# DecodeGenetics/Ratatosk

Hardware: AMD Instinct MI355X
Metric: corrected long-read bases/sec (higher is better)
Workload: dtype u64

## Files before the change

include/ratatosk_hip.h:

```cpp
#ifndef RATATOSK_HIP_H
#define RATATOSK_HIP_H

#include <stdint.h>

#ifdef __cplusplus
extern "C" {
#endif

#define RTK_OK 0
#define RTK_ERR_IO (-1)
#define RTK_ERR_FORMAT (-2)
#define RTK_ERR_ARG (-3)
#define RTK_ERR_NO_DEVICE (-4)
#define RTK_ERR_DEVICE (-5)
#define RTK_ERR_UNSUPPORTED (-6)

typedef struct rtk_graph rtk_graph;
typedef struct rtk_batch rtk_batch;

typedef struct rtk_opts {
    uint64_t insert_sz;
    uint64_t min_cov_vertices;
    uint64_t max_len_weak_region1;
    uint64_t max_km_cov;
    double weak_region_len_factor;
    double large_k_factor;
    double min_score;
    int32_t max_qual;
    int32_t out_qual;
    double min_confidence_snp_corr;
    int32_t long_read_correct;
    int32_t force_unres_snp_corr;
    uint64_t max_len_weak_region2;
    int32_t a2_exclusive;
    int32_t a3_strand_order;
    int32_t d1_desc;
    uint32_t struct_size;
} rtk_opts;

typedef struct rtk_graph_info {
    uint64_t n_unitigs, n_kmers, n_bases, n_colour_ids, n_global_sets;
    uint64_t table_slots, hbm_bytes;
    uint64_t max_km_cov_top;
    int32_t k, device;
} rtk_graph_info;

typedef struct rtk_stats {
    double ms_total, ms_lookup_exact, ms_mask, ms_lookup_inexact, ms_seeds, ms_regions, ms_correct, ms_stitch;
    uint64_t n_windows, n_probes_exact, n_probes_inexact, n_hits_inexact, n_regions, n_region_items, n_arena_overflow;
    uint64_t n_expand, n_colour_elem, n_path_base, n_align, n_align_cells;
    uint64_t in_bases, out_bases;
    uint64_t cyc_colour, cyc_paths, cyc_consensus, cyc_total, cyc_myers, cyc_sets , cyc_tostring, cyc_pathqual;
    uint64_t n_slots_exact, n_slots_inexact;
    uint64_t cyc_walk, n_moves;
    double ms_lanes;
    uint64_t n_lane_regions, n_lane_handed;
    double ms_phase;
    uint64_t n_phase_skipped;
    uint64_t n_trim_stored, n_trim_column, n_trim_fallback, n_consensus_resumed, n_consensus_swept;
    uint64_t n_fa_linked_run, n_fa_linked_skipped, n_fa_linked_entries;
    uint64_t n_strand2_run, n_strand2_skipped, n_strand2_audit_mismatch;
    uint64_t n_park_walked, n_park_deferred;
    uint64_t n_colours_small, n_colours_wide, n_colours_bits, n_colours_general, n_colours_audit_mismatch;
} rtk_stats;

int rtk_graph_load(const char* unitig_fasta_gz, const char* rtsk, int k, int n_threads, rtk_graph** out);
#define RTK_LOAD_DEVICE_TABLES 1u
int rtk_graph_load2(const char* unitig_fasta_gz, const char* rtsk, int k, int n_threads, uint32_t flags, rtk_graph** out);

int rtk_graph_upload(rtk_graph* g, int device);

int rtk_graph_shell(int k, rtk_graph** out);
int rtk_graph_n_buffers(const rtk_graph* g);
int rtk_graph_buffer(rtk_graph* g, int idx, void** dev_ptr, uint64_t* bytes);
int rtk_graph_alloc_buffers(rtk_graph* g, int device, const uint64_t* bytes, int n, const rtk_graph_info* info);
int rtk_graph_adopt_device(rtk_graph* g);
int rtk_graph_attach_buffers(rtk_graph* g, int device, void* const* dev_ptrs, const uint64_t* bytes, int n, const rtk_graph_info* info);
int rtk_graph_buffer_bytes(const rtk_graph* g, uint64_t* bytes, int n);
int rtk_graph_move_buffer(rtk_graph* g, int idx, void* dev_ptr, uint64_t bytes);
int rtk_graph_host_buffer(const rtk_graph* g, int idx, const void** p, uint64_t* bytes);
int rtk_graph_download_buffer(const rtk_graph* g, int idx, void* host_dst, uint64_t bytes);

int rtk_n_devices(void);
int rtk_device_memory(int device, uint64_t* free_bytes, uint64_t* total_bytes);
int rtk_graph_clone_to_device(const rtk_graph* src, int device, rtk_graph** out);

int rtk_graph_get_info(const rtk_graph* g, rtk_graph_info* info);
void rtk_graph_free(rtk_graph* g);
long long rtk_graph_strip_annotations(rtk_graph* g);

int rtk_reserve_scratch(int device, uint32_t max_read_len);
int rtk_reserve_second_pass(int device, uint32_t n_tickets, uint64_t phase_bytes, uint64_t region_bytes);
int rtk_graph_reserve_batches(rtk_graph* g, uint32_t n_batches, uint64_t bases_per_batch, uint32_t reads_per_batch, int with_qualities, uint64_t raw_bases_per_batch);

int rtk_opts_default(const rtk_graph* g, rtk_opts* opts);

int rtk_correct_batch(rtk_graph* g, const rtk_opts* opts, uint32_t n, const char* const* seq, const char* const* qual,
                      const uint32_t* len, char** out_seq, char** out_qual, uint32_t* out_len);
int rtk_coalesce_stats(rtk_graph* g, uint64_t* n_groups, uint64_t* n_tickets);

int rtk_batch_create(rtk_graph* g, uint32_t n, const char* const* seq, const char* const* qual, const uint32_t* len, rtk_batch** out);
int rtk_batch_create2(rtk_graph* g, uint32_t n, const char* const* seq, const char* const* qual, const uint32_t* len,
                      const char* const* raw, const uint32_t* raw_len, rtk_batch** out);
int rtk_batch_run(rtk_batch* b, const rtk_opts* opts);
int rtk_batch_run_seeds(rtk_batch* b, const rtk_opts* opts);
int rtk_batch_run_regions(rtk_batch* b, const rtk_opts* opts);
int rtk_batch_fetch(rtk_batch* b, char** out_seq, char** out_qual, uint32_t* out_len);
int rtk_batch_fetch_view(rtk_batch* b, const char** pool, const uint64_t** off, const uint32_t** len);
int rtk_batch_get_stats(const rtk_batch* b, rtk_stats* stats);
void rtk_batch_free(rtk_batch* b);


int rtk_lookup_exact(rtk_graph* g, const char* seq, uint32_t len, int64_t* hits);

int rtk_fix_snps(rtk_graph* g, const char* seq, uint32_t len, char* out);

int rtk_seeds(rtk_graph* g, const rtk_opts* opts, const char* seq, uint32_t len,
              uint64_t* n_solid, int64_t* solid, uint64_t* n_weak, int64_t* weak, uint64_t cap);

int rtk_myers_batch(uint32_t n, const char* const* query, const uint32_t* qlen, const char* const* target, const uint32_t* tlen,
                    const int32_t* k, const int32_t* mode, int want_path, int use_iupac,
                    int32_t* dist, int32_t* n_loc, int32_t* end_locs, uint32_t cap_locs, char* cigar, uint32_t cap_cigar);

int rtk_myers_batch_waves(uint32_t n, const char* const* query, const uint32_t* qlen, const char* const* target, const uint32_t* tlen,
                          const int32_t* k, const int32_t* mode, int want_path, int use_iupac,
                          int32_t* dist, int32_t* n_loc, int32_t* end_locs, uint32_t cap_locs, char* cigar, uint32_t cap_cigar, int waves);

#define RTK_MYERS_MODE_SHW_BY_COLUMN 3
#define RTK_MYERS_MODE_NW_PREFIX 4
#define RTK_MYERS_MODE_NW_PREFIX_LAST 5
void rtk_myers_column_last_routes(uint64_t* column_route, uint64_t* fallback);

int rtk_myers_batch_lanes(uint32_t n, const char* const* query, const uint32_t* qlen, const char* const* target, const uint32_t* tlen,
                          const int32_t* k, const int32_t* mode, int want_path, int use_iupac,
                          int32_t* dist, int32_t* n_loc, int32_t* end_locs, uint32_t cap_locs, char* cigar, uint32_t cap_cigar);
void rtk_myers_lanes_last_routes(uint64_t* lane_route, uint64_t* wave_route);

int rtk_index_count_kmers(int device, int k, const char* const* files, int n_files, uint32_t min_count, int n_threads, uint64_t** solid, uint64_t* n_solid);
int rtk_index_unitigs(int device, int k, const uint64_t* solid, uint64_t n_solid, char** seq_pool, uint64_t** seq_off, uint64_t** seeds, uint64_t* n_unitigs,
                      uint64_t** left, uint64_t* n_left);

int rtk_index_colour_begin(int device, int k, const char* seq_pool, const uint64_t* seq_off, uint64_t n_unitigs, void** job);
int rtk_index_colour_chunk(void* job, const char* chars, uint64_t n_chars, const uint64_t* starts, const uint32_t* ids, uint32_t n_reads);
int rtk_index_colour_end(void* job, uint64_t** events, uint64_t* n_events, uint64_t** cov);

int rtk_rescue_begin(int device, int k, const uint64_t* lr, uint64_t n_lr, const uint64_t* sr, uint64_t n_sr, uint32_t min_positions, void** job);
int rtk_rescue_chunk(void* job, const char* chars, uint64_t n_chars, const uint64_t* starts, uint32_t n_reads, unsigned char* keep);
int rtk_rescue_end(void* job, uint64_t* n_positions_probed, uint64_t* n_hits);

#define RTK_SETS_UNION 0
#define RTK_SETS_INTER 1
#define RTK_SETS_DIFF 2
#define RTK_SETS_INTER_COUNT 3
#define RTK_SETS_SORT_PAIRS 4
#define RTK_SETS_RADIX_U32 5
#define RTK_SETS_RADIX_PAIRS_U32 6
#define RTK_SETS_BM_LOWEST 7
#define RTK_SETS_BM8_LOWEST 8
#define RTK_SETS_OK 0
#define RTK_SETS_NOT_IN_BUILD 1
int rtk_sets_batch(uint32_t n, const uint32_t* op, const uint32_t* const* a, const uint32_t* na, const uint32_t* const* b, const uint32_t* nb, const uint32_t* scalar,
                   uint32_t* out_pool, const uint64_t* out_off, uint32_t* out_n, uint32_t* result, uint32_t* status);

void rtk_free(void* p);
void rtk_free_many(void** p, uint32_t n);
const char* rtk_last_error(void);
const char* rtk_version(void);
#define RTK_API_REVISION 10
int rtk_api_revision(void);

#ifdef __cplusplus
}
#endif

#endif
```

ratatosk_amd/api.py:

```python
import ctypes as C
import os

_HERE = os.path.dirname(os.path.abspath(__file__))
LIB_PATH = os.environ.get("RTK_LIB_OVERRIDE") or os.path.join(_HERE, "libratatosk_hip.so")


class RtkError(RuntimeError):
    pass


class RtkOpts(C.Structure):
    _fields_ = [("insert_sz", C.c_uint64), ("min_cov_vertices", C.c_uint64), ("max_len_weak_region1", C.c_uint64),
                ("max_km_cov", C.c_uint64), ("weak_region_len_factor", C.c_double), ("large_k_factor", C.c_double),
                ("min_score", C.c_double), ("max_qual", C.c_int32), ("out_qual", C.c_int32), ("min_confidence_snp_corr", C.c_double),
                ("long_read_correct", C.c_int32), ("force_unres_snp_corr", C.c_int32), ("max_len_weak_region2", C.c_uint64),
                ("a2_exclusive", C.c_int32), ("a3_strand_order", C.c_int32), ("d1_desc", C.c_int32), ("struct_size", C.c_uint32)]


class RtkGraphInfo(C.Structure):
    _fields_ = [("n_unitigs", C.c_uint64), ("n_kmers", C.c_uint64), ("n_bases", C.c_uint64), ("n_colour_ids", C.c_uint64),
                ("n_global_sets", C.c_uint64), ("table_slots", C.c_uint64), ("hbm_bytes", C.c_uint64), ("max_km_cov_top", C.c_uint64),
                ("k", C.c_int32), ("device", C.c_int32)]


class RtkStats(C.Structure):
    _fields_ = [(n, C.c_double) for n in ("ms_total", "ms_lookup_exact", "ms_mask", "ms_lookup_inexact", "ms_seeds", "ms_regions", "ms_correct", "ms_stitch")] + \
               [(n, C.c_uint64) for n in ("n_windows", "n_probes_exact", "n_probes_inexact", "n_hits_inexact", "n_regions", "n_region_items", "n_arena_overflow",
                                         "n_expand", "n_colour_elem", "n_path_base", "n_align", "n_align_cells", "in_bases", "out_bases",
                                         "cyc_colour", "cyc_paths", "cyc_consensus", "cyc_total", "cyc_myers", "cyc_sets", "cyc_tostring", "cyc_pathqual", "n_slots_exact", "n_slots_inexact", "cyc_walk", "n_moves")] + \
               [("ms_lanes", C.c_double), ("n_lane_regions", C.c_uint64), ("n_lane_handed", C.c_uint64), ("ms_phase", C.c_double), ("n_phase_skipped", C.c_uint64)] + \
               [(n, C.c_uint64) for n in ("n_trim_stored", "n_trim_column", "n_trim_fallback", "n_consensus_resumed", "n_consensus_swept",
                                         "n_fa_linked_run", "n_fa_linked_skipped", "n_fa_linked_entries",
                                         "n_strand2_run", "n_strand2_skipped", "n_strand2_audit_mismatch",
                                         "n_park_walked", "n_park_deferred",
                                         "n_colours_small", "n_colours_wide", "n_colours_bits", "n_colours_general", "n_colours_audit_mismatch")]

    def as_dict(self):
        return {n: getattr(self, n) for n, _ in self._fields_}


_libs = {}


os.environ.setdefault("GPU_MAX_HW_QUEUES", "16")


def load_library(path=None):
    path = path or LIB_PATH
    if path in _libs:
        return _libs[path]
    if not os.path.exists(path):
        raise RtkError("%s is missing: build it with `python -c 'import __graft_entry__ as g; g.build()'` (make -C ratatosk_amd/csrc)" % path)
    L = C.CDLL(path)
    L.rtk_last_error.restype = C.c_char_p
    L.rtk_version.restype = C.c_char_p
    L.rtk_graph_load.argtypes = [C.c_char_p, C.c_char_p, C.c_int, C.c_int, C.POINTER(C.c_void_p)]
    L.rtk_graph_load2.argtypes = [C.c_char_p, C.c_char_p, C.c_int, C.c_int, C.c_uint32, C.POINTER(C.c_void_p)]
    L.rtk_graph_move_buffer.argtypes = [C.c_void_p, C.c_int, C.c_void_p, C.c_uint64]
    L.rtk_graph_host_buffer.argtypes = [C.c_void_p, C.c_int, C.POINTER(C.c_void_p), C.POINTER(C.c_uint64)]
    L.rtk_graph_download_buffer.argtypes = [C.c_void_p, C.c_int, C.c_void_p, C.c_uint64]
    L.rtk_graph_upload.argtypes = [C.c_void_p, C.c_int]
    L.rtk_graph_shell.argtypes = [C.c_int, C.POINTER(C.c_void_p)]
    L.rtk_graph_n_buffers.argtypes = [C.c_void_p]
    L.rtk_graph_buffer.argtypes = [C.c_void_p, C.c_int, C.POINTER(C.c_void_p), C.POINTER(C.c_uint64)]
    L.rtk_graph_alloc_buffers.argtypes = [C.c_void_p, C.c_int, C.POINTER(C.c_uint64), C.c_int, C.POINTER(RtkGraphInfo)]
    L.rtk_graph_adopt_device.argtypes = [C.c_void_p]
    L.rtk_graph_buffer_bytes.argtypes = [C.c_void_p, C.POINTER(C.c_uint64), C.c_int]
    L.rtk_graph_get_info.argtypes = [C.c_void_p, C.POINTER(RtkGraphInfo)]
    L.rtk_graph_free.argtypes = [C.c_void_p]
    L.rtk_opts_default.argtypes = [C.c_void_p, C.POINTER(RtkOpts)]
    L.rtk_correct_batch.argtypes = [C.c_void_p, C.POINTER(RtkOpts), C.c_uint32, C.POINTER(C.c_char_p), C.POINTER(C.c_char_p), C.POINTER(C.c_uint32),
                                    C.POINTER(C.c_void_p), C.POINTER(C.c_void_p), C.POINTER(C.c_uint32)]
    L.rtk_batch_create.argtypes = [C.c_void_p, C.c_uint32, C.POINTER(C.c_char_p), C.POINTER(C.c_char_p), C.POINTER(C.c_uint32), C.POINTER(C.c_void_p)]
    L.rtk_batch_create2.argtypes = [C.c_void_p, C.c_uint32, C.POINTER(C.c_char_p), C.POINTER(C.c_char_p), C.POINTER(C.c_uint32),
                                    C.POINTER(C.c_char_p), C.POINTER(C.c_uint32), C.POINTER(C.c_void_p)]
    L.rtk_batch_run.argtypes = [C.c_void_p, C.POINTER(RtkOpts)]
    L.rtk_graph_strip_annotations.restype = C.c_longlong
    L.rtk_graph_strip_annotations.argtypes = [C.c_void_p]
    L.rtk_batch_run_seeds.argtypes = [C.c_void_p, C.POINTER(RtkOpts)]
    L.rtk_batch_run_regions.argtypes = [C.c_void_p, C.POINTER(RtkOpts)]
    L.rtk_batch_fetch.argtypes = [C.c_void_p, C.POINTER(C.c_void_p), C.POINTER(C.c_void_p), C.POINTER(C.c_uint32)]
    L.rtk_batch_fetch_view.argtypes = [C.c_void_p, C.POINTER(C.c_char_p), C.POINTER(C.POINTER(C.c_uint64)), C.POINTER(C.POINTER(C.c_uint32))]
    L.rtk_n_devices.restype = C.c_int
    L.rtk_device_memory.argtypes = [C.c_int, C.POINTER(C.c_uint64), C.POINTER(C.c_uint64)]
    L.rtk_graph_clone_to_device.argtypes = [C.c_void_p, C.c_int, C.POINTER(C.c_void_p)]
    L.rtk_batch_get_stats.argtypes = [C.c_void_p, C.POINTER(RtkStats)]
    L.rtk_batch_free.argtypes = [C.c_void_p]
    L.rtk_lookup_exact.argtypes = [C.c_void_p, C.c_char_p, C.c_uint32, C.POINTER(C.c_int64)]
    L.rtk_fix_snps.argtypes = [C.c_void_p, C.c_char_p, C.c_uint32, C.c_char_p]
    L.rtk_seeds.argtypes = [C.c_void_p, C.POINTER(RtkOpts), C.c_char_p, C.c_uint32, C.POINTER(C.c_uint64), C.POINTER(C.c_int64),
                            C.POINTER(C.c_uint64), C.POINTER(C.c_int64), C.c_uint64]
    L.rtk_myers_batch.argtypes = [C.c_uint32, C.POINTER(C.c_char_p), C.POINTER(C.c_uint32), C.POINTER(C.c_char_p), C.POINTER(C.c_uint32),
                                  C.POINTER(C.c_int32), C.POINTER(C.c_int32), C.c_int, C.c_int,
                                  C.POINTER(C.c_int32), C.POINTER(C.c_int32), C.POINTER(C.c_int32), C.c_uint32, C.c_char_p, C.c_uint32]
    L.rtk_myers_batch_waves.argtypes = L.rtk_myers_batch.argtypes + [C.c_int]
    L.rtk_myers_batch_lanes.argtypes = L.rtk_myers_batch.argtypes
    L.rtk_myers_batch_lanes.restype = C.c_int
    L.rtk_coalesce_stats.argtypes = [C.c_void_p, C.POINTER(C.c_uint64), C.POINTER(C.c_uint64)]
    L.rtk_graph_reserve_batches.argtypes = [C.c_void_p, C.c_uint32, C.c_uint64, C.c_uint32, C.c_int, C.c_uint64]
    L.rtk_free_many.argtypes = [C.POINTER(C.c_void_p), C.c_uint32]; L.rtk_free_many.restype = None
    if L.rtk_api_revision() >= 9:
        L.rtk_rescue_begin.argtypes = [C.c_int, C.c_int, C.POINTER(C.c_uint64), C.c_uint64, C.POINTER(C.c_uint64), C.c_uint64, C.c_uint32, C.POINTER(C.c_void_p)]
        L.rtk_rescue_chunk.argtypes = [C.c_void_p, C.c_char_p, C.c_uint64, C.POINTER(C.c_uint64), C.c_uint32, C.POINTER(C.c_ubyte)]
        L.rtk_rescue_end.argtypes = [C.c_void_p, C.POINTER(C.c_uint64), C.POINTER(C.c_uint64)]
    if L.rtk_api_revision() >= 10:
        L.rtk_sets_batch.argtypes = [C.c_uint32, C.POINTER(C.c_uint32), C.POINTER(C.POINTER(C.c_uint32)), C.POINTER(C.c_uint32), C.POINTER(C.POINTER(C.c_uint32)), C.POINTER(C.c_uint32),
                                     C.POINTER(C.c_uint32), C.POINTER(C.c_uint32), C.POINTER(C.c_uint64), C.POINTER(C.c_uint32), C.POINTER(C.c_uint32), C.POINTER(C.c_uint32)]
    L.rtk_free.argtypes = [C.c_void_p]
    _libs[path] = L
    return L


RTK_LOAD_DEVICE_TABLES = 1


def _b(s):
    return s.encode() if isinstance(s, str) else s


class Graph:

    def __init__(self, fasta_gz, rtsk, k=31, device=0, lib_path=None, upload=True, n_threads=None, host_tables=None):
        self.L = load_library(lib_path)
        self.h = C.c_void_p()
        if n_threads is None:
            n_threads = max(1, min(32, os.cpu_count() or 1))
        if host_tables is None:
            host_tables = not upload or os.environ.get("RTK_HOST_TABLES") == "1"
        self._check(self.L.rtk_graph_load2(_b(fasta_gz), _b(rtsk), k, n_threads, 0 if host_tables else RTK_LOAD_DEVICE_TABLES, C.byref(self.h)))
        self.k = k
        if upload:
            self._check(self.L.rtk_graph_upload(self.h, device))

    def _check(self, rc):
        if rc != 0:
            raise RtkError("rtk error %d: %s" % (rc, self.L.rtk_last_error().decode()))

    def close(self):
        if getattr(self, "h", None):
            self.L.rtk_graph_free(self.h)
            self.h = None

    def __del__(self):
        try:
            self.close()
        except Exception:
            pass

    def info(self):
        i = RtkGraphInfo()
        self._check(self.L.rtk_graph_get_info(self.h, C.byref(i)))
        return i

    def opts(self, **kw):
        o = RtkOpts()
        self._check(self.L.rtk_opts_default(self.h, C.byref(o)))
        for k_, v in kw.items():
            setattr(o, k_, v)
        return o

    def lookup_exact(self, seq):
        s = _b(seq)
        nw = max(0, len(s) - self.k + 1)
        out = (C.c_int64 * max(1, nw))()
        self._check(self.L.rtk_lookup_exact(self.h, s, len(s), out))
        return [out[i] for i in range(nw)]

    def fix_snps(self, seq):
        s = _b(seq)
        out = C.create_string_buffer(len(s) + 1)
        self._check(self.L.rtk_fix_snps(self.h, s, len(s), out))
        return out.raw[:len(s)]

    def seeds(self, seq, opts=None):
        s = _b(seq)
        o = opts or self.opts()
        cap = 64 * len(s) + 64
        ns, nw = C.c_uint64(), C.c_uint64()
        so, we = (C.c_int64 * (4 * cap))(), (C.c_int64 * (4 * cap))()
        self._check(self.L.rtk_seeds(self.h, C.byref(o), s, len(s), C.byref(ns), so, C.byref(nw), we, cap))
        f = lambda a, n: [(a[4 * i], a[4 * i + 1], a[4 * i + 2], a[4 * i + 3]) for i in range(n)]
        return f(so, ns.value), f(we, nw.value)

    def correct_batch(self, seqs, quals=None, opts=None, raw=None):
        b = Batch(self, seqs, quals, raw)
        try:
            b.run(opts)
            return b.fetch()
        finally:
            b.close()


class Batch:

    def __init__(self, graph, seqs, quals=None, raw=None):
        self.g = graph
        self.L = graph.L
        n = len(seqs)
        bs = [_b(s) for s in seqs]
        seq_arr = (C.c_char_p * n)(*bs)
        qual_arr = None
        if quals is not None:
            bq = [_b(q) for q in quals]
            qual_arr = (C.c_char_p * n)(*bq)
        lens = (C.c_uint32 * n)(*[len(b) for b in bs])
        self.n = n
        self.in_bases = sum(len(b) for b in bs)
        self.h = C.c_void_p()
        if raw is not None:
            br = [_b(s) for s in raw]
            raw_arr = (C.c_char_p * n)(*br)
            raw_lens = (C.c_uint32 * n)(*[len(b) for b in br])
            graph._check(self.L.rtk_batch_create2(graph.h, n, seq_arr, qual_arr, lens, raw_arr, raw_lens, C.byref(self.h)))
        else:
            graph._check(self.L.rtk_batch_create(graph.h, n, seq_arr, qual_arr, lens, C.byref(self.h)))

    def run(self, opts=None):
        o = opts or self.g.opts()
        self.g._check(self.L.rtk_batch_run(self.h, C.byref(o)))

    def run_seeds(self, opts=None):
        o = opts or self.g.opts()
        self.g._check(self.L.rtk_batch_run_seeds(self.h, C.byref(o)))

    def run_regions(self, opts=None):
        o = opts or self.g.opts()
        self.g._check(self.L.rtk_batch_run_regions(self.h, C.byref(o)))

    def fetch(self):
        n = self.n
        os_, oq = (C.c_void_p * n)(), (C.c_void_p * n)()
        ol = (C.c_uint32 * n)()
        self.g._check(self.L.rtk_batch_fetch(self.h, os_, oq, ol))
        out = []
        for i in range(n):
            out.append((C.string_at(os_[i], ol[i]).decode(), C.string_at(oq[i], ol[i]).decode()))
            self.L.rtk_free(os_[i]); self.L.rtk_free(oq[i])
        return out

    def stats(self):
        s = RtkStats()
        self.g._check(self.L.rtk_batch_get_stats(self.h, C.byref(s)))
        return s.as_dict()

    def close(self):
        if getattr(self, "h", None):
            self.L.rtk_batch_free(self.h)
            self.h = None

    def __del__(self):
        try:
            self.close()
        except Exception:
            pass


def myers_batch(queries, targets, ks=None, modes=None, want_path=False, use_iupac=True, lib_path=None, waves=0, lanes=False):
    L = load_library(lib_path)
    n = len(queries)
    bq = [_b(q) for q in queries]; bt = [_b(t) for t in targets]
    ks = ks if ks is not None else [-1] * n
    modes = modes if modes is not None else [0] * n
    qa = (C.c_char_p * n)(*bq); ta = (C.c_char_p * n)(*bt)
    ql = (C.c_uint32 * n)(*[len(x) for x in bq]); tl = (C.c_uint32 * n)(*[len(x) for x in bt])
    ka = (C.c_int32 * n)(*ks); ma = (C.c_int32 * n)(*modes)
    cap_locs = max(len(x) for x in bt) + 2 if n else 2
    cap_cig = 4 * (max((len(x) for x in bq), default=0) + max((len(x) for x in bt), default=0)) + 16
    dist = (C.c_int32 * n)(); nloc = (C.c_int32 * n)(); locs = (C.c_int32 * (n * cap_locs))()
    cig = C.create_string_buffer(n * cap_cig) if want_path else None
    if lanes:
        rc = L.rtk_myers_batch_lanes(n, qa, ql, ta, tl, ka, ma, 1 if want_path else 0, 1 if use_iupac else 0, dist, nloc, locs, cap_locs, cig, cap_cig)
    elif waves > 1:
        rc = L.rtk_myers_batch_waves(n, qa, ql, ta, tl, ka, ma, 1 if want_path else 0, 1 if use_iupac else 0, dist, nloc, locs, cap_locs, cig, cap_cig, waves)
    else:
        rc = L.rtk_myers_batch(n, qa, ql, ta, tl, ka, ma, 1 if want_path else 0, 1 if use_iupac else 0, dist, nloc, locs, cap_locs, cig, cap_cig)
    if rc != 0:
        raise RtkError("rtk error %d: %s" % (rc, L.rtk_last_error().decode()))
    out = []
    for i in range(n):
        el = [locs[i * cap_locs + j] for j in range(min(nloc[i], cap_locs))] if dist[i] >= 0 else []
        c = ""
        if want_path:
            c = cig.raw[i * cap_cig:(i + 1) * cap_cig].split(b"\0", 1)[0].decode()
        out.append((dist[i], el, c))
    return out


def _u64_array(a):
    if hasattr(a, "ctypes"):
        import numpy as np
        arr = np.ascontiguousarray(a, dtype=np.uint64)
        return arr, arr.ctypes.data_as(C.POINTER(C.c_uint64)), int(arr.size)
    arr = (C.c_uint64 * max(1, len(a)))(*[int(x) for x in a])
    return arr, arr, len(a)


def rescue_reads(lr_kmers, sr_kmers, seqs, k=31, min_positions=31, device=0, stats=None, lib_path=None):
    L = load_library(lib_path)
    if L.rtk_api_revision() < 9:
        raise RtkError("%s is of interface revision %d: the rescue entries came with revision 9" % (L._name, L.rtk_api_revision()))
    keep_lr, p_lr, n_lr = _u64_array(lr_kmers)
    keep_sr, p_sr, n_sr = _u64_array(sr_kmers)
    job = C.c_void_p()

    def check(rc):
        if rc != 0:
            raise RtkError("rtk error %d: %s" % (rc, L.rtk_last_error().decode()))

    check(L.rtk_rescue_begin(device, k, p_lr, n_lr, p_sr, n_sr, min_positions, C.byref(job)))
    out = []
    try:
        bs = [_b(s) for s in seqs]
        i = 0
        while i < len(bs):
            j, size = i, 0
            while j < len(bs) and (j == i or (size + len(bs[j]) + 1 <= (48 << 20) and j - i < (2 << 20))):
                size += len(bs[j]) + 1; j += 1
            starts, at = (C.c_uint64 * (j - i))(), 0
            for r in range(i, j):
                starts[r - i] = at; at += len(bs[r]) + 1
            chars = b"\n".join(bs[i:j]) + b"\n"
            keep = (C.c_ubyte * (j - i))()
            check(L.rtk_rescue_chunk(job, chars, len(chars), starts, j - i, keep))
            out.extend(bool(x) for x in keep)
            i = j
    except Exception:
        L.rtk_rescue_end(job, None, None)
        raise
    probed, hits = C.c_uint64(), C.c_uint64()
    check(L.rtk_rescue_end(job, C.byref(probed), C.byref(hits)))
    if stats is not None:
        stats["n_positions_probed"], stats["n_hits"] = probed.value, hits.value
    return out


MODE_SHW_BY_COLUMN, MODE_NW_PREFIX, MODE_NW_PREFIX_LAST = 3, 4, 5


def myers_column_last_routes(lib_path=None):
    L = load_library(lib_path)
    a, b = C.c_uint64(), C.c_uint64()
    L.rtk_myers_column_last_routes.argtypes = [C.POINTER(C.c_uint64), C.POINTER(C.c_uint64)]; L.rtk_myers_column_last_routes.restype = None
    L.rtk_myers_column_last_routes(C.byref(a), C.byref(b))
    return a.value, b.value


def myers_lanes_last_routes(lib_path=None):
    L = load_library(lib_path)
    a, b = C.c_uint64(), C.c_uint64()
    L.rtk_myers_lanes_last_routes.argtypes = [C.POINTER(C.c_uint64), C.POINTER(C.c_uint64)]; L.rtk_myers_lanes_last_routes.restype = None
    L.rtk_myers_lanes_last_routes(C.byref(a), C.byref(b))
    return a.value, b.value


SETS_UNION, SETS_INTER, SETS_DIFF, SETS_INTER_COUNT, SETS_SORT_PAIRS, SETS_RADIX_U32, SETS_RADIX_PAIRS_U32, SETS_BM_LOWEST, SETS_BM8_LOWEST = range(9)
SETS_OK, SETS_NOT_IN_BUILD = 0, 1


def sets_batch(problems, lib_path=None):
    import numpy as np
    L = load_library(lib_path)
    if L.rtk_api_revision() < 10:
        raise RtkError("%s is of interface revision %d: rtk_sets_batch came with revision 10" % (L._name, L.rtk_api_revision()))
    n = len(problems)
    keep, off = [], [0]
    ops = (C.c_uint32 * max(1, n))(); na = (C.c_uint32 * max(1, n))(); nb = (C.c_uint32 * max(1, n))(); sc = (C.c_uint32 * max(1, n))()
    pa = (C.POINTER(C.c_uint32) * max(1, n))(); pb = (C.POINTER(C.c_uint32) * max(1, n))()
    for i, (op, a, b, scalar) in enumerate(problems):
        if op == SETS_SORT_PAIRS:
            a = np.ascontiguousarray(a, dtype="<u8"); b = np.ascontiguousarray(b, dtype="<u8")
            count_a, count_b, a, b = int(a.size), int(b.size), a.view("<u4"), b.view("<u4")
        else:
            a = np.ascontiguousarray(a, dtype=np.uint32); b = np.ascontiguousarray(b, dtype=np.uint32)
            count_a, count_b = int(a.size), int(b.size)
        keep.append((a, b))
        ops[i], na[i], nb[i], sc[i] = op, count_a, count_b, scalar
        pa[i] = a.ctypes.data_as(C.POINTER(C.c_uint32)); pb[i] = b.ctypes.data_as(C.POINTER(C.c_uint32))
        need = {SETS_UNION: count_a + count_b, SETS_INTER: count_a, SETS_DIFF: count_a, SETS_INTER_COUNT: 0, SETS_SORT_PAIRS: 4 * count_a, SETS_RADIX_U32: count_a,
                SETS_RADIX_PAIRS_U32: 2 * count_a, SETS_BM_LOWEST: min(scalar, count_b), SETS_BM8_LOWEST: min(scalar, count_b)}.get(op, 0)
        off.append(off[-1] + need)
    out = np.zeros(max(1, off[-1]), dtype=np.uint32)
    offs = (C.c_uint64 * (n + 1))(*off)
    out_n = (C.c_uint32 * max(1, n))(); res = (C.c_uint32 * max(1, n))(); st = (C.c_uint32 * max(1, n))()
    rc = L.rtk_sets_batch(n, ops, pa, na, pb, nb, sc, out.ctypes.data_as(C.POINTER(C.c_uint32)), offs, out_n, res, st)
    if rc != 0:
        raise RtkError("rtk error %d: %s" % (rc, L.rtk_last_error().decode()))
    ret = []
    for i, (op, _, _, _) in enumerate(problems):
        if out_n[i] > off[i + 1] - off[i]:
            raise RtkError("rtk_sets_batch: problem %d reports %d output words for a slice of %d" % (i, out_n[i], off[i + 1] - off[i]))
        w = out[off[i]:off[i] + out_n[i]]
        if op == SETS_SORT_PAIRS and st[i] == SETS_OK:
            h = len(w) // 2
            words = (w[:h].copy().view("<u8").tolist(), w[h:].copy().view("<u8").tolist())
        else:
            words = w.tolist()
        ret.append((words, int(res[i]), int(st[i])))
    return ret


def run_pipelined(batches, opts=None):
    import threading
    prev, err = None, []

    def seeds(b):
        try:
            b.run_seeds(opts)
        except Exception as e:
            err.append(e)

    for b in batches:
        t = threading.Thread(target=seeds, args=(b,))
        t.start()
        if prev is not None:
            prev.run_regions(opts)
        t.join()
        if err:
            raise err[0]
        prev = b
    if prev is not None:
        prev.run_regions(opts)
```

ratatosk_amd/csrc/hip/rtk_colours.h:

```cpp
#ifndef RTK_COLOURS_H
#define RTK_COLOURS_H

#define RTK_CB_MAX_IDS (RTK_LDS_SET_CAP - 384u)
#define RTK_CB_MAX_SLOTS 24u

#ifndef RTK_SIM
RTK_DEV void rtk_radix_sort_u32(uint32_t* a, uint32_t* b, uint32_t n, uint32_t* bins, uint32_t max_key) {
    const uint32_t lane = static_cast<uint32_t>(rtk_lane());
    const uint64_t lt = (1ull << lane) - 1ull;
    int passes = 0; { uint32_t m = max_key; while (m) { ++passes; m >>= 8; } if (passes == 0) passes = 1; }
    if (passes & 1) ++passes;
    uint32_t* src = a; uint32_t* dst = b;
    for (int ps = 0; ps < passes; ++ps) {
        const int sh = 8 * ps;
        for (uint32_t i = lane; i < 256u; i += RTK_WAVE) bins[i] = 0u;
        RTK_WG_SYNC();
        for (uint32_t c0 = 0; c0 < n; c0 += RTK_WAVE) {
            const uint32_t i = c0 + lane; const bool ok = i < n;
            const uint32_t d = ok ? ((src[i] >> sh) & 0xFFu) : 0x100u;
            uint64_t eq = rtk_ballot(ok);
            for (int bt = 0; bt < 8; ++bt) { const uint64_t bb = rtk_ballot((d >> bt) & 1u); eq &= ((d >> bt) & 1u) ? bb : ~bb; }
            if (ok && (eq & lt) == 0ull) atomicAdd(&bins[d], static_cast<uint32_t>(rtk_popc(eq)));
        }
        RTK_WG_SYNC();
        {
            uint32_t v[4]; uint32_t sum = 0;
            for (int x = 0; x < 4; ++x) { v[x] = bins[4u * lane + static_cast<uint32_t>(x)]; sum += v[x]; }
            int tot; uint32_t base = static_cast<uint32_t>(rtk_wave_excl_scan(static_cast<int>(sum), &tot));
            RTK_WG_SYNC();
            for (int x = 0; x < 4; ++x) { bins[4u * lane + static_cast<uint32_t>(x)] = base; base += v[x]; }
        }
        RTK_WG_SYNC();
        for (uint32_t c0 = 0; c0 < n; c0 += RTK_WAVE) {
            const uint32_t i = c0 + lane; const bool ok = i < n;
            const uint32_t key = ok ? src[i] : 0u;
            const uint32_t d = ok ? ((key >> sh) & 0xFFu) : 0x100u;
            uint64_t eq = rtk_ballot(ok);
            for (int bt = 0; bt < 8; ++bt) { const uint64_t bb = rtk_ballot((d >> bt) & 1u); eq &= ((d >> bt) & 1u) ? bb : ~bb; }
            const uint32_t before = static_cast<uint32_t>(rtk_popc(eq & lt));
            uint32_t base = 0;
            if (ok) base = bins[d];
            RTK_WG_SYNC();
            if (ok && before == 0u) bins[d] = base + static_cast<uint32_t>(rtk_popc(eq));
            if (ok) dst[base + before] = key;
            RTK_WG_SYNC();
        }
        uint32_t* t_ = src; src = dst; dst = t_;
    }
}
#endif

#ifdef RTK_SIM
struct RtkBM { uint64_t w[64]; };
inline RtkBM rtk_bm_zero() { RtkBM r; for (int i = 0; i < 64; ++i) r.w[i] = 0; return r; }
inline RtkBM operator|(const RtkBM& a, const RtkBM& b) { RtkBM r; for (int i = 0; i < 64; ++i) r.w[i] = a.w[i] | b.w[i]; return r; }
inline RtkBM operator&(const RtkBM& a, const RtkBM& b) { RtkBM r; for (int i = 0; i < 64; ++i) r.w[i] = a.w[i] & b.w[i]; return r; }
inline RtkBM rtk_bm_andn(const RtkBM& a, const RtkBM& b) { RtkBM r; for (int i = 0; i < 64; ++i) r.w[i] = a.w[i] & ~b.w[i]; return r; }
inline uint32_t rtk_bm_count(const RtkBM& a) { uint32_t c = 0; for (int i = 0; i < 64; ++i) c += static_cast<uint32_t>(__builtin_popcountll(a.w[i])); return c; }
inline RtkBM rtk_bm_lowest(const RtkBM& a, uint32_t q) { RtkBM r = rtk_bm_zero(); for (int i = 0; i < 64 && q; ++i) { uint64_t x = a.w[i]; while (x && q) { const uint64_t b = x & (~x + 1ull); r.w[i] |= b; x ^= b; --q; } } return r; }
inline RtkBM rtk_bm_load(const uint64_t* p) { RtkBM r; for (int i = 0; i < 64; ++i) r.w[i] = p[i]; return r; }
inline void rtk_bm_store(uint64_t* p, const RtkBM& a) { for (int i = 0; i < 64; ++i) p[i] = a.w[i]; }
#else
typedef uint64_t RtkBM;
RTK_DEV RtkBM rtk_bm_zero() { return 0ull; }
RTK_DEV RtkBM rtk_bm_andn(RtkBM a, RtkBM b) { return a & ~b; }
RTK_DEV uint32_t rtk_bm_count(RtkBM a) { return static_cast<uint32_t>(rtk_u(rtk_wave_sum(rtk_popc(a)))); }
RTK_DEV RtkBM rtk_bm_lowest(RtkBM a, uint32_t q) {
    int total; const int before = rtk_wave_excl_scan(rtk_popc(a), &total);
    int keep = static_cast<int>(q) - before; const int mine = rtk_popc(a);
    keep = keep < 0 ? 0 : (keep > mine ? mine : keep);
    uint64_t rest = a; for (int i = 0; i < keep; ++i) rest &= rest - 1ull;
    return a & ~rest;
}
RTK_DEV RtkBM rtk_bm_load(const uint64_t* p) { return p[rtk_lane()]; }
RTK_DEV void rtk_bm_store(uint64_t* p, RtkBM a) { p[rtk_lane()] = a; }
#endif

RTK_DEV RtkBM rtk_bm_from_ids(const uint32_t* uni, uint32_t U, uint64_t* scatter, const uint32_t* ids, uint32_t n) {
#ifdef RTK_SIM
    (void)scatter;
    RtkBM r = rtk_bm_zero();
    for (uint32_t i = 0; i < n; ++i) { const uint32_t x = rtk_lower_bound(uni, U, ids[i]); r.w[x >> 6] |= 1ull << (x & 63u); }
    return r;
#else
    scatter[rtk_lane()] = 0ull;
    RTK_WG_SYNC();
    for (uint32_t i = static_cast<uint32_t>(rtk_lane()); i < n; i += RTK_WAVE) {
        const uint32_t id = ids[i];
        uint32_t lo = 0, hi = U; while (lo < hi) { const uint32_t mid = (lo + hi) >> 1; if (uni[mid] < id) lo = mid + 1; else hi = mid; }
        atomicOr(reinterpret_cast<unsigned long long*>(scatter) + (lo >> 6), 1ull << (lo & 63u));
    }
    RTK_WG_SYNC();
    return scatter[rtk_lane()];
#endif
}


#ifndef RTK_SIM
#ifndef RTK_CS_MAX_IDS
#define RTK_CS_MAX_IDS 512u
#endif
static_assert(2u * RTK_CS_MAX_IDS + 768u <= RTK_LDS_SET_CAP && RTK_CS_MAX_IDS <= 512u, "small path of the colour selection: universe + unsorted ids + 24 x 2 x 8 vector words in the LDS buffer");
RTK_DEV int rtk_sum8(int v) {
    v += __builtin_amdgcn_update_dpp(0, v, 0xB1, 0xF, 0xF, false);
    v += __builtin_amdgcn_update_dpp(0, v, 0x4E, 0xF, 0xF, false);
    v += __builtin_amdgcn_update_dpp(0, v, 0x141, 0xF, 0xF, false);
    return v;
}
RTK_DEV uint32_t rtk_bm8_count(RtkBM a) { return static_cast<uint32_t>(__builtin_amdgcn_readfirstlane(rtk_sum8(rtk_popc(a)))); }
RTK_DEV RtkBM rtk_bm8_lowest(RtkBM a, uint32_t q) {
    const int mine = rtk_popc(a);
    int inc = mine;
    inc += __builtin_amdgcn_update_dpp(0, inc, 0x111, 0xF, 0xF, true);
    inc += __builtin_amdgcn_update_dpp(0, inc, 0x112, 0xF, 0xF, true);
    inc += __builtin_amdgcn_update_dpp(0, inc, 0x114, 0xF, 0xF, true);
    int keep = static_cast<int>(q) - (inc - mine);
    keep = keep < 0 ? 0 : (keep > mine ? mine : keep);
    uint64_t rest = a; for (int i = 0; i < keep; ++i) rest &= rest - 1ull;
    return a & ~rest;
}
RTK_FN uint32_t rtk_choose_colors_small(const RCtx& c_, const SideList& side_s_, const SideList& side_e_, const SideList& side_w_) {
    const RCtx& c = *rtk_u(&c_); const SideList& side_s = *rtk_u(&side_s_); const SideList& side_e = *rtk_u(&side_e_); const SideList& side_w = *rtk_u(&side_w_); RTK_ASSUME_LDS(&side_s); RTK_ASSUME_LDS(&side_e); RTK_ASSUME_LDS(&side_w);
    RegionScratch& s = rtk_hdr(c);
    const GraphView& g = c.g;
    const uint32_t nw = rtk_u(side_w.n), ne = rtk_u(side_e.n), ns = rtk_u(side_s.n), n_slots = nw + ne + ns;
    if (n_slots == 0 || n_slots > RTK_CB_MAX_SLOTS) return RTK_NONE32;
    const uint32_t lane = static_cast<uint32_t>(rtk_lane());
    const uint32_t* const pw = rtk_u(side_w.u); const uint32_t* const pe = rtk_u(side_e.u); const uint32_t* const ps = rtk_u(side_s.u);
    const uint8_t* const qw = rtk_u(side_w.nb); const uint8_t* const qe = rtk_u(side_e.nb); const uint8_t* const qs = rtk_u(side_s.nb);
    const uint32_t* const col = g.col; const uint64_t* const loff = g.loff; const uint64_t* const goff = g.goff; const int32_t* const gid = g.gid; const uint32_t* const cardp = g.card;
    unsigned long long tl_ = rtk_clock();
#define RTK_CS_LAP(i) { (void)tl_; }
    uint32_t m_u = 0, m_nl = 0, m_ng = 0, m_card = 0, m_nb = 0; uint64_t m_lo = 0, m_go = 0; int32_t m_gi = -1;
    if (lane < n_slots) {
        const uint32_t* pu; const uint8_t* pn; uint32_t i = lane;
        if (i < nw) { pu = pw; pn = qw; } else if (i - nw < ne) { i -= nw; pu = pe; pn = qe; } else { i -= nw + ne; pu = ps; pn = qs; }
        m_u = pu[i]; m_nb = pn[i];
        m_gi = gid[m_u]; m_lo = loff[m_u]; m_nl = static_cast<uint32_t>(loff[m_u + 1] - m_lo); m_card = cardp[m_u];
        if (m_gi >= 0) { m_go = goff[m_gi]; m_ng = static_cast<uint32_t>(goff[m_gi + 1] - m_go); }
    }
    int total = 0; const uint32_t st = static_cast<uint32_t>(rtk_wave_excl_scan(static_cast<int>(m_nl + m_ng), &total));
    const uint32_t T = static_cast<uint32_t>(rtk_u(total));
    const bool big = T > RTK_CS_MAX_IDS;
    if (T > RTK_CB_MAX_IDS || (big && (s.set_cap < RTK_CB_MAX_IDS || s.set_cap < 2u * 2u * 64u * RTK_CB_MAX_SLOTS))) return RTK_NONE32;
    RTK_CS_LAP(1)
    const uint32_t min_cov_v = c.o.min_cov_vertices;
    bool dup = false;
    for (uint32_t j = 0; j + 1 < n_slots; ++j) { const uint32_t uj = rtk_shfl(m_u, static_cast<int>(j)); dup = dup || ((j < lane) && (uj == m_u)); }
    const bool cand = lane < n_slots && m_card >= min_cov_v && !dup;
    const uint64_t cb = rtk_ballot(cand); const uint32_t nsp = static_cast<uint32_t>(rtk_popc(cb));
    const uint64_t key = rtk_d1_key(m_card, m_u, c.o.d1_desc);
    uint32_t rank = 0;
    for (uint32_t j = 0; j < n_slots; ++j) { const uint64_t kj = rtk_shfl(key, static_cast<int>(j)); rank += (((cb >> j) & 1ull) && kj < key) ? 1u : 0u; }
    uint32_t src = 0;
    for (uint32_t j = 0; j < n_slots; ++j) { const uint32_t rj = rtk_shfl(rank, static_cast<int>(j)); if (((cb >> j) & 1ull) && rj == lane) src = j; }
    const uint32_t cov = 30;
    const uint32_t k_slot = src; const uint32_t k_card = rtk_shfl(m_card, static_cast<int>(src));
    uint32_t k_quota = k_card < cov ? k_card : cov;
    RTK_CS_LAP(2)
    uint32_t* const L = rtk_lds_set_buf();
    uint32_t* const uni = L; uint32_t* const raw = L + RTK_CS_MAX_IDS;
    uint64_t* const cbm = big ? reinterpret_cast<uint64_t*>(s.set[2].get()) : reinterpret_cast<uint64_t*>(L + 2u * RTK_CS_MAX_IDS);
    const uint32_t VW = big ? 64u : 8u;
    uint32_t P = 64; while (P < T) P <<= 1;
    for (uint32_t t0 = 0; t0 < P; t0 += RTK_WAVE) {
        const uint32_t t = t0 + lane;
        uint32_t i = 0;
        for (uint32_t j = 1; j < n_slots; ++j) { const uint32_t sj = rtk_shfl(st, static_cast<int>(j)); if (sj <= t) i = j; }
        const uint32_t s_i = rtk_shfl(st, static_cast<int>(i)), nl_i = rtk_shfl(m_nl, static_cast<int>(i));
        const uint64_t lo_i = rtk_shfl(m_lo, static_cast<int>(i)), go_i = rtk_shfl(m_go, static_cast<int>(i));
        uint32_t x = 0xFFFFFFFFu;
        if (t < T) { const uint32_t off = t - s_i; x = col[off < nl_i ? lo_i + off : go_i + (off - nl_i)]; if (!big) raw[t] = x; }
        if (t < T || !big) uni[t] = x;
    }
    RTK_WG_SYNC();
    s.cnt[RTK_RC_COLOUR] += T;
    RTK_CS_LAP(3)
    {
        uint32_t mx = 0; for (uint32_t i2 = lane; i2 < T; i2 += RTK_WAVE) mx = uni[i2] > mx ? uni[i2] : mx;
        for (int o = 32; o > 0; o >>= 1) { const uint32_t v2 = static_cast<uint32_t>(__shfl_xor(static_cast<int>(mx), o, 64)); mx = v2 > mx ? v2 : mx; }
        if (big) rtk_radix_sort_u32(uni, s.set[1], T, L + RTK_CB_MAX_IDS, rtk_u(mx));
        else rtk_radix_sort_u32(uni, L + 2u * RTK_CS_MAX_IDS, T, L + 2u * RTK_CS_MAX_IDS + RTK_CS_MAX_IDS, rtk_u(mx));
    }
    uint32_t U = 0;
    for (uint32_t i0 = 0; i0 < T; i0 += RTK_WAVE) {
        const uint32_t i = i0 + lane;
        uint32_t x = 0; bool keep = false;
        if (i < T) { x = uni[i]; keep = (i == 0) || (uni[i - 1] != x); }
        RTK_WG_SYNC();
        const uint64_t bal = rtk_ballot(keep);
        if (keep) uni[U + static_cast<uint32_t>(rtk_popc(bal & ((1ull << lane) - 1ull)))] = x;
        U += static_cast<uint32_t>(rtk_popc(bal));
        RTK_WG_SYNC();
    }
    RTK_CS_LAP(4)
    for (uint32_t i = lane; i < n_slots * 2u * VW; i += RTK_WAVE) cbm[i] = 0ull;
    RTK_WG_SYNC();
    for (uint32_t t0 = 0; t0 < T; t0 += RTK_WAVE) {
        const uint32_t t = t0 + lane;
        uint32_t i = 0;
        for (uint32_t j = 1; j < n_slots; ++j) { const uint32_t sj = rtk_shfl(st, static_cast<int>(j)); if (sj <= t) i = j; }
        const uint32_t s_i = rtk_shfl(st, static_cast<int>(i)), nl_i = rtk_shfl(m_nl, static_cast<int>(i));
        const uint64_t lo_i2 = rtk_shfl(m_lo, static_cast<int>(i)), go_i2 = rtk_shfl(m_go, static_cast<int>(i));
        if (t < T) {
            const uint32_t off2 = t - s_i;
            const uint32_t id = big ? col[off2 < nl_i ? lo_i2 + off2 : go_i2 + (off2 - nl_i)] : raw[t];
            uint32_t lo = 0, hi = U; while (lo < hi) { const uint32_t mid = (lo + hi) >> 1; if (uni[mid] < id) lo = mid + 1; else hi = mid; }
            const uint32_t seg = 2u * i + ((t - s_i) >= nl_i ? 1u : 0u);
            atomicOr(reinterpret_cast<unsigned long long*>(cbm) + seg * VW + (lo >> 6), 1ull << (lo & 63u));
        }
    }
    RTK_WG_SYNC();
    RTK_CS_LAP(5)
    auto ld = [&](uint32_t idx) -> RtkBM { if (lane >= VW) return 0ull; return big ? static_cast<RtkBM>(__hip_atomic_load(reinterpret_cast<const unsigned long long*>(cbm) + idx * VW + lane, __ATOMIC_RELAXED, __HIP_MEMORY_SCOPE_AGENT)) : cbm[idx * VW + lane]; };
    auto cnt_ = [&](RtkBM a) -> uint32_t { return big ? rtk_bm_count(a) : rtk_bm8_count(a); };
    auto low_ = [&](RtkBM a, uint32_t q) -> RtkBM { return big ? rtk_bm_lowest(a, q) : rtk_bm8_lowest(a, q); };
    RtkBM a[6];
    for (int sh = 0; sh < 6; ++sh) {
        RtkBM acc = 0ull;
        const uint32_t first = (sh % 3 == 0) ? 0u : (sh % 3 == 1 ? nw : nw + ne), cnt = (sh % 3 == 0) ? nw : (sh % 3 == 1 ? ne : ns);
        const uint32_t want_nb = sh >= 3 ? 1u : 0u;
        for (uint32_t slot = first; slot < first + cnt; ++slot) {
            if (rtk_u(rtk_shfl(m_nb, static_cast<int>(slot))) != want_nb) continue;
            const bool has_global = rtk_u(rtk_shfl(m_gi, static_cast<int>(slot))) >= 0;
            acc |= ld(2u * slot + (has_global ? 1u : 0u));
        }
        a[sh] = acc;
    }
    const RtkBM pos0 = a[0] | a[3], pos1 = a[1] | a[4], pos2 = a[2] | a[5];
    const RtkBM a01 = pos0 & pos1, a12 = pos1 & pos2, a02 = pos0 & pos2;
    const RtkBM nobranch_all = a[3] | a[4] | a[5];
    const RtkBM i3 = a01 & a12, i2 = a01 | a12 | a02;
    RtkBM nobranch = nobranch_all, branching = 0ull, prev2 = 0ull, all = 0ull;
    uint32_t nb_unselected = nsp;
    for (int i = 5; i >= 0; --i) {
        if (nb_unselected == 0) break;
        RtkBM a2;
        if (i == 5) a2 = nobranch & i3;
        else if (i == 4) { nobranch = rtk_bm_andn(nobranch, prev2); a2 = nobranch & i2; }
        else if (i == 3) { nobranch = rtk_bm_andn(nobranch, prev2); a2 = nobranch; }
        else if (i == 2) { branching = rtk_bm_andn(a[0] | a[1] | a[2], nobranch_all); a2 = branching & i3; }
        else if (i == 1) { branching = rtk_bm_andn(branching, prev2); a2 = branching & i2; }
        else { branching = rtk_bm_andn(branching, prev2); a2 = branching; }
        prev2 = a2;
        if (cnt_(a2) == 0) continue;
        nb_unselected = 0;
        RtkBM curr = a2;
        for (uint32_t j = 0; j < nsp; ++j) {
            int quota = static_cast<int>(rtk_u(rtk_shfl(k_quota, static_cast<int>(j))));
            if (quota > 0) {
                const uint32_t slot = rtk_u(rtk_shfl(k_slot, static_cast<int>(j)));
                const RtkBM cu = ld(2u * slot) | ld(2u * slot + 1u);
                if (i == 0 || cnt_(cu & curr) >= 1) {
                    const uint32_t cd = rtk_u(rtk_shfl(k_card, static_cast<int>(j))); const uint32_t min_cov = cd < cov ? cd : cov;
                    const uint32_t sh = cnt_(cu & all);
                    quota = static_cast<int>(min_cov - (sh < min_cov ? sh : min_cov));
                    if (quota > 0) {
                        const uint32_t all_card = cnt_(all);
                        const RtkBM pid = low_(cu & curr, static_cast<uint32_t>(quota));
                        all = all | pid; curr = rtk_bm_andn(curr, pid);
                        const int gained = static_cast<int>(cnt_(all) - all_card);
                        quota -= gained < quota ? gained : quota;
                    }
                }
                if (lane == j) k_quota = static_cast<uint32_t>(quota);
            }
            nb_unselected += quota > 0 ? 1u : 0u;
        }
    }
    RTK_CS_LAP(6)
    const uint32_t n_all = rtk_bm_count(all);
    if (n_all > s.set_cap) { rtk_fail_ovf(s, 9); return 0; }
    uint32_t* out = s.set[0];
    { int tot2; uint32_t at = static_cast<uint32_t>(rtk_wave_excl_scan(rtk_popc(all), &tot2)); uint64_t x = all;
      while (x) { const int b = __builtin_ctzll(x); out[at++] = uni[64u * lane + static_cast<uint32_t>(b)]; x &= x - 1ull; } }
    rtk_sync();
    s.cnt[big ? RTK_RC_COLOURS_WIDE : RTK_RC_COLOURS_SMALL] += 1;
    return n_all;
}
#endif

RTK_FN uint32_t rtk_choose_colors_bits(const RCtx& c_, const SideList& side_s_, const SideList& side_e_, const SideList& side_w_) {
    const RCtx& c = *rtk_u(&c_); const SideList& side_s = *rtk_u(&side_s_); const SideList& side_e = *rtk_u(&side_e_); const SideList& side_w = *rtk_u(&side_w_); RTK_ASSUME_LDS(&side_s); RTK_ASSUME_LDS(&side_e); RTK_ASSUME_LDS(&side_w);
    RegionScratch& s = rtk_hdr(c);
    const GraphView& g = c.g;
    const SideList* sides[3] = {&side_w, &side_e, &side_s};
    const uint32_t n_slots = side_w.n + side_e.n + side_s.n;
    if (n_slots == 0 || n_slots > RTK_CB_MAX_SLOTS || s.set_cap < 2 * RTK_CB_MAX_IDS + 64u * 4u * RTK_CB_MAX_SLOTS || s.list_cap < 2 * RTK_CB_MAX_SLOTS) return RTK_NONE32;
    uint32_t T = 0;
    for (int sd = 0; sd < 3; ++sd) for (uint32_t i = 0; i < sides[sd]->n; ++i) {
        const uint32_t u = sides[sd]->u[i]; const int32_t gi = g.gid[u];
        T += static_cast<uint32_t>(g.loff[u + 1] - g.loff[u]) + (gi >= 0 ? static_cast<uint32_t>(g.goff[gi + 1] - g.goff[gi]) : 0u);
        if (T > RTK_CB_MAX_IDS) return RTK_NONE32;
    }
    uint64_t* keys = s.list[4]; uint64_t* vals = s.list[3]; uint64_t* slot_of = s.list[5];
    uint32_t nsp = 0;
    { uint32_t slot = 0;
      for (int sd = 0; sd < 3; ++sd) for (uint32_t i = 0; i < sides[sd]->n; ++i, ++slot) {
        const uint32_t u = sides[sd]->u[i];
        if (g.card[u] < c.o.min_cov_vertices) continue;
        bool dup = false; for (uint32_t j0 = 0; j0 < nsp && !dup; j0 += RTK_WAVE) { const uint32_t j = j0 + static_cast<uint32_t>(rtk_lane()); dup = rtk_ballot(j < nsp && rtk_d1_unitig(keys[j], c.o.d1_desc) == u) != 0ull; }
        if (dup) continue;
        keys[nsp] = rtk_d1_key(g.card[u], u, c.o.d1_desc); vals[nsp] = slot; ++nsp; rtk_sync();
      } }
    rtk_sort_pairs(keys, vals, nsp);
    const uint32_t cov = 30;
    for (uint32_t j = static_cast<uint32_t>(rtk_lane()); j < nsp; j += RTK_WAVE) { slot_of[j] = vals[j]; const uint32_t cd = static_cast<uint32_t>(keys[j] >> 32); vals[j] = cd < cov ? cd : cov; }
    rtk_sync();
    uint32_t* gathered = s.set[1];
    { uint32_t at = 0;
      for (int sd = 0; sd < 3; ++sd) for (uint32_t i = 0; i < sides[sd]->n; ++i) {
        const uint32_t u = sides[sd]->u[i]; const int32_t gi = g.gid[u];
        const uint32_t nl = static_cast<uint32_t>(g.loff[u + 1] - g.loff[u]); const uint32_t* pl = g.col + g.loff[u];
        for (uint32_t x = static_cast<uint32_t>(rtk_lane()); x < nl; x += RTK_WAVE) gathered[at + x] = pl[x];
        at += nl;
        if (gi >= 0) { const uint32_t ng = static_cast<uint32_t>(g.goff[gi + 1] - g.goff[gi]); const uint32_t* pg = g.col + g.goff[gi];
                       for (uint32_t x = static_cast<uint32_t>(rtk_lane()); x < ng; x += RTK_WAVE) gathered[at + x] = pg[x]; at += ng; }
      } }
    rtk_sync();
    s.cnt[RTK_RC_COLOUR] += T;
    uint32_t U = 0;
#ifdef RTK_SIM
    uint32_t* const uni = s.set[1] + RTK_CB_MAX_IDS; uint64_t* const scatter = nullptr;
    { for (uint32_t i = 0; i < T; ++i) uni[i] = gathered[i];
      std::sort(uni, uni + T);
      for (uint32_t i = 0; i < T; ++i) if (i == 0 || uni[i] != uni[i - 1]) uni[U++] = uni[i]; }
#else
    uint32_t* const uni = rtk_lds_set_buf(); uint64_t* const scatter = reinterpret_cast<uint64_t*>(uni + RTK_CB_MAX_IDS + 256u);
    {
      uint32_t mx = 0;
      for (uint32_t i = static_cast<uint32_t>(rtk_lane()); i < T; i += RTK_WAVE) { const uint32_t x = gathered[i]; uni[i] = x; mx = x > mx ? x : mx; }
      for (int o = 32; o > 0; o >>= 1) { const uint32_t v2 = static_cast<uint32_t>(__shfl_xor(static_cast<int>(mx), o, 64)); mx = v2 > mx ? v2 : mx; }
      RTK_WG_SYNC();
      rtk_radix_sort_u32(uni, gathered, T, uni + RTK_CB_MAX_IDS, rtk_u(mx));
      for (uint32_t i0 = 0; i0 < T; i0 += RTK_WAVE) {
          const uint32_t i = i0 + static_cast<uint32_t>(rtk_lane());
          uint32_t x = 0; bool keep = false;
          if (i < T) { x = uni[i]; keep = (i == 0) || (uni[i - 1] != x); }
          RTK_WG_SYNC();
          const uint64_t bal = rtk_ballot(keep);
          if (keep) uni[U + static_cast<uint32_t>(rtk_popc(bal & ((1ull << rtk_lane()) - 1ull)))] = x;
          U += static_cast<uint32_t>(rtk_popc(bal));
          RTK_WG_SYNC();
      } }
#endif
    uint64_t* const store = reinterpret_cast<uint64_t*>(s.set[2].get());
    { uint32_t slot = 0;
      for (int sd = 0; sd < 3; ++sd) for (uint32_t i = 0; i < sides[sd]->n; ++i, ++slot) {
        const uint32_t u = sides[sd]->u[i]; const int32_t gi = g.gid[u];
        const RtkBM bl = rtk_bm_from_ids(uni, U, scatter, g.col + g.loff[u], static_cast<uint32_t>(g.loff[u + 1] - g.loff[u]));
        rtk_bm_store(store + (2ull * slot) * 64ull, bl);
        const RtkBM bg = gi >= 0 ? rtk_bm_from_ids(uni, U, scatter, g.col + g.goff[gi], static_cast<uint32_t>(g.goff[gi + 1] - g.goff[gi])) : rtk_bm_zero();
        rtk_bm_store(store + (2ull * slot + 1ull) * 64ull, bg);
      } }
    rtk_sync();
    RtkBM a[6];
    for (int sh = 0; sh < 6; ++sh) {
        RtkBM acc = rtk_bm_zero();
        uint32_t slot = (sh % 3 == 0) ? 0u : (sh % 3 == 1 ? side_w.n : side_w.n + side_e.n);
        const SideList& sl = *sides[sh % 3]; const uint8_t want_nb = sh >= 3 ? 1 : 0;
        for (uint32_t i = 0; i < sl.n; ++i, ++slot) {
            if (sl.nb[i] != want_nb) continue;
            const bool has_global = g.gid[sl.u[i]] >= 0;
            acc = acc | rtk_bm_load(store + (2ull * slot + (has_global ? 1ull : 0ull)) * 64ull);
        }
        a[sh] = acc;
    }
    const RtkBM pos0 = a[0] | a[3], pos1 = a[1] | a[4], pos2 = a[2] | a[5];
    const RtkBM a01 = pos0 & pos1, a12 = pos1 & pos2, a02 = pos0 & pos2;
    const RtkBM nobranch_all = a[3] | a[4] | a[5];
    const RtkBM i3 = a01 & a12, i2 = a01 | a12 | a02;
    RtkBM nobranch = nobranch_all, branching = rtk_bm_zero(), prev2 = rtk_bm_zero(), all = rtk_bm_zero();
    uint32_t nb_unselected = nsp;
    for (int i = 5; i >= 0; --i) {
        if (nb_unselected == 0) break;
        RtkBM a2;
        if (i == 5) a2 = nobranch & i3;
        else if (i == 4) { nobranch = rtk_bm_andn(nobranch, prev2); a2 = nobranch & i2; }
        else if (i == 3) { nobranch = rtk_bm_andn(nobranch, prev2); a2 = nobranch; }
        else if (i == 2) { branching = rtk_bm_andn(a[0] | a[1] | a[2], nobranch_all); a2 = branching & i3; }
        else if (i == 1) { branching = rtk_bm_andn(branching, prev2); a2 = branching & i2; }
        else { branching = rtk_bm_andn(branching, prev2); a2 = branching; }
        prev2 = a2;
        if (rtk_bm_count(a2) == 0) continue;
        nb_unselected = 0;
        RtkBM curr = a2;
        for (uint32_t j = 0; j < nsp; ++j) {
            const uint32_t u = rtk_d1_unitig(rtk_ld(keys + j), c.o.d1_desc);
            int quota = static_cast<int>(rtk_ld(vals + j));
            if (quota > 0) {
                const uint64_t slot = rtk_ld(slot_of + j);
                const RtkBM cu = rtk_bm_load(store + (2ull * slot) * 64ull) | rtk_bm_load(store + (2ull * slot + 1ull) * 64ull);
                if (i == 0 || rtk_bm_count(cu & curr) >= 1) {
                    const uint32_t cd = rtk_ld(g.card.get() + u); const uint32_t min_cov = cd < cov ? cd : cov;
                    const uint32_t sh = rtk_bm_count(cu & all);
                    quota = static_cast<int>(min_cov - (sh < min_cov ? sh : min_cov));
                    if (quota > 0) {
                        const uint32_t all_card = rtk_bm_count(all);
                        const RtkBM pid = rtk_bm_lowest(cu & curr, static_cast<uint32_t>(quota));
                        all = all | pid; curr = rtk_bm_andn(curr, pid);
                        const int gained = static_cast<int>(rtk_bm_count(all) - all_card);
                        quota -= gained < quota ? gained : quota;
                    }
                }
            }
            vals[j] = static_cast<uint64_t>(quota);
            nb_unselected += quota > 0 ? 1u : 0u;
        }
        rtk_sync();
    }
    const uint32_t n_all = rtk_bm_count(all);
    if (n_all > s.set_cap) { rtk_fail_ovf(s, 9); return 0; }
    uint32_t* out = s.set[0];
#ifdef RTK_SIM
    { uint32_t at = 0; for (uint32_t w = 0; w < 64; ++w) { uint64_t x = all.w[w]; while (x) { const int b = __builtin_ctzll(x); out[at++] = uni[64u * w + static_cast<uint32_t>(b)]; x &= x - 1ull; } } }
#else
    { int total; uint32_t at = static_cast<uint32_t>(rtk_wave_excl_scan(rtk_popc(all), &total)); uint64_t x = all;
      while (x) { const int b = __builtin_ctzll(x); out[at++] = uni[64u * static_cast<uint32_t>(rtk_lane()) + static_cast<uint32_t>(b)]; x &= x - 1ull; } }
#endif
    rtk_sync();
    return n_all;
}

#endif
```

ratatosk_amd/csrc/hip/rtk_device.hip:

```cpp
#include <algorithm>
#include <atomic>
#include <chrono>
#include <cmath>
#include <cstdio>
#include <cstring>
#include <map>
#include <memory>
#include <condition_variable>
#include <mutex>
#include <string>
#include <thread>
#include <vector>

#include "../../../include/ratatosk_hip.h"
#include "../host/flat_graph.hpp"
#include "rtk_graph_tables.h"
#include "rtk_mem.h"
#include "rtk_myers.h"
#include "rtk_myers_lane.h"
#include "rtk_types.h"
#include "rtk_wave.h"

#ifdef RTK_SIM
thread_local int rtk_sim_block_id = 0;
// ... 432 lines not shown

RTK_FN void rtk_myers_column_item(const MyersScratch& sc, const MyersProb& p, uint32_t i, const char* q, const char* t, int use_iupac, int32_t* dist, int32_t* n_loc, int32_t* end_locs,
                                  uint32_t cap_locs, uint8_t* moves_out, uint32_t* n_moves_out, uint32_t cap_moves, uint32_t* status) {
    const int m = static_cast<int>(p.qlen), n = static_cast<int>(p.tlen); const bool iupac = use_iupac != 0;
    uint32_t route = 2, nm = 0;
    MyersResult r;
    if (p.mode == RTK_MYERS_MODE_SHW_BY_COLUMN) {
        if (rtk_myers_shw_by_column(sc, t, n, q, m, iupac, 0, 0, &r, nullptr)) route = 1;
        else r = rtk_myers_distance(sc, q, m, t, n, -1, RTK_MODE_SHW, iupac);
        if (cap_locs > 0) end_locs[static_cast<uint64_t>(i) * cap_locs] = r.first;
        if (r.nloc > 1 && static_cast<uint32_t>(r.nloc) <= cap_locs) end_locs[static_cast<uint64_t>(i) * cap_locs + (r.nloc - 1)] = r.last;
        n_loc[i] = r.nloc;
    } else {
        const int k = p.k; const bool last_only = p.mode == RTK_MYERS_MODE_NW_PREFIX_LAST;
        int at = 0, last = -1;
        if (k > 0 && rtk_myers_shw_by_column(sc, q, m, t, n, iupac, 1, k, &r, &at)) {
            const long long W = (k + 63) >> 6;
            if (static_cast<uint32_t>(k) <= sc.r_cap && static_cast<uint32_t>(k + n) <= sc.mv_cap && (2LL * 8 + 4) * W * n + 8LL * n < 1024 * 1024) {
                if (last_only) last = rtk_myers_last_move(sc, k, n, n, at);
                else rtk_myers_walk(sc, k, n, n, at, &nm);
                r.dist = at; route = 1;
            }
        }
        if (route != 1) {
            if (k > 0 && n > 0) r = rtk_myers_path(sc, q, k, t, n, RTK_MODE_NW, iupac, &nm);
            else r = rtk_myers_distance(sc, q, k, t, n, -1, RTK_MODE_NW, iupac);
            if (last_only) { rtk_sync(); last = nm ? static_cast<int>(rtk_ld(sc.moves.get() + (nm - 1u))) : -1; nm = 0; }
        }
        if (cap_locs > 0) end_locs[static_cast<uint64_t>(i) * cap_locs] = last_only ? last : n - 1;
        n_loc[i] = 1;
    }
    dist[i] = r.dist;
    if (nm <= cap_moves) rtk_wcopy(moves_out + static_cast<uint64_t>(i) * cap_moves, sc.moves, nm);
    n_moves_out[i] = nm;
    status[i] = *sc.overflow | (route << 16);
}

RTK_FN void rtk_myers_batch_item(const MyersScratch& sc, const MyersProb& p, uint32_t i, const char* pool, int want_path, int use_iupac, int32_t* dist, int32_t* n_loc, int32_t* end_locs, uint32_t cap_locs,
                                 uint8_t* moves_out, uint32_t* n_moves_out, uint32_t cap_moves, uint32_t* status) {
    *sc.overflow = 0;
    const char* q = pool + p.q_off; const char* t = pool + p.t_off;
    if (p.mode >= RTK_MYERS_MODE_SHW_BY_COLUMN) { rtk_myers_column_item(sc, p, i, q, t, use_iupac, dist, n_loc, end_locs, cap_locs, moves_out, n_moves_out, cap_moves, status); return; }
    const MyersResult r = rtk_myers_distance(sc, q, static_cast<int>(p.qlen), t, static_cast<int>(p.tlen), p.k, p.mode, use_iupac != 0, cap_locs ? end_locs + static_cast<uint64_t>(i) * cap_locs : nullptr, static_cast<int>(cap_locs));
    dist[i] = r.dist; n_loc[i] = r.nloc;
    uint32_t nm = 0;
    if (want_path && r.dist >= 0 && p.qlen > 0 && p.tlen > 0) {
        if (p.k < 0 && p.mode != RTK_MODE_HW) {
            const MyersResult r2 = rtk_myers_path(sc, q, static_cast<int>(p.qlen), t, static_cast<int>(p.tlen), p.mode, use_iupac != 0, &nm);
            if (r2.dist != r.dist || r2.first != r.first) *sc.overflow = 3;
        } else
        rtk_myers_alignment(sc, q, static_cast<int>(p.qlen), t, r.first + 1, r.dist, use_iupac != 0, &nm);
        if (nm <= cap_moves) rtk_wcopy(moves_out + static_cast<uint64_t>(i) * cap_moves, sc.moves, nm);
    }
    n_moves_out[i] = nm;
    status[i] = *sc.overflow;
}

RTK_GLOBAL void k_myers_batch(const MyersProb* probs, uint32_t n, const char* pool, int want_path, int use_iupac, char* scratch, uint64_t scratch_stride, ScratchCfg cfg,
                              int grid, int32_t* dist, int32_t* n_loc, int32_t* end_locs, uint32_t cap_locs, uint8_t* moves_out, uint32_t* n_moves_out, uint32_t cap_moves, uint32_t* status, unsigned long long* prof) {
#ifdef RTK_SIM
    const MyersScratch sc = scratch_carve(scratch + static_cast<uint64_t>(RTK_BLOCK_ID) * scratch_stride, cfg);
#else
    __shared__ MyersScratch sc;
    sc = scratch_carve(scratch + static_cast<uint64_t>(RTK_BLOCK_ID) * scratch_stride, cfg);
    __syncthreads();
#endif
    for (uint32_t i = static_cast<uint32_t>(RTK_BLOCK_ID); i < n; i += static_cast<uint32_t>(grid))
        rtk_myers_batch_item(sc, probs[i], i, pool, want_path, use_iupac, dist, n_loc, end_locs, cap_locs, moves_out, n_moves_out, cap_moves, status);
    if (prof && rtk_lane() == 0) { rtk_atomic_add(prof + 0, sc.hb_total.get()); rtk_atomic_add(prof + 1, sc.hb_pass.get()); rtk_atomic_add(prof + 2, sc.hb_split.get()); rtk_atomic_add(prof + 3, sc.hb_leaf.get()); rtk_atomic_add(prof + 4, sc.walk_cycles.get()); }
}

#ifndef RTK_SIM
void rtk_launch_myers_batch_waves(int grid, int waves, const MyersProb* probs, uint32_t n, const char* pool, int want_path, int use_iupac, char* scratch, uint64_t scratch_stride, const ScratchCfg& cfg,
                                  int32_t* dist, int32_t* n_loc, int32_t* end_locs, uint32_t cap_locs, uint8_t* moves_out, uint32_t* n_moves_out, uint32_t cap_moves, uint32_t* status, unsigned long long* prof);
#endif
static thread_local uint64_t g_col_routes[2] = {0, 0};
extern "C" void rtk_myers_column_last_routes(uint64_t* column_route, uint64_t* fallback) { if (column_route) *column_route = g_col_routes[0]; if (fallback) *fallback = g_col_routes[1]; }
extern "C" int rtk_myers_batch(uint32_t n, const char* const* query, const uint32_t* qlen, const char* const* target, const uint32_t* tlen,
                               const int32_t* k, const int32_t* mode, int want_path, int use_iupac,
                               int32_t* dist, int32_t* n_loc, int32_t* end_locs, uint32_t cap_locs, char* cigar, uint32_t cap_cigar) {
    return rtk_myers_batch_waves(n, query, qlen, target, tlen, k, mode, want_path, use_iupac, dist, n_loc, end_locs, cap_locs, cigar, cap_cigar, 1);
}
extern "C" int rtk_myers_batch_waves(uint32_t n, const char* const* query, const uint32_t* qlen, const char* const* target, const uint32_t* tlen,
                                     const int32_t* k, const int32_t* mode, int want_path, int use_iupac,
                                     int32_t* dist, int32_t* n_loc, int32_t* end_locs, uint32_t cap_locs, char* cigar, uint32_t cap_cigar, int waves) {
    if (waves > 16) return rtk_fail(RTK_ERR_ARG, "rtk_myers_batch_waves: at most 16 waves per workgroup");
    if (!query || !qlen || !target || !tlen || !k || !mode || !dist || !n_loc || (!end_locs && cap_locs)) return rtk_fail(RTK_ERR_ARG, "rtk_myers_batch: null argument");
    if (rtk_device_count() <= 0) return rtk_fail(RTK_ERR_NO_DEVICE, "rtk_myers_batch: no HIP device visible (no CPU fallback)");
    if (n == 0) return RTK_OK;
    try {
        std::vector<MyersProb> probs(n);
        std::string pool;
        uint32_t max_q = 1, max_t = 1;
        for (uint32_t i = 0; i < n; ++i) {
            probs[i].q_off = pool.size(); pool.append(query[i], qlen[i]);
            probs[i].t_off = pool.size(); pool.append(target[i], tlen[i]);
            probs[i].qlen = qlen[i]; probs[i].tlen = tlen[i]; probs[i].k = k[i]; probs[i].mode = mode[i];
            if (mode[i] == RTK_MODE_HW && want_path) return rtk_fail(RTK_ERR_UNSUPPORTED, "rtk_myers_batch: HW path alignment is not on the hot path");
            if (mode[i] < 0 || mode[i] > RTK_MYERS_MODE_NW_PREFIX_LAST || (mode[i] > RTK_MODE_HW && waves > 1)) return rtk_fail(RTK_ERR_ARG, "rtk_myers_batch: unknown mode (the test-only modes 3 to 5 run on one wave)");
            if ((mode[i] == RTK_MYERS_MODE_SHW_BY_COLUMN && k[i] >= 0) || (mode[i] >= RTK_MYERS_MODE_NW_PREFIX && (k[i] < 0 || static_cast<uint32_t>(k[i]) > qlen[i])))
                return rtk_fail(RTK_ERR_ARG, "rtk_myers_batch: mode 3 takes k < 0, modes 4 and 5 a query row 0 <= k <= qlen");
            max_q = std::max(max_q, qlen[i]); max_t = std::max(max_t, tlen[i]);
        }
        for (uint32_t i = 0; i < n; ++i) if (mode[i] > RTK_MODE_HW) { max_q = max_t = std::max(max_q, max_t); break; }
        ScratchCfg cfg;
        cfg.w_cap = (max_q + 63) / 64 + 1; cfg.t_cap = max_t + 64; cfg.r_cap = max_q + 64; cfg.mv_cap = max_q + max_t + 64;
        cfg.tb_cap_words = std::max<uint64_t>(4ull * 52429 + 64, 4ull * cfg.w_cap + 64);
        const int grid = static_cast<int>(std::min<uint32_t>(n, static_cast<uint32_t>(default_grid() / 4 > 0 ? default_grid() / 4 : 1)));
        const uint64_t stride = scratch_bytes(cfg) + (waves > 1 ? static_cast<uint64_t>((waves < RTK_LEAF_WAVES ? waves : RTK_LEAF_WAVES) - 1) * scratch_bytes(rtk_leaf_cfg()) : 0ull);
        const uint32_t cap_moves = want_path ? (max_q + max_t + 8) : 1;
        struct Held { std::vector<void*> v; void* get(uint64_t bytes) { v.push_back(nullptr); v.back() = rtk_dmalloc(bytes); return v.back(); } void release() { for (void* p : v) if (p) rtk_dfree(p); v.clear(); } ~Held() { release(); } } held;
        char* dpool = static_cast<char*>(held.get(pool.size() + 64));
        MyersProb* dprobs = static_cast<MyersProb*>(held.get(sizeof(MyersProb) * n));
        char* dscr = static_cast<char*>(held.get(stride * grid));
        int32_t* ddist = static_cast<int32_t*>(held.get(4ull * n)); int32_t* dnloc = static_cast<int32_t*>(held.get(4ull * n));
        int32_t* dlocs = static_cast<int32_t*>(held.get(4ull * n * cap_locs + 8)); uint32_t* dst = static_cast<uint32_t*>(held.get(4ull * n));
        uint8_t* dmoves = static_cast<uint8_t*>(held.get(static_cast<uint64_t>(n) * cap_moves + 8)); uint32_t* dnm = static_cast<uint32_t*>(held.get(4ull * n));
        rtk_h2d(dpool, pool.data(), pool.size()); rtk_h2d(dprobs, probs.data(), sizeof(MyersProb) * n);
        unsigned long long* dprof = nullptr;
        if (rtk_knob_myers_prof()) { dprof = static_cast<unsigned long long*>(rtk_dmalloc(64)); const unsigned long long z[8] = {0, 0, 0, 0, 0, 0, 0, 0}; rtk_h2d(dprof, z, 64); }
#ifndef RTK_SIM
        if (waves > 1) rtk_launch_myers_batch_waves(grid, waves, static_cast<const MyersProb*>(dprobs), n, static_cast<const char*>(dpool), want_path, use_iupac, dscr, stride, cfg, ddist, dnloc, dlocs, cap_locs, dmoves, dnm, cap_moves, dst, dprof);
        else
#endif
        { RtkTimer tk; const bool timed = rtk_knob_myers_time() && waves <= 1; if (timed) tk.start(0);
          rtk_launch(k_myers_batch, grid, 0, static_cast<const MyersProb*>(dprobs), n, static_cast<const char*>(dpool), want_path, use_iupac, dscr, stride, cfg, grid, ddist, dnloc, dlocs, cap_locs, dmoves, dnm, cap_moves, dst, dprof);
          if (timed) { tk.stop(0); rtk_dsync(); fprintf(stderr, "[rtk myers time] one wave per problem: %u problems, %d waves, kernel %.3f ms\n", n, grid, tk.elapsed()); } }
        if (dprof) { rtk_dsync(); unsigned long long pc[8]; rtk_d2h(pc, dprof, 64); rtk_dfree(dprof);
            fprintf(stderr, "[rtk myers prof] waves %d: Hirschberg driver %.3g cycles (half passes %.3g, columns + split %.3g, leaf tracebacks %.3g of which walks %.3g)\n", waves, double(pc[0]), double(pc[1]), double(pc[2]), double(pc[3]), double(pc[4])); }
        rtk_dsync();
        std::vector<uint32_t> st(n), nm(n);
        rtk_d2h(dist, ddist, 4ull * n); rtk_d2h(n_loc, dnloc, 4ull * n); if (cap_locs) rtk_d2h(end_locs, dlocs, 4ull * n * cap_locs);
        rtk_d2h(st.data(), dst, 4ull * n); rtk_d2h(nm.data(), dnm, 4ull * n);
        int rc = RTK_OK;
        g_col_routes[0] = 0; g_col_routes[1] = 0;
        for (uint32_t i = 0; i < n; ++i) {
            if (st[i] & 0xFFFFu) rc = rtk_fail(RTK_ERR_DEVICE, "rtk_myers_batch: scratch capacity exceeded on device");
            if (mode[i] > RTK_MODE_HW) ++g_col_routes[(st[i] >> 16) == 1u ? 0 : 1];
        }
        if (want_path && cigar && rc == RTK_OK) {
            std::vector<uint8_t> mv(static_cast<size_t>(n) * cap_moves);
            rtk_d2h(mv.data(), dmoves, mv.size());
            static const char code[4] = {'M', 'I', 'D', 'M'};
            for (uint32_t i = 0; i < n; ++i) {
                std::string c;
                const uint8_t* a = &mv[static_cast<size_t>(i) * cap_moves];
                for (uint32_t x = 0; x < nm[i];) { uint32_t y = x; while (y < nm[i] && code[a[y]] == code[a[x]]) ++y; c += std::to_string(y - x); c.push_back(code[a[x]]); x = y; }
                if (c.size() + 1 > cap_cigar) { rc = rtk_fail(RTK_ERR_ARG, "rtk_myers_batch: cigar buffer too small"); break; }
                memcpy(cigar + static_cast<size_t>(i) * cap_cigar, c.c_str(), c.size() + 1);
            }
        }
        held.release();
        return rc;
    } catch (const std::exception& e) { return rtk_fail(RTK_ERR_DEVICE, e.what()); }
}

RTK_GLOBAL void k_myers_batch_lanes(const MyersProb* probs, uint32_t n, const char* pool, int want_path, int use_iupac, char* scratch, uint64_t stride, int grid, int32_t* dist, int32_t* n_loc, int32_t* end_locs, uint32_t cap_locs,
                                    uint8_t* moves_out, uint32_t* n_moves_out, uint32_t cap_moves, uint32_t* status) {
#ifdef RTK_SIM
    static thread_local uint64_t lpeq[RTK_ML_PEQ_WORDS];
#else
    __shared__ uint64_t lpeq[RTK_ML_PEQ_WORDS];
#endif
    uint64_t* const peq = lpeq + rtk_lane();
    char* const area = scratch + static_cast<uint64_t>(RTK_BLOCK_ID) * stride;
    int32_t* const cs = reinterpret_cast<int32_t*>(area) + rtk_lane();
    uint64_t* const tb = reinterpret_cast<uint64_t*>(area + rtk_ml_scratch_bytes()) + rtk_lane();
    for (uint64_t i0 = static_cast<uint64_t>(RTK_BLOCK_ID) * RTK_WAVE; i0 < n; i0 += static_cast<uint64_t>(grid) * RTK_WAVE) {
        const uint64_t i = i0 + static_cast<uint64_t>(rtk_lane());
        if (i >= n) continue;
        const MyersProb p = probs[i];
        const int m = static_cast<int>(p.qlen), tn = static_cast<int>(p.tlen);
        int32_t d = -1, nl = 0, first = -1; uint32_t nm = 0;
        uint32_t st = rtk_myers_lane(pool + p.q_off, m, pool + p.t_off, tn, p.k, p.mode, use_iupac != 0, peq, cs, &d, &nl, cap_locs ? end_locs + i * cap_locs : nullptr, static_cast<int>(cap_locs), &first);
        if (st == 0u && want_path && d >= 0 && m > 0 && tn > 0) {
            uint8_t* const mv = moves_out + i * cap_moves;
            if (first + 1 == 0) { if (static_cast<uint32_t>(m) > cap_moves) st = 1u; else { for (int x = 0; x < m; ++x) mv[x] = 1; nm = static_cast<uint32_t>(m); } }
            else st = rtk_myers_lane_path(m, pool + p.t_off, first + 1, peq, tb, mv, cap_moves, &nm);
        }
        status[i] = st; dist[i] = d; n_loc[i] = nl; n_moves_out[i] = nm;
    }
}

static thread_local uint64_t g_ml_routes[2] = {0, 0};
extern "C" void rtk_myers_lanes_last_routes(uint64_t* lane_route, uint64_t* wave_route) { if (lane_route) *lane_route = g_ml_routes[0]; if (wave_route) *wave_route = g_ml_routes[1]; }
extern "C" int rtk_myers_batch_lanes(uint32_t n, const char* const* query, const uint32_t* qlen, const char* const* target, const uint32_t* tlen,
                                     const int32_t* k, const int32_t* mode, int want_path, int use_iupac,
                                     int32_t* dist, int32_t* n_loc, int32_t* end_locs, uint32_t cap_locs, char* cigar, uint32_t cap_cigar) {
    if (!query || !qlen || !target || !tlen || !k || !mode || !dist || !n_loc || (!end_locs && cap_locs)) return rtk_fail(RTK_ERR_ARG, "rtk_myers_batch_lanes: null argument");
    if (rtk_device_count() <= 0) return rtk_fail(RTK_ERR_NO_DEVICE, "rtk_myers_batch_lanes: no HIP device visible (no CPU fallback)");
    g_ml_routes[0] = 0; g_ml_routes[1] = 0;
    if (n == 0) return RTK_OK;
    try {
        std::vector<MyersProb> probs(n);
        std::string pool;
        uint32_t max_q = 1, max_t = 1;
        for (uint32_t i = 0; i < n; ++i) {
            probs[i].q_off = pool.size(); pool.append(query[i], qlen[i]);
            probs[i].t_off = pool.size(); pool.append(target[i], tlen[i]);
            probs[i].qlen = qlen[i]; probs[i].tlen = tlen[i]; probs[i].k = k[i]; probs[i].mode = mode[i];
            if (mode[i] == RTK_MODE_HW && want_path) return rtk_fail(RTK_ERR_UNSUPPORTED, "rtk_myers_batch_lanes: HW path alignment is not on the hot path");
            if (mode[i] < 0 || mode[i] > RTK_MODE_HW) return rtk_fail(RTK_ERR_ARG, "rtk_myers_batch_lanes: unknown mode (the test-only modes 3 to 5 are rtk_myers_batch's)");
            max_q = std::max(max_q, qlen[i]); max_t = std::max(max_t, tlen[i]);
        }
        uint64_t tb_cols = 1;
        if (want_path) for (uint32_t i = 0; i < n; ++i) tb_cols = std::max(tb_cols, std::min<uint64_t>(static_cast<uint64_t>((qlen[i] + 63u) >> 6) * tlen[i], RTK_ML_TB_WORDCOLS));
        const uint64_t stride = rtk_ml_scratch_bytes() + (want_path ? static_cast<uint64_t>(RTK_WAVE) * 32ull * tb_cols : 0ull);
        const int grid = static_cast<int>(std::min<uint64_t>((static_cast<uint64_t>(n) + RTK_WAVE - 1) / RTK_WAVE, static_cast<uint64_t>(want_path ? std::min(default_grid(), 512) : default_grid())));
        const uint32_t cap_moves = want_path ? (std::min<uint32_t>(max_q, 64u * RTK_ML_MAXW) + std::min<uint32_t>(max_t, RTK_ML_MAXN) + 8) : 1;
        struct Held { std::vector<void*> v; void* get(uint64_t bytes) { v.push_back(nullptr); v.back() = rtk_dmalloc(bytes); return v.back(); } void release() { for (void* p : v) if (p) rtk_dfree(p); v.clear(); } ~Held() { release(); } } held;
        char* dpool = static_cast<char*>(held.get(pool.size() + 64));
        MyersProb* dprobs = static_cast<MyersProb*>(held.get(sizeof(MyersProb) * n));
        char* dscr = static_cast<char*>(held.get(stride * grid));
        int32_t* ddist = static_cast<int32_t*>(held.get(4ull * n)); int32_t* dnloc = static_cast<int32_t*>(held.get(4ull * n));
        int32_t* dlocs = static_cast<int32_t*>(held.get(4ull * n * cap_locs + 8)); uint32_t* dst = static_cast<uint32_t*>(held.get(4ull * n));
        uint8_t* dmoves = static_cast<uint8_t*>(held.get(static_cast<uint64_t>(n) * cap_moves + 8)); uint32_t* dnm = static_cast<uint32_t*>(held.get(4ull * n));
        rtk_h2d(dpool, pool.data(), pool.size()); rtk_h2d(dprobs, probs.data(), sizeof(MyersProb) * n);
        { RtkTimer tk; const bool timed = rtk_knob_myers_time(); if (timed) tk.start(0);
          rtk_launch(k_myers_batch_lanes, grid, 0, static_cast<const MyersProb*>(dprobs), n, static_cast<const char*>(dpool), want_path, use_iupac, dscr, stride, grid, ddist, dnloc, dlocs, cap_locs, dmoves, dnm, cap_moves, dst);
          if (timed) { tk.stop(0); rtk_dsync(); fprintf(stderr, "[rtk myers time] one lane per problem%s: %u problems, %d waves, kernel %.3f ms\n", want_path ? " (with paths)" : "", n, grid, tk.elapsed()); } }
        rtk_dsync();
        std::vector<uint32_t> st(n), nm(n);
        rtk_d2h(dist, ddist, 4ull * n); rtk_d2h(n_loc, dnloc, 4ull * n); if (cap_locs) rtk_d2h(end_locs, dlocs, 4ull * n * cap_locs); rtk_d2h(st.data(), dst, 4ull * n); rtk_d2h(nm.data(), dnm, 4ull * n);
        int rc = RTK_OK;
        if (want_path && cigar) {
            std::vector<uint8_t> mv(static_cast<size_t>(n) * cap_moves);
            rtk_d2h(mv.data(), dmoves, mv.size());
            static const char code[4] = {'M', 'I', 'D', 'M'};
            for (uint32_t i = 0; i < n && rc == RTK_OK; ++i) {
                if (st[i]) continue;
                std::string c;
                const uint8_t* a = &mv[static_cast<size_t>(i) * cap_moves];
                for (uint32_t x = 0; x < nm[i];) { uint32_t y = x; while (y < nm[i] && code[a[y]] == code[a[x]]) ++y; c += std::to_string(y - x); c.push_back(code[a[x]]); x = y; }
                if (c.size() + 1 > cap_cigar) { rc = rtk_fail(RTK_ERR_ARG, "rtk_myers_batch_lanes: cigar buffer too small"); break; }
                memcpy(cigar + static_cast<size_t>(i) * cap_cigar, c.c_str(), c.size() + 1);
            }
        }
        held.release();
        if (rc != RTK_OK) return rc;
        std::vector<uint32_t> rest; for (uint32_t i = 0; i < n; ++i) if (st[i]) rest.push_back(i);
        g_ml_routes[0] = n - rest.size(); g_ml_routes[1] = rest.size();
        if (rtk_knob_myers_time()) fprintf(stderr, "[rtk myers time] %zu of %u problems handed on to the wave route\n", rest.size(), n);
        if (!rest.empty()) {
            const uint32_t nr = static_cast<uint32_t>(rest.size());
            std::vector<const char*> q2(nr), t2(nr); std::vector<uint32_t> ql2(nr), tl2(nr); std::vector<int32_t> k2(nr), m2(nr), d2(nr), nl2(nr), loc2(static_cast<size_t>(nr) * cap_locs + 1);
            std::vector<char> cg2(want_path && cigar ? static_cast<size_t>(nr) * cap_cigar : 1);
            for (uint32_t x = 0; x < nr; ++x) { const uint32_t i = rest[x]; q2[x] = query[i]; t2[x] = target[i]; ql2[x] = qlen[i]; tl2[x] = tlen[i]; k2[x] = k[i]; m2[x] = mode[i]; }
            rc = rtk_myers_batch(nr, q2.data(), ql2.data(), t2.data(), tl2.data(), k2.data(), m2.data(), want_path, use_iupac, d2.data(), nl2.data(), loc2.data(), cap_locs, want_path && cigar ? cg2.data() : nullptr, cap_cigar);
            if (rc != RTK_OK) return rc;
            for (uint32_t x = 0; x < nr; ++x) { const uint32_t i = rest[x]; dist[i] = d2[x]; n_loc[i] = nl2[x]; for (uint32_t y = 0; y < cap_locs; ++y) end_locs[static_cast<size_t>(i) * cap_locs + y] = loc2[static_cast<size_t>(x) * cap_locs + y];
                if (want_path && cigar) memcpy(cigar + static_cast<size_t>(i) * cap_cigar, &cg2[static_cast<size_t>(x) * cap_cigar], cap_cigar); }
        }
        return RTK_OK;
    } catch (const std::exception& e) { return rtk_fail(RTK_ERR_DEVICE, e.what()); }
}

#include "rtk_pipeline.inc"

struct SetsProb { uint32_t op, na, nb, scalar; uint64_t a_off, b_off, out_off, work_off; uint32_t out_cap, pad; };

RTK_GLOBAL void k_sets_batch(const SetsProb* probs, uint32_t n, const uint32_t* in_pool, uint32_t* out_pool, uint64_t* work_pool, int grid, uint32_t* out_n, uint32_t* result, uint32_t* status) {
    const uint32_t lane = static_cast<uint32_t>(rtk_lane());
    for (uint32_t pi = static_cast<uint32_t>(RTK_BLOCK_ID); pi < n; pi += static_cast<uint32_t>(grid)) {
        const uint32_t op = rtk_u(probs[pi].op), na = rtk_u(probs[pi].na), nb = rtk_u(probs[pi].nb), sc = rtk_u(probs[pi].scalar), cap = rtk_u(probs[pi].out_cap);
        const uint32_t* const a = in_pool + rtk_u(probs[pi].a_off); const uint32_t* const b = in_pool + rtk_u(probs[pi].b_off);
        uint32_t* const out = out_pool + rtk_u(probs[pi].out_off); uint64_t* const work = work_pool + rtk_u(probs[pi].work_off);
        uint32_t* const work32 = reinterpret_cast<uint32_t*>(work);
        uint32_t nout = 0, res = 0, st = RTK_SETS_OK;
        if (op == RTK_SETS_UNION) { nout = res = rtk_u(rtk_set_union(a, na, b, nb, out, work32)); }
        else if (op == RTK_SETS_INTER) { nout = res = rtk_u(rtk_set_inter(a, na, b, nb, out)); }
        else if (op == RTK_SETS_DIFF) { nout = res = rtk_u(rtk_set_diff(a, na, b, nb, out)); }
        else if (op == RTK_SETS_INTER_COUNT) { res = rtk_u(rtk_set_inter_count(a, na, b, nb, sc)); }
        else if (op == RTK_SETS_SORT_PAIRS) {
            uint32_t p = 1; while (p < na) p <<= 1;
            uint64_t* const key = work; uint64_t* const val = work + p;
            for (uint32_t i = lane; i < na; i += RTK_WAVE) { key[i] = static_cast<uint64_t>(a[2u * i]) | (static_cast<uint64_t>(a[2u * i + 1u]) << 32); val[i] = static_cast<uint64_t>(b[2u * i]) | (static_cast<uint64_t>(b[2u * i + 1u]) << 32); }
            rtk_sync();
            rtk_sort_pairs(key, val, na);
            rtk_sync();
            for (uint32_t i = lane; i < na; i += RTK_WAVE) { out[2u * i] = static_cast<uint32_t>(key[i]); out[2u * i + 1u] = static_cast<uint32_t>(key[i] >> 32); out[2u * na + 2u * i] = static_cast<uint32_t>(val[i]); out[2u * na + 2u * i + 1u] = static_cast<uint32_t>(val[i] >> 32); }
            nout = 4u * na;
        }
#ifndef RTK_SIM
        else if (op == RTK_SETS_RADIX_U32) {
            uint32_t* const L = rtk_lds_set_buf();
            const bool wide = na > RTK_CS_MAX_IDS || nb != 0u;
            for (uint32_t i = lane; i < na; i += RTK_WAVE) L[i] = a[i];
            RTK_WG_SYNC();
            if (wide) rtk_radix_sort_u32(L, work32, na, L + RTK_CB_MAX_IDS, sc);
            else rtk_radix_sort_u32(L, L + 2u * RTK_CS_MAX_IDS, na, L + 2u * RTK_CS_MAX_IDS + RTK_CS_MAX_IDS, sc);
            RTK_WG_SYNC();
            for (uint32_t i = lane; i < na; i += RTK_WAVE) out[i] = L[i];
            nout = na;
        }
        else if (op == RTK_SETS_RADIX_PAIRS_U32) {
            uint32_t* const ka = work32; uint32_t* const pa = ka + na; uint32_t* const kb = pa + na; uint32_t* const pb = kb + na;
            for (uint32_t i = lane; i < na; i += RTK_WAVE) { ka[i] = a[i]; pa[i] = b[i]; }
            rtk_sync();
            rtk_radix_sort_pairs_u32(ka, pa, kb, pb, na, sc);
            rtk_sync();
            for (uint32_t i = lane; i < na; i += RTK_WAVE) { out[i] = ka[i]; out[na + i] = pa[i]; }
            nout = 2u * na;
        }
#endif
        else if (op == RTK_SETS_BM_LOWEST
#ifndef RTK_SIM
                 || op == RTK_SETS_BM8_LOWEST
#endif
                 ) {
#ifdef RTK_SIM
            const uint32_t* const uni = a; uint64_t* const scatter = nullptr;
            const RtkBM v = rtk_bm_from_ids(uni, na, scatter, b, nb);
            res = rtk_bm_count(v);
            const RtkBM low = rtk_bm_lowest(v, sc);
            for (uint32_t w = 0; w < 64; ++w) { uint64_t x = low.w[w]; while (x) { const int bt = __builtin_ctzll(x); if (nout < cap) out[nout] = uni[64u * w + static_cast<uint32_t>(bt)]; ++nout; x &= x - 1ull; } }
#else
            uint32_t* const L = rtk_lds_set_buf(); uint64_t* const scatter = reinterpret_cast<uint64_t*>(L + RTK_CB_MAX_IDS + 256u);
            const uint32_t* uni = a;
            if (na <= RTK_CB_MAX_IDS) { for (uint32_t i = lane; i < na; i += RTK_WAVE) L[i] = a[i]; RTK_WG_SYNC(); uni = L; }
            RtkBM v = rtk_bm_from_ids(uni, na, scatter, b, nb);
            RtkBM low;
            if (op == RTK_SETS_BM8_LOWEST) { if (lane >= 8u) v = 0ull; res = rtk_bm8_count(v); low = rtk_bm8_lowest(v, sc); }
            else { res = rtk_bm_count(v); low = rtk_bm_lowest(v, sc); }
            int tot; uint32_t at = static_cast<uint32_t>(rtk_wave_excl_scan(rtk_popc(low), &tot)); uint64_t x = low;
            while (x) { const int bt = __builtin_ctzll(x); if (at < cap) out[at] = uni[64u * lane + static_cast<uint32_t>(bt)]; ++at; x &= x - 1ull; }
            nout = static_cast<uint32_t>(rtk_u(tot));
#endif
        }
        else st = RTK_SETS_NOT_IN_BUILD;
        if (lane == 0u) { out_n[pi] = nout; result[pi] = res; status[pi] = st; }
        rtk_sync();
    }
}

extern "C" int rtk_sets_batch(uint32_t n, const uint32_t* op, const uint32_t* const* a, const uint32_t* na, const uint32_t* const* b, const uint32_t* nb, const uint32_t* scalar,
                              uint32_t* out_pool, const uint64_t* out_off, uint32_t* out_n, uint32_t* result, uint32_t* status) {
    if (!op || !a || !na || !b || !nb || !scalar || !out_pool || !out_off || !out_n || !result || !status) return rtk_fail(RTK_ERR_ARG, "rtk_sets_batch: null argument");
    if (rtk_device_count() <= 0) return rtk_fail(RTK_ERR_NO_DEVICE, "rtk_sets_batch: no HIP device visible (no CPU fallback)");
    if (n == 0) return RTK_OK;
    try {
        std::vector<SetsProb> probs(n);
        std::vector<uint32_t> in_pool;
        uint64_t work_top = 0;
        for (uint32_t i = 0; i < n; ++i) {
            SetsProb& p = probs[i];
            if ((na[i] && !a[i]) || (nb[i] && !b[i]) || out_off[i + 1] < out_off[i] || out_off[i + 1] - out_off[i] > 0xFFFFFFFFull) return rtk_fail(RTK_ERR_ARG, "rtk_sets_batch: null array or bad output slice");
            const uint64_t cap = out_off[i + 1] - out_off[i], A = na[i], B = nb[i];
            uint64_t need = 0, work = 0, wa = A, wb = B;
            switch (op[i]) {
                case RTK_SETS_UNION: need = A + B; work = (B + 1) / 2; break;
                case RTK_SETS_INTER: case RTK_SETS_DIFF: need = A; break;
                case RTK_SETS_INTER_COUNT: break;
                case RTK_SETS_SORT_PAIRS: { if (B != A || A > (1u << 24)) return rtk_fail(RTK_ERR_ARG, "rtk_sets_batch: SORT_PAIRS wants nb == na <= 2^24"); uint64_t pw = 1; while (pw < A) pw <<= 1; need = 4 * A; work = 2 * pw; wa = 2 * A; wb = 2 * B; break; }
                case RTK_SETS_RADIX_U32: if (A > RTK_CB_MAX_IDS) return rtk_fail(RTK_ERR_ARG, "rtk_sets_batch: RADIX_U32 sorts at most 1664 keys"); need = A; work = (A + 1) / 2; wb = 0; break;
                case RTK_SETS_RADIX_PAIRS_U32: if (B != A) return rtk_fail(RTK_ERR_ARG, "rtk_sets_batch: RADIX_PAIRS_U32 wants nb == na"); need = 2 * A; work = 2 * A; break;
                case RTK_SETS_BM_LOWEST: case RTK_SETS_BM8_LOWEST: {
                    if (A > (op[i] == RTK_SETS_BM8_LOWEST ? 512u : 4096u)) return rtk_fail(RTK_ERR_ARG, "rtk_sets_batch: universe too large for the bit vector");
                    for (uint64_t x = 1; x < A; ++x) if (a[i][x - 1] >= a[i][x]) return rtk_fail(RTK_ERR_ARG, "rtk_sets_batch: the universe is not sorted and free of repeats");
                    for (uint64_t x = 0; x < B; ++x) if (!std::binary_search(a[i], a[i] + A, b[i][x]) || (x && b[i][x - 1] >= b[i][x])) return rtk_fail(RTK_ERR_ARG, "rtk_sets_batch: the ids are not a sorted subset of the universe");
                    need = std::min<uint64_t>(scalar[i], B); break; }
                default: return rtk_fail(RTK_ERR_ARG, "rtk_sets_batch: unknown operation");
            }
            if (cap < need) return rtk_fail(RTK_ERR_ARG, "rtk_sets_batch: output slice too small for problem " + std::to_string(i));
            p.op = op[i]; p.na = na[i]; p.nb = nb[i]; p.scalar = scalar[i]; p.out_off = out_off[i]; p.out_cap = static_cast<uint32_t>(cap); p.pad = 0;
            p.a_off = in_pool.size(); in_pool.insert(in_pool.end(), a[i], a[i] + wa);
            p.b_off = in_pool.size(); in_pool.insert(in_pool.end(), b[i], b[i] + wb);
            p.work_off = work_top; work_top += work + 1;
        }
        const uint64_t out_words = out_off[n];
        const int grid = static_cast<int>(std::min<uint32_t>(n, static_cast<uint32_t>(default_grid())));
        struct Held { std::vector<void*> v; void* get(uint64_t bytes) { v.push_back(nullptr); v.back() = rtk_dmalloc(bytes); return v.back(); } void release() { for (void* p : v) if (p) rtk_dfree(p); v.clear(); } ~Held() { release(); } } held;
        SetsProb* dprobs = static_cast<SetsProb*>(held.get(sizeof(SetsProb) * n));
        uint32_t* din = static_cast<uint32_t*>(held.get(4ull * in_pool.size() + 8)); uint32_t* dout = static_cast<uint32_t*>(held.get(4ull * out_words + 8));
        uint64_t* dwork = static_cast<uint64_t*>(held.get(8ull * work_top + 8));
        uint32_t* dn = static_cast<uint32_t*>(held.get(4ull * n)); uint32_t* dres = static_cast<uint32_t*>(held.get(4ull * n)); uint32_t* dst = static_cast<uint32_t*>(held.get(4ull * n));
        rtk_h2d(dprobs, probs.data(), sizeof(SetsProb) * n); rtk_h2d(din, in_pool.data(), 4ull * in_pool.size()); rtk_dzero(dout, 4ull * out_words);
        rtk_launch(k_sets_batch, grid, 0, static_cast<const SetsProb*>(dprobs), n, static_cast<const uint32_t*>(din), dout, dwork, grid, dn, dres, dst);
        rtk_dsync();
        rtk_d2h(out_pool, dout, 4ull * out_words); rtk_d2h(out_n, dn, 4ull * n); rtk_d2h(result, dres, 4ull * n); rtk_d2h(status, dst, 4ull * n);
        return RTK_OK;
    } catch (const std::exception& e) { return rtk_fail(RTK_ERR_DEVICE, e.what()); }
}

#ifdef RTK_SIM
thread_local std::vector<RtkSimPair> rtk_sim_pair_log;
std::atomic<int> rtk_sim_pairs_on(0);
std::atomic<unsigned long long> rtk_sim_pair_stat[32][10];
extern "C" void rtk_sim_pairs(int on) { rtk_sim_pairs_on = on; }
extern "C" void rtk_sim_pair_stats(unsigned long long* out, int reset) { for (int i = 0; i < 32; ++i) for (int j = 0; j < 10; ++j) { out[10 * i + j] = rtk_sim_pair_stat[i][j].load(); if (reset) rtk_sim_pair_stat[i][j] = 0; } }
#endif
```

ratatosk_amd/csrc/hip/rtk_pipeline_run.inc:

```

RTK_GLOBAL void k_enum(const LaunchCtx* L, BatchView bv, int grid) {
#ifdef RTK_SIM
    unsigned char comp_tab[256];
#else
    __shared__ unsigned char comp_tab[256];
#endif
    for (uint32_t c = static_cast<uint32_t>(rtk_lane()); c < 256u; c += RTK_WAVE) comp_tab[c] = static_cast<unsigned char>(rtk_comp(static_cast<char>(c)));
    rtk_sync();
    for (uint32_t ri = static_cast<uint32_t>(RTK_BLOCK_ID); ri < bv.n_reads; ri += static_cast<uint32_t>(grid)) rtk_enum_regions(L->g, L->bv, L->rb, bv.order[ri], comp_tab);
}

RTK_DEV bool rtk_region_is_heavy(const BatchView& bv, const RegionDesc& rd) {
    if (rd.kind == RTK_RG_GAP) { const uint32_t* sp = bv.s_pos + bv.roff[rd.read]; return (sp[rd.i_solid + 1] - sp[rd.i_solid]) >= 160u; }
    return rd.kind == RTK_RG_HEAD || rd.kind == RTK_RG_TAIL;
}
RTK_DEV bool rtk_gap_is_easy(const GraphView& g, const OptsView& o, const BatchView& bv, const RegionDesc& rd, bool* shortcut, UMap* ua_out, uint32_t* len_unitig_km_out, uint32_t* min_pos_out) {
    const uint64_t base = bv.roff[rd.read]; const uint32_t* sp = bv.s_pos + base; const uint32_t k = static_cast<uint32_t>(g.k);
    const uint32_t pa = sp[rd.i_solid], pb = sp[rd.i_solid + 1];
    const UMap ua = rtk_unpack_hit(bv.hits[base + pa]), ub = rtk_unpack_hit(bv.hits[base + pb]);
    *shortcut = false;
    bool same = (ua.unitig == ub.unitig) && (ua.strand == ub.strand);
    if (same && !(g.flags[ua.unitig] & RTK_F_SHORT_CYCLE)) {
        const uint32_t min_pos = ua.dist < ub.dist ? ua.dist : ub.dist, max_pos = ua.dist < ub.dist ? ub.dist : ua.dist;
        const uint32_t len_query_km = pb - pa, len_unitig_km = max_pos - min_pos;
// ... 398 lines not shown
    ~OwnSlab() { if (p) g->phase_give(p, n); }
};
struct RegionRun {
    rtk_batch* b; rtk_graph* g; OptsView ov; rtk_stream_t sm;
    bool trace;
    bool own_slab;
    std::chrono::steady_clock::time_point w0;
    int grid; uint32_t max_len; unsigned long long n_regions, n_ovf_total, out_top;
    bool lane_auto, lanes_on, lanes_beside; int lane_waves_used;
    RtkTimer t_enum, t_easy, t_lanes, t_reg, t_st; double ms_reg;
    SlabHold hold; OwnSlab slab;
    const LaunchCtx* ctx() const { return static_cast<const LaunchCtx*>(b->ctx()); }
    void set_ctx() { rtk_launch(k_set_ctx, 1, sm, b->ctx(), g->dview, ov, b->bv, b->rb); }
    void lap(const char* what) const {
        if (trace) fprintf(stderr, "[rtk trace] regions %-10s +%.2f ms\n", what, std::chrono::duration<double, std::milli>(std::chrono::steady_clock::now() - w0).count());
    }
};

static void region_alloc_lists(rtk_batch* b, uint64_t cap) {
    RegionBatch& rb = b->rb;
    rb.regions_cap = cap;
    rb.regions = b->alloc<RegionDesc>(cap); rb.rorder = b->alloc<uint32_t>(cap); rb.eorder = b->alloc<uint32_t>(cap);
    rb.lorder = b->alloc<uint32_t>(4 * cap); rb.horder = b->alloc<uint32_t>(cap); rb.st_off = b->alloc<uint64_t>(cap);
}

static void region_alloc(RegionRun& R) {
    rtk_batch* b = R.b; RegionBatch& rb = b->rb;
    if (rb.seq_rc) return;
    rb.seq_rc = b->alloc<char>(b->n_bases + 64);
    rb.qual_rev = b->bv.qual.get() ? b->alloc<char>(b->n_bases + 64) : nullptr;
    rb.r_first = b->alloc<uint64_t>(b->n); rb.r_count = b->alloc<uint32_t>(b->n);
    rb.n_regions = b->alloc<unsigned long long>(1); rb.n_heavy = b->alloc<unsigned long long>(16); rb.seg_top = b->alloc<unsigned long long>(1);
    rb.next_region = b->alloc<unsigned long long>(1); rb.n_overflow = b->alloc<unsigned long long>(1); rb.out_top = b->alloc<unsigned long long>(1);
    rb.out_off = b->alloc<uint64_t>(b->n); rb.out_seq_len = b->alloc<uint32_t>(b->n); rb.out_qual_len = b->alloc<uint32_t>(b->n);
    region_alloc_lists(b, std::max<uint64_t>(1024, b->n_bases / 8 + 4ull * b->n));
    rb.next_lane = b->alloc<unsigned long long>(4);
    rb.seg_cap = 6 * b->n_bases + (1ull << 20); rb.seg_pool = b->alloc<char>(rb.seg_cap);
    rb.out_cap = 6 * b->n_bases + (1ull << 20); rb.out_pool = b->alloc<char>(rb.out_cap);
}

static void region_lane_class(RegionRun& R) {
    const uint64_t auto_bases = rtk_knob_lane_auto_bases();
    R.lane_auto = !R.own_slab && !rtk_knob_lane_max_gap_set() && auto_bases != 0 && R.b->n_bases >= auto_bases;
    R.b->rb.lane_max_gap = R.own_slab ? 0u : (R.lane_auto ? 128u : rtk_knob_lane_max_gap());
}

static void region_enumerate(RegionRun& R) {
    rtk_batch* b = R.b; RegionBatch& rb = b->rb; const rtk_stream_t sm = R.sm;
    const int eg = std::min<int>(R.grid, static_cast<int>(b->n) > 0 ? static_cast<int>(b->n) : 1);
    for (int tries = 0; tries < 2; ++tries) {
        rtk_dzero_s(rb.n_regions, 8, sm);
        R.set_ctx();
        R.t_enum.start(sm);
        rtk_launch(k_enum, eg, sm, R.ctx(), b->bv, eg);
        R.t_enum.stop(sm);
        rtk_ssync(sm);
        rtk_d2h_s(&R.n_regions, rb.n_regions, 8, sm);
        if (R.n_regions <= rb.regions_cap) break;
        region_alloc_lists(b, R.n_regions + 1024);
    }
    if (R.n_regions) {
        rtk_dzero_s(rb.n_heavy, 128, sm);
        R.set_ctx();
        const unsigned long long per_wave = RTK_OQ * RTK_WAVE;
        const int og = static_cast<int>(std::min<unsigned long long>(static_cast<unsigned long long>(R.grid), (R.n_regions + per_wave - 1ull) / per_wave));
        rtk_launch(k_region_order, og, sm, R.ctx(), static_cast<uint64_t>(R.n_regions), og);
    }
}

static void region_easy(RegionRun& R) {
    rtk_dzero_s(R.b->rb.seg_top, 8, R.sm); rtk_dzero_s(R.b->rb.out_top, 8, R.sm);
    if (!R.n_regions) return;
    const int eg = static_cast<int>(std::min<unsigned long long>(static_cast<unsigned long long>(2 * R.grid), R.n_regions));
    R.t_easy.start(R.sm);
    rtk_launch(k_regions_easy, eg, R.sm, R.ctx(), eg);
    R.t_easy.stop(R.sm);
}

static void region_lanes(RegionRun& R) {
    rtk_batch* b = R.b; RegionBatch& rb = b->rb; const rtk_stream_t sm = R.sm;
    R.lane_waves_used = 0;
    R.lanes_on = R.n_regions && rb.lane_max_gap;
    R.lanes_beside = R.lanes_on && !R.lane_auto && !rtk_knob_lane_serial();
    if (!R.lanes_on) return;
    R.hold.take(false);
#ifdef RTK_SIM
    const int lgrid = 16;
#else
    const int lgrid = R.lane_auto ? 4096 : rtk_knob_lane_waves();
#endif
    R.lane_waves_used = lgrid;
    const uint64_t a_bytes = rl_area_bytes(), t_bytes = rl_table_bytes();
    char* ls = graph_scratch(R.g, 2, (a_bytes + t_bytes) * static_cast<uint64_t>(lgrid));
    RlLimits lim;
    lim.str = RL_STR_BYTES; lim.um = RL_UM_CAP; lim.list = RL_LIST_CAP; lim.arena0 = RL_A0_W; lim.arena1 = RL_A1_W; lim.arena2 = RL_A2_W; lim.tb = RL_TB_WORDCOLS;
    if (rtk_knob_test_tiny_scratch()) { lim.str = 200; lim.um = 6; lim.list = 3; lim.arena0 = 160; lim.arena1 = 400; lim.arena2 = 400; lim.tb = 400; }
    rtk_dzero_s(rb.next_lane, 32, sm);
    rtk_stream_t sl = sm;
    if (R.lanes_beside) { sl = b->lane_stream(); rtk_event_record(b->ev[0], sm); rtk_stream_wait(sl, b->ev[0]); }
    R.t_lanes.start(sl);
    rtk_launch(k_regions_lanes, lgrid, sl, R.ctx(), reinterpret_cast<uint32_t*>(ls), reinterpret_cast<uint64_t*>(ls + a_bytes * static_cast<uint64_t>(lgrid)),
               static_cast<uint64_t>(R.n_regions), lim, lgrid, rtk_knob_lane_round());
    R.t_lanes.stop(sl);
    if (R.lanes_beside) rtk_event_record(b->ev[1], sl);
}

static void region_take_areas(RegionRun& R) {
    rtk_batch* b = R.b; rtk_graph* g = R.g;
    if (!R.own_slab && R.hold.what < 0) {
        const uint64_t half_max_bases = rtk_knob_half_slab_bases();
        R.hold.take(half_max_bases != 0 && b->n_bases <= half_max_bases && !region_compact());
        if (R.hold.what != 2) {
            const uint64_t st0 = region_scratch_bytes(region_cfg(R.max_len, 0)), half_bytes = (g->scratch_bytes_[1] / 2) & ~255ull;
            if (!g->scratch[1] || half_bytes / st0 < 512) { R.hold.release(); R.hold.take(false); }
        }
    }
    if (b->on_region_slab) { b->on_region_slab(b->on_region_slab_arg); b->on_region_slab = nullptr; }
}

struct RegionGridIn {
    int attempt; bool compact;
    int waves_that_fit;
    bool own_slab; int p2_cap;
    bool lanes_beside; int lane_waves;
    bool on_half; int half_waves; uint64_t half_fit;
    unsigned long long n_regions;
};
static int region_grid(const RegionGridIn& in) {
#ifdef RTK_SIM
    int rgrid = 16;
#else
    const int big = in.attempt - (in.compact ? 1 : 0);
    int rgrid = in.attempt == 0 ? in.waves_that_fit : (big == 0 ? 1024 : (big == 1 ? 256 : 8));
#endif
    if (in.own_slab && in.attempt == 0)
        rgrid = static_cast<int>(std::min<unsigned long long>(static_cast<unsigned long long>(in.p2_cap), std::max<unsigned long long>(128ull, in.n_regions / 4ull)));
    if (in.attempt == 0 && in.lanes_beside) rgrid = std::max(1024, rgrid - in.lane_waves);
    rgrid = static_cast<int>(std::min<unsigned long long>(static_cast<unsigned long long>(rgrid), in.n_regions ? in.n_regions : 1ull));
    if (in.on_half) rgrid = static_cast<int>(std::min<uint64_t>(static_cast<uint64_t>(std::min(rgrid, in.half_waves)), in.half_fit));
    return rgrid;
}

static void region_attempt_trace(RegionRun& R, int attempt, int rgrid, uint64_t stride) {
    const BatchView& bv = R.b->bv; const rtk_stream_t sm = R.sm;
    std::vector<RegionDesc> rds(R.n_regions); rtk_d2h_s(rds.data(), R.b->rb.regions, sizeof(RegionDesc) * R.n_regions, sm);
    unsigned long long hist[16] = {0}; for (size_t i = 0; i < rds.size(); ++i) hist[rds[i].status & 15u]++;
    fprintf(stderr, "[rtk trace] k_regions attempt %d: %.2f ms, %d waves, stride %.2f MB; status codes:", attempt, R.t_reg.elapsed(), rgrid, stride / 1048576.0);
    for (int i = 1; i < 16; ++i) if (hist[i]) fprintf(stderr, " %d:%llu", i, hist[i]);
    fprintf(stderr, "\n");
    unsigned long long tc[RTK_CNT_WAVE_TRACE_END - RTK_CNT_WAVE_TRACE] = {0}; rtk_d2h_s(tc, bv.counters + RTK_CNT_WAVE_TRACE, sizeof(tc), sm);
    const double span = static_cast<double>(tc[2] - ~tc[1]) / 100e6 * 1e3, avg_life = tc[4] ? static_cast<double>(tc[3]) / static_cast<double>(tc[4]) / 100e6 * 1e3 : 0.0;
    fprintf(stderr, "[rtk trace] k_regions waves: first start to last end %.2f ms, average lifetime of a wave %.2f ms (%.0f %% of it), longest single region %.3g cycles "
                    "(taken off the queue at place %llu of %llu), most regions on one wave %llu\n",
            span, avg_life, span > 0 ? 100.0 * avg_life / span : 0.0, static_cast<double>(tc[0]), tc[6], static_cast<unsigned long long>(R.n_regions), tc[7]);
}

static int region_attempts(RegionRun& R) {
    rtk_batch* b = R.b; rtk_graph* g = R.g; RegionBatch& rb = b->rb; const rtk_stream_t sm = R.sm;
    const int n_attempts = region_compact() ? 4 : 3;
    R.ms_reg = 0; R.n_ovf_total = 0;
    for (int attempt = 0; attempt < n_attempts; ++attempt) {
        if (attempt != 0 && !R.own_slab && R.hold.what != 2) { R.hold.release(); R.hold.take(false); }
        const RegionScratchCfg cfg = region_cfg(R.max_len, attempt);
        const uint64_t stride = region_scratch_bytes(cfg);
        if (R.trace) fprintf(stderr, "[rtk trace] region work area: %llu bytes per wave\n", static_cast<unsigned long long>(stride));
        const bool on_half = !R.own_slab && R.hold.what != 2;
        const uint64_t half_bytes = (g->scratch_bytes_[1] / 2) & ~255ull;
        RegionGridIn gi;
        gi.attempt = attempt; gi.compact = region_compact(); gi.n_regions = R.n_regions;
#ifdef RTK_SIM
        gi.waves_that_fit = 0;
#else
        gi.waves_that_fit = attempt == 0 ? region_waves_that_fit(stride, R.own_slab ? 0 : g->scratch_bytes_[1], R.trace) : 0;
#endif
        gi.own_slab = R.own_slab; gi.p2_cap = rtk_knob_p2_rgrid();
        gi.lanes_beside = R.lanes_beside; gi.lane_waves = R.lane_waves_used;
        gi.on_half = on_half; gi.half_waves = on_half ? rtk_knob_half_waves() : 0; gi.half_fit = on_half ? half_bytes / stride : 0;
        const int rgrid = region_grid(gi);
        char* scratch;
        if (R.own_slab) scratch = R.slab.at_least(stride * rgrid);
        else if (!on_half) scratch = graph_scratch(g, 1, stride * rgrid);
        else scratch = static_cast<char*>(g->scratch[1]) + static_cast<uint64_t>(R.hold.what) * half_bytes;
        rtk_dzero_s(rb.next_region, 8, sm); rtk_dzero_s(rb.n_overflow, 8, sm);
        if (attempt != 0) R.set_ctx();
        const int tcls = rtk_knob_trace_class(R.trace ? -2 : -1);
        R.t_reg.start(sm);
        rtk_launch(k_regions, rgrid, sm, R.ctx(), g->dview, R.ov, b->bv, rb, scratch, stride, cfg, static_cast<uint64_t>(R.n_regions), attempt == 0 ? 0 : 1, tcls,
                   attempt == 0 ? (R.lanes_beside ? 5 : 1) : 3);
        if (attempt == 0 && R.lanes_on) {
            if (R.lanes_beside) rtk_stream_wait(sm, b->ev[1]);
            rtk_dzero_s(rb.next_region, 8, sm);
            rtk_launch(k_regions, std::min(rgrid, 1024), sm, R.ctx(), g->dview, R.ov, b->bv, rb, scratch, stride, cfg, static_cast<uint64_t>(R.n_regions), 0, tcls, 2);
        }
        R.t_reg.stop(sm);
        rtk_ssync(sm);
        R.ms_reg += R.t_reg.elapsed();
        if (R.trace) region_attempt_trace(R, attempt, rgrid, stride);
        unsigned long long n_ovf = 0; rtk_d2h_s(&n_ovf, rb.n_overflow, 8, sm);
        if (attempt == 0) R.n_ovf_total = n_ovf;
        unsigned long long seg_top = 0; rtk_d2h_s(&seg_top, rb.seg_top, 8, sm);
        if (seg_top > rb.seg_cap) return rtk_fail(RTK_ERR_DEVICE, "region stage: segment pool exhausted");
        if (n_ovf == 0) return RTK_OK;
    }
    return rtk_fail(RTK_ERR_DEVICE, "region stage: scratch capacity exceeded after " + std::to_string(n_attempts) + " attempts");
}

static int region_stitch(RegionRun& R) {
    rtk_batch* b = R.b; const rtk_stream_t sm = R.sm;
    R.t_st.start(sm);
    const int sg = std::min<int>(R.grid, static_cast<int>(b->n) > 0 ? static_cast<int>(b->n) : 1);
    rtk_launch(k_stitch, sg, sm, R.ctx(), b->bv, sg);
    if (R.n_regions) {
        const int cg = static_cast<int>(std::min<unsigned long long>(static_cast<unsigned long long>(2 * R.grid), (R.n_regions + RTK_WAVE - 1ull) / RTK_WAVE));
        rtk_launch(k_stitch_copy, cg, sm, R.ctx(), static_cast<uint64_t>(R.n_regions), cg);
    }
    R.t_st.stop(sm);
    b->t_all.stop(sm);
    rtk_ssync(sm);
    R.out_top = 0; rtk_d2h_s(&R.out_top, b->rb.out_top, 8, sm);
    if (R.out_top > b->rb.out_cap) return rtk_fail(RTK_ERR_DEVICE, "stitch: output pool exhausted");
    return RTK_OK;
}

static void region_trace_report(const unsigned long long* cnt) {
    const double total = double(cnt[RTK_CNT_CYC_TOTAL] ? cnt[RTK_CNT_CYC_TOTAL] : 1);
    auto share = [&](int slot) { return double(cnt[slot]) / total; };
#ifdef RTK_PROF
    {
        static const char* const pn[RTK_CNT_PROF_END - RTK_CNT_PROF] = {
            "driver: dispatch + anchors", "driver: same-unitig shortcut", "region: prologue", "region: side lists", "region: chooseColors",
            "semiweak: glue", "paths: prologue", "explore: prefix", "dfs: pop + adj", "dfs: nkm + colour_ok", "dfs T: load/extend",
            "dfs T: to_string", "dfs T: NW sweep", "dfs T: commit", "dfs NT: load/extend", "dfs NT: commit/rest", "dfs post: nt scoring",
            "dfs post: load + to_string", "dfs post: path qual", "dfs post: commit", "paths: after explore", "paths: final select",
            "semiweak: merge", "region: restart/select", "region: assemble", "region: fixAmbiguity", "region: corrected? + trim",
            "driver: between fw/bw", "consensus: rc + card", "consensus: fw NW path", "consensus: bw path / checks", "consensus: merge",
            "consensus: final", "driver: emit prep", "dequeue", "emit", 0, 0, 0, 0, "probe: 4 dependent cold loads", "probe: 4 dependent warm loads",
            "probe: slab store + load", 0};
        const unsigned long long* pr = cnt + RTK_CNT_PROF; const int n = RTK_CNT_PROF_END - RTK_CNT_PROF;
        if (pr[43]) fprintf(stderr, "[rtk trace] in-situ probes: cold load %.0f cycles, warm load %.0f cycles, slab store + load %.0f cycles "
                                    "(per round trip, %llu samples)\n",
                            double(pr[40]) / 4.0 / double(pr[43]), double(pr[41]) / 4.0 / double(pr[43]), double(pr[42]) / double(pr[43]), pr[43]);
        unsigned long long tot = 0; for (int i = 0; i < n; ++i) tot += pr[i];
        fprintf(stderr, "[rtk trace] k_regions lap profile (%.3g cycles):", double(tot));
        for (int i = 0; i < n; ++i) if (pr[i] && pn[i]) fprintf(stderr, " [%d %s %.4f]", i, pn[i], double(pr[i]) / double(tot ? tot : 1));
        fprintf(stderr, "\n");
    }
#endif
    {
        static const char* const hn[8] = {"gap<40", "gap<64", "gap<128", "gap<256", "gap<512", "gap<1024", "gap>=1024", "head/tail"};
        const unsigned long long* h = cnt + RTK_CNT_HIST;
        fprintf(stderr, "[rtk trace] k_regions by size class (share of region time, regions, avg kcycles, second-strand share, DFS calls per region):");
        for (int i = 0; i < 8; ++i) {
            const unsigned long long cyc = h[i], n = h[8 + i];
            if (n) fprintf(stderr, " [%s %.3f n=%llu %.0fk bw=%.2f dfs=%.1f]", hn[i], double(cyc) / total, n, 1e-3 * double(cyc) / double(n), double(h[16 + i]) / double(n),
                           double(h[24 + i]) / double(n));
        }
        fprintf(stderr, "\n");
    }
    {
        static const char* const fine_names[RTK_FINE_N] = {
            "colour: class unions", "fixAmbiguity: path alignment", "fixAmbiguity: walk of the moves",
            "fixAmbiguity: linked alleles (k-mer lookups)", "fixAmbiguity: apply", "colour small: bit vectors (or array: shared_with(all))",
            "colour small: classes + selection (or array: set ops)", "region: side lists", "region: trim alignment", "region: fixAmbiguity",
            "consensus: merge logic", "paths: explore_paths outside DFS", "colour: small path (cycles)", "colour: 4096-bit path (cycles)",
            "colour: small path calls / total cycles", "colour: 4096-bit path calls / total cycles"};
        const unsigned long long* f = cnt + RTK_CNT_FINE;
        fprintf(stderr, "[rtk trace] chooseColors calls: small path %llu, 4096-bit path %llu; fixAmbiguity calls %llu, of which left by the all-confident way out %llu\n",
                f[RTK_FINE_COL_S_CALLS], f[RTK_FINE_COL_B_CALLS], f[RTK_FINE_FA_CALLS], f[RTK_FINE_FA_ALL_CONFIDENT]);
        fprintf(stderr, "[rtk trace] k_regions fine shares:");
        for (int i = 0; i < RTK_FINE_N; ++i) if (f[i]) fprintf(stderr, " [%s %.3f]", fine_names[i], double(f[i]) / total);
        fprintf(stderr, "\n");
    }
#ifdef RTK_LANE_PROF
    {
        static const char* const ln[RL_NPROF] = {
            "driver", "side lists", "chooseColors", "search glue", "dfs walk", "colour_ok", "to_string", "peq build", "sweep", "walk",
            "path records", "path qual", "select", "amb collect", "fixAmbiguity", "assemble", "trim", "revcomp", "consensus", "emit",
            "idle at round end", "colours: universe", "colours: rows", 0};
        static_assert(RL_NPROF == RTK_CNT_LANE_PROF2 - RTK_CNT_LANE_PROF, "counter map: the lane profile has RL_NPROF slots");
        const unsigned long long* p1 = cnt + RTK_CNT_LANE_PROF; const unsigned long long* p2 = cnt + RTK_CNT_LANE_PROF2;
        unsigned long long tot = 0; for (int i = 0; i < RL_NPROF; ++i) tot += p1[i];
        fprintf(stderr, "[rtk trace] k_regions_lanes lap profile (%.3g lane cycles):", double(tot));
        for (int i = 0; i < RL_NPROF; ++i) if (p1[i] && ln[i]) fprintf(stderr, " [%s %.4f]", ln[i], double(p1[i]) / double(tot ? tot : 1));
        fprintf(stderr, "\n");
        unsigned long long tw = 0; for (int i = 0; i < RL_NPROF; ++i) tw += p2[i];
        fprintf(stderr, "[rtk trace] k_regions_lanes wave-time estimate by slot (share of %.3g, lanes together):", double(tw) / 64.0);
        for (int i = 0; i < RL_NPROF; ++i)
            if (p2[i] && ln[i]) fprintf(stderr, " [%s %.4f x%.1f]", ln[i], double(p2[i]) / double(tw ? tw : 1), 64.0 * double(p1[i]) / double(p2[i]));
        fprintf(stderr, "\n");
    }
#endif
    fprintf(stderr, "[rtk trace] k_regions shares of %.3g wave cycles: colour %.3f paths %.3f consensus %.3f myers %.3f sets %.3f tostring %.3f pathqual %.3f "
                    "walk %.3f\n",
            double(cnt[RTK_CNT_CYC_TOTAL]), share(RTK_CNT_CYC_COLOUR), share(RTK_CNT_CYC_PATHS), share(RTK_CNT_CYC_CONSENSUS), share(RTK_CNT_CYC_MYERS),
            share(RTK_CNT_CYC_SETS),
            share(RTK_CNT_CYC_TOSTRING), share(RTK_CNT_CYC_PATHQUAL), share(RTK_CNT_WALK_CYCLES));
    fprintf(stderr, "[rtk trace] k_regions cycle shares: DFS bookkeeping %.3f (of which colour checks %.3f)\n", share(RTK_CNT_CYC_DFS), share(RTK_CNT_CYC_COLOUR_OK));
    fprintf(stderr, "[rtk trace] trims: by column %llu (of which stored %llu), by the distance call %llu, cycles %.3g; consensus calls: forward alignment resumed %llu, swept %llu\n",
            cnt[RTK_CNT_ROUTES + 0] + cnt[RTK_CNT_ROUTES + 1], cnt[RTK_CNT_ROUTES + 0], cnt[RTK_CNT_ROUTES + 2], double(cnt[RTK_CNT_FINE + RTK_FINE_TRIM]), cnt[RTK_CNT_ROUTES + 3], cnt[RTK_CNT_ROUTES + 4]);
    fprintf(stderr, "[rtk trace] fixAmbiguity linked-allele searches: run %llu, skipped %llu, entries produced %llu, cycles %.3g\n", cnt[RTK_CNT_FA_LINKED + 0], cnt[RTK_CNT_FA_LINKED + 1],
            cnt[RTK_CNT_FA_LINKED + 2], double(cnt[RTK_CNT_FINE + RTK_FINE_FA_LINKED]));
    fprintf(stderr, "[rtk trace] second strand of gap regions: run %llu, skipped %llu (the forward result decides), audit mismatches %llu\n", cnt[RTK_CNT_STRAND2 + 0], cnt[RTK_CNT_STRAND2 + 1], cnt[RTK_CNT_STRAND2 + 2]);
    fprintf(stderr, "[rtk trace] stored sweeps of the forward trims: walked for a consensus %llu, never walked %llu\n", cnt[RTK_CNT_PARK + 0], cnt[RTK_CNT_PARK + 1]);
    fprintf(stderr, "[rtk trace] colour selections answered by: small %llu, wide %llu, bits %llu, general %llu; audit mismatches %llu\n", cnt[RTK_CNT_COLOURS + 0], cnt[RTK_CNT_COLOURS + 1], cnt[RTK_CNT_COLOURS + 2],
            cnt[RTK_CNT_COLOURS + 3], cnt[RTK_CNT_COLOURS + 4]);
    fprintf(stderr, "[rtk trace] walks %llu moves %llu reloads %llu scalar steps %llu cycles %.3g tail cycles %.3g\n", cnt[RTK_CNT_WALK_CALLS], cnt[RTK_CNT_WALK_MOVES],
            cnt[RTK_CNT_WALK_RELOADS], cnt[RTK_CNT_WALK_SCALAR], double(cnt[RTK_CNT_WALK_CYCLES]), double(cnt[RTK_CNT_WALK_TAIL]));
}

static void region_stats(RegionRun& R, const unsigned long long* cnt) {
    rtk_batch* b = R.b; rtk_stats& st = b->stats;
    st.cyc_colour = cnt[RTK_CNT_CYC_COLOUR]; st.cyc_paths = cnt[RTK_CNT_CYC_PATHS]; st.cyc_consensus = cnt[RTK_CNT_CYC_CONSENSUS]; st.cyc_total = cnt[RTK_CNT_CYC_TOTAL];
    st.cyc_myers = cnt[RTK_CNT_CYC_MYERS]; st.cyc_sets = cnt[RTK_CNT_CYC_SETS]; st.cyc_tostring = cnt[RTK_CNT_CYC_TOSTRING]; st.cyc_pathqual = cnt[RTK_CNT_CYC_PATHQUAL];
    st.cyc_walk = cnt[RTK_CNT_WALK_CYCLES]; st.n_moves = cnt[RTK_CNT_WALK_MOVES];
    st.n_slots_exact = cnt[RTK_CNT_SLOTS_EXACT]; st.n_slots_inexact = cnt[RTK_CNT_SLOTS_INEXACT];
    st.ms_regions = R.t_enum.elapsed() + (R.n_regions ? R.t_easy.elapsed() : 0.0);
    st.ms_lanes = R.lanes_on ? R.t_lanes.elapsed() : 0.0;
    st.ms_correct = R.ms_reg + ((R.lanes_on && !R.lanes_beside) ? st.ms_lanes : 0.0);
    st.n_lane_handed = cnt[RTK_CNT_LANE_HANDED]; st.n_lane_regions = cnt[RTK_CNT_LANE_HANDED] + cnt[RTK_CNT_LANE_DONE];
    st.n_trim_stored = cnt[RTK_CNT_ROUTES + 0]; st.n_trim_column = cnt[RTK_CNT_ROUTES + 1]; st.n_trim_fallback = cnt[RTK_CNT_ROUTES + 2];
    st.n_consensus_resumed = cnt[RTK_CNT_ROUTES + 3]; st.n_consensus_swept = cnt[RTK_CNT_ROUTES + 4];
    st.n_fa_linked_run = cnt[RTK_CNT_FA_LINKED + 0]; st.n_fa_linked_skipped = cnt[RTK_CNT_FA_LINKED + 1]; st.n_fa_linked_entries = cnt[RTK_CNT_FA_LINKED + 2];
    st.n_strand2_run = cnt[RTK_CNT_STRAND2 + 0]; st.n_strand2_skipped = cnt[RTK_CNT_STRAND2 + 1]; st.n_strand2_audit_mismatch = cnt[RTK_CNT_STRAND2 + 2];
    st.n_park_walked = cnt[RTK_CNT_PARK + 0]; st.n_park_deferred = cnt[RTK_CNT_PARK + 1];
    st.n_colours_small = cnt[RTK_CNT_COLOURS + 0]; st.n_colours_wide = cnt[RTK_CNT_COLOURS + 1]; st.n_colours_bits = cnt[RTK_CNT_COLOURS + 2]; st.n_colours_general = cnt[RTK_CNT_COLOURS + 3];
    st.n_colours_audit_mismatch = cnt[RTK_CNT_COLOURS + 4];
    st.ms_stitch = R.t_st.elapsed(); st.ms_total = b->t_all.elapsed();
    st.n_windows = b->n_bases;
    st.n_probes_exact = cnt[RTK_CNT_PROBES_EXACT]; st.n_probes_inexact = cnt[RTK_CNT_PROBES_INEXACT]; st.n_hits_inexact = cnt[RTK_CNT_HITS_INEXACT];
    st.n_regions = R.n_regions; st.n_region_items = R.n_regions; st.n_arena_overflow = R.n_ovf_total;
    st.n_expand = cnt[RTK_CNT_EXPAND]; st.n_colour_elem = cnt[RTK_CNT_COLOUR]; st.n_path_base = cnt[RTK_CNT_PATHBASE];
    st.n_align = cnt[RTK_CNT_ALIGN]; st.n_align_cells = cnt[RTK_CNT_CELLS];
    st.in_bases = b->n_bases; st.out_bases = R.out_top / 2;
}

extern "C" int rtk_batch_run_regions(rtk_batch* b, const rtk_opts* opts) {
    int rc = batch_precheck(b, opts, "rtk_batch_run_regions");
    if (rc) return rc;
    if (!b->seeded) return rtk_fail(RTK_ERR_ARG, "rtk_batch_run_regions: rtk_batch_run_seeds has not completed for this batch");
    if (opts->long_read_correct && !b->bv.qual.get())
        return rtk_fail(RTK_ERR_ARG, "rtk_batch_run_regions: the second pass (long_read_correct) needs a batch created with quality strings");
    rtk_graph* g = b->g;
    try {
        rtk_set_device(g->device);
        RegionRun R = {};
        R.b = b; R.g = g; R.ov = opts_view(opts); R.sm = b->stream; R.own_slab = opts->long_read_correct != 0;
        R.hold.g = g; R.hold.what = -1; R.slab.g = g;
        R.trace = rtk_knob_trace(); R.w0 = std::chrono::steady_clock::now();
        for (uint32_t i = 0; i < b->n; ++i) R.max_len = std::max<uint32_t>(R.max_len, static_cast<uint32_t>(b->roff[i + 1] - b->roff[i]));
        R.grid = default_grid();
        region_alloc(R);
        region_lane_class(R);
        R.lap("alloc");
        region_enumerate(R);
        R.lap("enum");
        region_easy(R);
        region_lanes(R);
        region_take_areas(R);
        rc = region_attempts(R);
        if (rc) return rc;
        R.hold.release();
        R.lap("regions");
        rc = region_stitch(R);
        if (rc) return rc;
        unsigned long long cnt[RTK_CNT_TOTAL]; rtk_d2h_s(cnt, b->bv.counters, sizeof(cnt), R.sm);
        if (R.trace) region_trace_report(cnt);
        region_stats(R, cnt);
        R.lap("done");
        if (b->h_out) { g->stage_give(b->h_out, b->h_out_bytes); b->h_out = nullptr; }
        b->ran = true; b->seeded = false;
    } catch (const std::exception& e) { return rtk_fail(RTK_ERR_DEVICE, e.what()); }
    return RTK_OK;
}

extern "C" int rtk_batch_run(rtk_batch* b, const rtk_opts* opts) {
    const int rc = rtk_batch_run_seeds(b, opts);
    return rc ? rc : rtk_batch_run_regions(b, opts);
}

static int batch_fetch_host(rtk_batch* b) {
    if (b->h_out) return RTK_OK;
    rtk_set_device(b->g->device);
    const auto tf0 = std::chrono::steady_clock::now();
    unsigned long long out_top = 0; rtk_d2h_s(&out_top, b->rb.out_top, 8, b->stream);
    const auto tf1 = std::chrono::steady_clock::now();
    b->h_out = b->g->stage_take(out_top + 8, &b->h_out_bytes);
    const auto tf2 = std::chrono::steady_clock::now();
    b->h_off.resize(b->n); b->h_sl.resize(b->n); b->h_ql.resize(b->n);
    if (out_top) rtk_check_async_d2h(b->h_out, b->rb.out_pool, out_top, b->stream);
    rtk_d2h_s(b->h_off.data(), b->rb.out_off, 8ull * b->n, b->stream); rtk_d2h_s(b->h_sl.data(), b->rb.out_seq_len, 4ull * b->n, b->stream); rtk_d2h_s(b->h_ql.data(), b->rb.out_qual_len, 4ull * b->n, b->stream);
    if (rtk_knob_trace()) { auto ms = [](std::chrono::steady_clock::time_point a, std::chrono::steady_clock::time_point b_) { return std::chrono::duration<double, std::milli>(b_ - a).count(); }; fprintf(stderr, "[rtk trace] fetch: wait for the stream %.2f ms, staging buffer %.2f ms, %.1f MB to the host %.2f ms\n", ms(tf0, tf1), ms(tf1, tf2), out_top / 1048576.0, ms(tf2, std::chrono::steady_clock::now())); }
    for (uint32_t i = 0; i < b->n; ++i) {
        const char* bad = nullptr;
        if (b->h_sl[i] != b->h_ql[i]) bad = "rtk_batch_fetch: sequence and quality lengths differ for a read";
        else if (b->h_off[i] + 2ull * b->h_sl[i] > out_top) bad = "rtk_batch_fetch: record outside the output pool";
        if (bad) { rtk_ssync(b->stream); b->g->stage_give(b->h_out, b->h_out_bytes); b->h_out = nullptr; return rtk_fail(RTK_ERR_DEVICE, bad); }
    }
    return RTK_OK;
}

extern "C" int rtk_batch_fetch_view(rtk_batch* b, const char** pool, const uint64_t** off, const uint32_t** len) {
    if (!b || !pool || !off || !len) return rtk_fail(RTK_ERR_ARG, "rtk_batch_fetch_view: null argument");
    if (!b->ran) return rtk_fail(RTK_ERR_ARG, "rtk_batch_fetch_view: rtk_batch_run has not completed");
    try { const int rc = batch_fetch_host(b); if (rc) return rc; }
    catch (const std::exception& e) { return rtk_fail(RTK_ERR_DEVICE, e.what()); }
    *pool = static_cast<const char*>(b->h_out); *off = b->h_off.data(); *len = b->h_sl.data();
    return RTK_OK;
}

extern "C" int rtk_batch_fetch(rtk_batch* b, char** out_seq, char** out_qual, uint32_t* out_len) {
    if (!b || !out_seq || !out_qual || !out_len) return rtk_fail(RTK_ERR_ARG, "rtk_batch_fetch: null argument");
    if (!b->ran) return rtk_fail(RTK_ERR_ARG, "rtk_batch_fetch: rtk_batch_run has not completed");
    try {
        const int rc = batch_fetch_host(b); if (rc) return rc;
        const char* pool = static_cast<const char*>(b->h_out);
        for (uint32_t i = 0; i < b->n; ++i) { out_seq[i] = nullptr; out_qual[i] = nullptr; }
        std::atomic<bool> oom(false);
        auto copy_range = [&](uint32_t lo, uint32_t hi) {
            for (uint32_t i = lo; i < hi && !oom.load(std::memory_order_relaxed); ++i) {
                const uint32_t sl = b->h_sl[i];
                out_seq[i] = static_cast<char*>(malloc(sl + 1)); out_qual[i] = static_cast<char*>(malloc(sl + 1));
                if (!out_seq[i] || !out_qual[i]) { oom.store(true); return; }
                memcpy(out_seq[i], pool + b->h_off[i], sl); out_seq[i][sl] = 0;
                memcpy(out_qual[i], pool + b->h_off[i] + sl, sl); out_qual[i][sl] = 0;
                out_len[i] = sl;
            }
        };
        {
            const uint32_t n_thr = (b->n_bases >= (4u << 20) && b->n >= 8) ? 4u : 1u;
            std::vector<uint32_t> cut(n_thr + 1, b->n); cut[0] = 0;
            for (uint32_t t = 1, i = 0; t < n_thr; ++t) { const uint64_t want = b->n_bases / n_thr * t; while (i < b->n && b->roff[i] < want) ++i; cut[t] = i; }
            std::vector<std::thread> thr;
            for (uint32_t t = 1; t < n_thr; ++t) thr.emplace_back(copy_range, cut[t], cut[t + 1]);
            copy_range(cut[0], cut[1]);
            for (size_t t = 0; t < thr.size(); ++t) thr[t].join();
        }
        if (oom.load()) { for (uint32_t j = 0; j < b->n; ++j) { free(out_seq[j]); free(out_qual[j]); out_seq[j] = nullptr; out_qual[j] = nullptr; } return rtk_fail(RTK_ERR_DEVICE, "rtk_batch_fetch: out of host memory"); }
    } catch (const std::exception& e) { return rtk_fail(RTK_ERR_DEVICE, e.what()); }
    return RTK_OK;
}

extern "C" int rtk_batch_get_stats(const rtk_batch* b, rtk_stats* stats) { if (!b || !stats) return rtk_fail(RTK_ERR_ARG, "rtk_batch_get_stats: null"); *stats = b->stats; return RTK_OK; }

struct CoGroup { rtk_batch* b = nullptr; const char* pool = nullptr; const uint64_t* off = nullptr; const uint32_t* len = nullptr; std::atomic<int> left{0}; };
struct CoTicket {
    const rtk_opts* opts; uint32_t n; const char* const* seq; const char* const* qual; const uint32_t* len; uint64_t bases;
    bool taken = false, done = false, alone_after_all = false; int rc = 0; std::string err; CoGroup* grp = nullptr; uint32_t first = 0;
};
static bool co_compatible(const CoTicket& a, const CoTicket& b) { return (a.qual == nullptr) == (b.qual == nullptr) && memcmp(a.opts, b.opts, sizeof(rtk_opts)) == 0; }

extern "C" int rtk_coalesce_stats(rtk_graph* g, uint64_t* n_groups, uint64_t* n_tickets) {
    if (!g || !n_groups || !n_tickets) return rtk_fail(RTK_ERR_ARG, "rtk_coalesce_stats: null argument");
    std::lock_guard<std::mutex> lk(g->co_m); *n_groups = g->co_groups; *n_tickets = g->co_tickets; return RTK_OK;
}

static int correct_batch_alone(rtk_graph* g, const rtk_opts* opts, uint32_t n, const char* const* seq, const char* const* qual, const uint32_t* len, char** out_seq, char** out_qual, uint32_t* out_len) {
    rtk_batch* b = nullptr;
    const bool trace = rtk_knob_trace();
    const auto t0 = std::chrono::steady_clock::now();
    auto ms = [&](std::chrono::steady_clock::time_point a) { return std::chrono::duration<double, std::milli>(std::chrono::steady_clock::now() - a).count(); };
    int rc = rtk_batch_create(g, n, seq, qual, len, &b);
    if (rc) return rc;
    const double t_create = ms(t0); const auto t1 = std::chrono::steady_clock::now();
    rc = rtk_batch_run(b, opts);
    const double t_run = ms(t1); const auto t2 = std::chrono::steady_clock::now();
    if (rc == RTK_OK) rc = rtk_batch_fetch(b, out_seq, out_qual, out_len);
    const double t_fetch = ms(t2); const auto t3 = std::chrono::steady_clock::now();
    rtk_batch_free(b);
    if (trace) fprintf(stderr, "[rtk trace] correct_batch: create %.1f ms, run %.1f ms, fetch %.1f ms, free %.1f ms\n", t_create, t_run, t_fetch, ms(t3));
    return rc;
}

extern "C" int rtk_correct_batch(rtk_graph* g, const rtk_opts* opts, uint32_t n, const char* const* seq, const char* const* qual, const uint32_t* len,
                                 char** out_seq, char** out_qual, uint32_t* out_len) {
    if (!g || !opts || (n && (!seq || !len || !out_seq || !out_qual || !out_len))) return rtk_fail(RTK_ERR_ARG, "rtk_correct_batch: null argument");
    if (!opts_ok(opts)) return rtk_fail(RTK_ERR_ARG, "rtk_correct_batch: rtk_opts was not filled by this library's rtk_opts_default (struct_size does not match: older header, or a zero-filled struct)");
    if (!g->on_device) return rtk_fail(RTK_ERR_NO_DEVICE, "rtk_correct_batch: graph is not resident on a device (call rtk_graph_upload); there is no CPU fallback");
    if (n == 0) return RTK_OK;
    uint64_t bases = 0; for (uint32_t i = 0; i < n; ++i) bases += len[i];
    const uint64_t cap = rtk_knob_coalesce_bases();
    if (cap == 0 || bases >= cap || opts->long_read_correct) return correct_batch_alone(g, opts, n, seq, qual, len, out_seq, out_qual, out_len);

    CoTicket me; me.opts = opts; me.n = n; me.seq = seq; me.qual = qual; me.len = len; me.bases = bases;
    std::unique_lock<std::mutex> lk(g->co_m);
    g->co_q.push_back(&me);
    g->co_cv.notify_all();
    while (!me.done) {
        if (me.taken || g->co_gathering) { g->co_cv.wait(lk); continue; }
        g->co_gathering = true;
        const bool alone = g->co_q.size() == 1 && g->co_running == 0 && g->co_last_group <= 1;
        const auto deadline = std::chrono::steady_clock::now() + std::chrono::microseconds(alone ? 0L : rtk_knob_coalesce_wait_us());
        const bool cold = g->co_running == 0;
        while (true) {
            uint64_t sum = 0; for (size_t i = 0; i < g->co_q.size(); ++i) if (co_compatible(*g->co_q[i], me)) sum += g->co_q[i]->bases;
            if (sum >= cap) break;
            const bool late = std::chrono::steady_clock::now() >= deadline;
            if (late && (g->co_running == 0 || (g->co_pre_region == 0 && g->co_running < 3))) break;
            if (late) g->co_cv.wait(lk); else g->co_cv.wait_until(lk, deadline);
        }
        uint64_t take_cap = cap; uint32_t take_n = 0xFFFFFFFFu;
        { uint32_t nw = 0; for (size_t i = 0; i < g->co_q.size(); ++i) if (co_compatible(*g->co_q[i], me)) ++nw;
          const uint32_t split = rtk_knob_coalesce_split();
          const uint32_t around = nw + g->co_inflight_tickets; if (around >= 2 * split) take_n = (around + split - 1) / split; }
        (void)cold;
        std::vector<CoTicket*> grp; uint64_t sum = 0;
        for (size_t i = 0; i < g->co_q.size();) {
            CoTicket* t = g->co_q[i];
            if (((sum < take_cap && grp.size() < take_n) || t == &me) && co_compatible(*t, me)) { t->taken = true; sum += t->bases; grp.push_back(t); g->co_q.erase(g->co_q.begin() + static_cast<long>(i)); } else ++i;
        }
        g->co_gathering = false; g->co_running += 1; g->co_pre_region += 1; g->co_last_group = static_cast<uint32_t>(grp.size()); g->co_inflight_tickets += static_cast<uint32_t>(grp.size()); g->co_groups += 1; g->co_tickets += grp.size();
        g->co_cv.notify_all();
        lk.unlock();
        int rc = RTK_OK; std::string err; CoGroup* cg = new CoGroup();
        struct Pace { rtk_graph* g; bool in_regions; } pace = {g, false};
        auto enter_regions_fn = [](void* p_) { Pace* p = static_cast<Pace*>(p_); if (!p->in_regions) { p->in_regions = true; std::lock_guard<std::mutex> l2(p->g->co_m); p->g->co_pre_region -= 1; p->g->co_cv.notify_all(); } };
        auto enter_regions = [&]() { enter_regions_fn(&pace); };
        if (grp.size() == 1) {
            delete cg; cg = nullptr;
            rtk_batch* b1 = nullptr;
            rc = rtk_batch_create(g, n, seq, qual, len, &b1);
            if (rc == RTK_OK) { b1->on_region_slab = enter_regions_fn; b1->on_region_slab_arg = &pace; rc = rtk_batch_run_seeds(b1, opts); }
            if (rc == RTK_OK) rc = rtk_batch_run_regions(b1, opts);
            enter_regions();
            if (rc == RTK_OK) rc = rtk_batch_fetch(b1, out_seq, out_qual, out_len);
            if (rc) err = rtk_last_error();
            if (b1) rtk_batch_free(b1);
        } else {
            uint32_t tot = 0; for (size_t i = 0; i < grp.size(); ++i) { grp[i]->first = tot; tot += grp[i]->n; }
            std::vector<const char*> sa(tot), qa(qual ? tot : 0); std::vector<uint32_t> la(tot);
            for (size_t i = 0; i < grp.size(); ++i) for (uint32_t j = 0; j < grp[i]->n; ++j) { sa[grp[i]->first + j] = grp[i]->seq[j]; la[grp[i]->first + j] = grp[i]->len[j]; if (qual) qa[grp[i]->first + j] = grp[i]->qual[j]; }
            const bool tr_ = rtk_knob_trace(); static const auto t_epoch = std::chrono::steady_clock::now();
            auto now_ms = [&]() { return std::chrono::duration<double, std::milli>(std::chrono::steady_clock::now() - t_epoch).count(); };
            const double tq0 = now_ms();
            rc = rtk_batch_create(g, tot, sa.data(), qual ? qa.data() : nullptr, la.data(), &cg->b);
            const double tq1 = now_ms();
            if (rc == RTK_OK) { cg->b->on_region_slab = enter_regions_fn; cg->b->on_region_slab_arg = &pace; rc = rtk_batch_run_seeds(cg->b, opts); }
            const double tq2 = now_ms();
            if (rc == RTK_OK) rc = rtk_batch_run_regions(cg->b, opts);
            enter_regions();
            const double tq3 = now_ms();
            if (rc == RTK_OK) rc = rtk_batch_fetch_view(cg->b, &cg->pool, &cg->off, &cg->len);
            if (tr_) fprintf(stderr, "[rtk trace] correct_batch group at %.1f ms: %zu tickets, %u reads, %.2f Mb; create %.2f seeds %.2f (kernels %.2f) regions %.2f (k_regions %.2f) fetch %.2f ms (rc %d)\n", tq0, grp.size(), tot, sum / 1e6, tq1 - tq0, tq2 - tq1,
                            cg->b ? cg->b->stats.ms_lookup_exact + cg->b->stats.ms_mask + cg->b->stats.ms_lookup_inexact + cg->b->stats.ms_seeds : 0.0, tq3 - tq2, cg->b ? cg->b->stats.ms_correct : 0.0, now_ms() - tq3, rc);
            if (rc == RTK_OK && rtk_knob_test_coalesce_fail()) rc = rtk_fail(RTK_ERR_DEVICE, "test hook: the merged batch is reported as failed");
            if (rc) { err = rtk_last_error(); if (cg->b) rtk_batch_free(cg->b); delete cg; cg = nullptr; }
            else cg->left.store(static_cast<int>(grp.size()));
        }
        enter_regions();
        lk.lock();
        g->co_running -= 1; g->co_inflight_tickets -= static_cast<uint32_t>(grp.size());
        const bool redo = rc != RTK_OK && grp.size() > 1;
        for (size_t i = 0; i < grp.size(); ++i) { grp[i]->rc = redo ? RTK_OK : rc; grp[i]->err = err; grp[i]->grp = cg; grp[i]->alone_after_all = redo; grp[i]->done = true; }
        g->co_cv.notify_all();
    }
    lk.unlock();
    if (me.rc) return rtk_fail(me.rc, me.err);
    if (me.alone_after_all) return correct_batch_alone(g, opts, n, seq, qual, len, out_seq, out_qual, out_len);
    if (!me.grp) return RTK_OK;
    CoGroup* cg = me.grp; int rc = RTK_OK;
    for (uint32_t i = 0; i < n; ++i) { out_seq[i] = nullptr; out_qual[i] = nullptr; }
    for (uint32_t i = 0; i < n && rc == RTK_OK; ++i) {
        const uint32_t r = me.first + i, sl = cg->len[r];
        out_seq[i] = static_cast<char*>(malloc(sl + 1)); out_qual[i] = static_cast<char*>(malloc(sl + 1));
        if (!out_seq[i] || !out_qual[i]) { for (uint32_t j = 0; j <= i; ++j) { free(out_seq[j]); free(out_qual[j]); out_seq[j] = nullptr; out_qual[j] = nullptr; } rc = rtk_fail(RTK_ERR_DEVICE, "rtk_correct_batch: out of host memory"); break; }
        memcpy(out_seq[i], cg->pool + cg->off[r], sl); out_seq[i][sl] = 0;
        memcpy(out_qual[i], cg->pool + cg->off[r] + sl, sl); out_qual[i][sl] = 0;
        out_len[i] = sl;
    }
    if (cg->left.fetch_sub(1) == 1) { rtk_batch_free(cg->b); delete cg; }
    return rc;
}

extern "C" int rtk_reserve_second_pass(int device, uint32_t n_tickets, uint64_t phase_bytes, uint64_t region_bytes) {
#ifdef RTK_SIM
    (void)device; (void)n_tickets; (void)phase_bytes; (void)region_bytes; return RTK_OK;
#endif
    try {
        rtk_set_device(device);
        {
            static std::vector<int> seeded; bool first = false;
            { std::lock_guard<std::mutex> lk(g_reserved_lock); if (std::find(seeded.begin(), seeded.end(), device) == seeded.end()) { seeded.push_back(device); first = true; } }
            if (first) {
                SeedScratchCfg sc; sc.set_cap = 32768u; sc.v_cap = 32768u; sc.s_cap = 131072u + 64;
                ReservedSlab r; r.device = device; r.bytes = seed_scratch_bytes(sc) * static_cast<uint64_t>(seed_waves()); r.p = rtk_dmalloc(r.bytes);
                std::lock_guard<std::mutex> lk(g_reserved_lock); g_reserved.push_back(r);
            }
        }
        for (uint32_t t = 0; t < n_tickets; ++t) for (int i = 0; i < 2; ++i) {
            const uint64_t want = i == 0 ? phase_bytes : region_bytes;
            if (!want) continue;
#ifndef RTK_SIM
            size_t fr = 0, tot = 0; if (hipMemGetInfo(&fr, &tot) != hipSuccess) break;
            if (static_cast<uint64_t>(fr) < want + (static_cast<uint64_t>(tot) / 4)) return rtk_fail(RTK_ERR_DEVICE, "rtk_reserve_second_pass: not reserved (less than a quarter of the device memory would stay free)");
#endif
            ReservedSlab r; r.device = device; r.bytes = want; r.p = rtk_dmalloc(want);
            std::lock_guard<std::mutex> lk(g_reserved_lock); g_reserved.push_back(r);
        }
    } catch (const std::exception& e) { return rtk_fail(RTK_ERR_DEVICE, std::string("rtk_reserve_second_pass: ") + e.what()); }
    return RTK_OK;
}

extern "C" int rtk_reserve_scratch(int device, uint32_t max_read_len) {
    try {
        rtk_set_device(device);
        SeedScratchCfg sc; sc.set_cap = 32768u; sc.v_cap = 32768u; { uint32_t q = 131072u; while (q < max_read_len) q <<= 1; sc.s_cap = q + 64; }
#ifdef RTK_SIM
        const uint64_t n_seed_waves = 16, reg_waves = 16;
#else
        const uint64_t n_seed_waves = static_cast<uint64_t>(seed_waves()), reg_waves = static_cast<uint64_t>(rtk_knob_region_waves());
#endif
#ifdef RTK_SIM
        uint64_t reg_bytes = region_scratch_bytes(region_cfg(max_read_len, 0)) * reg_waves;
#else
        (void)reg_waves;
        uint64_t reg_bytes = region_scratch_bytes(region_cfg(max_read_len, 0)) * static_cast<uint64_t>(region_waves_that_fit(region_scratch_bytes(region_cfg(max_read_len, 0)), 0, rtk_knob_trace()));
#endif
#ifndef RTK_SIM
        if (region_compact()) reg_bytes = std::max<uint64_t>(reg_bytes, region_scratch_bytes(region_cfg(max_read_len, 1)) * 1024ull);
#endif
        const uint64_t want[2] = { seed_scratch_bytes(sc) * n_seed_waves, reg_bytes };
        for (int i = 0; i < 2; ++i) {
            ReservedSlab r; r.device = device; r.bytes = want[i]; r.p = rtk_dmalloc(want[i]);
            std::lock_guard<std::mutex> lk(g_reserved_lock);
            g_reserved.push_back(r);
        }
    } catch (const std::exception& e) { return rtk_fail(RTK_ERR_DEVICE, std::string("rtk_reserve_scratch: ") + e.what()); }
    return RTK_OK;
}
```

ratatosk_amd/csrc/hip/rtk_types.h:

```cpp
#ifndef RTK_TYPES_H
#define RTK_TYPES_H

#include <stdint.h>

#if defined(__HIPCC__) && !defined(RTK_SIM)
#include <hip/hip_runtime.h>
#define RTK_HD __host__ __device__ __forceinline__
#else
#define RTK_HD inline
#endif

#if defined(__HIP_DEVICE_COMPILE__) && !defined(RTK_SIM)
template <class T> __device__ __forceinline__ T rtk_u(T v) {
    static_assert(sizeof(T) <= 8, "rtk_u: scalar types only");
    if (sizeof(T) <= 4) {
        uint32_t x = 0; __builtin_memcpy(&x, &v, sizeof(T));
        x = static_cast<uint32_t>(__builtin_amdgcn_readfirstlane(static_cast<int>(x)));
        T r; __builtin_memcpy(&r, &x, sizeof(T)); return r;
    } else {
        uint64_t x = 0; __builtin_memcpy(&x, &v, sizeof(T));
        const uint32_t lo = static_cast<uint32_t>(__builtin_amdgcn_readfirstlane(static_cast<int>(x & 0xFFFFFFFFull)));
        const uint32_t hi = static_cast<uint32_t>(__builtin_amdgcn_readfirstlane(static_cast<int>(x >> 32)));
        x = (static_cast<uint64_t>(hi) << 32) | lo;
        T r; __builtin_memcpy(&r, &x, sizeof(T)); return r;
    }
}
#else
template <class T> RTK_HD T rtk_u(T v) { return v; }
#endif

#if defined(__HIP_DEVICE_COMPILE__) && !defined(RTK_SIM) && !defined(RTK_NO_GLOBAL_PTRS)
template <class T> __device__ __forceinline__ T rtk_gp(T v) { return v; }
template <class T> __device__ __forceinline__ T* rtk_gp(T* p) { return (T*)(__attribute__((address_space(1))) T*)(unsigned long long)(p); }
#ifndef RTK_NO_CONST_PTRS
template <class T> __device__ __forceinline__ const T* rtk_gp(const T* p) { return (const T*)(__attribute__((address_space(4))) const T*)(unsigned long long)(p); }
#endif
#else
template <class T> RTK_HD T rtk_gp(T v) { return v; }
#endif

template <class T> struct U {
    T v;
    RTK_HD operator T() const { return rtk_gp(rtk_u(v)); }
    RTK_HD T get() const { return rtk_gp(rtk_u(v)); }
    RTK_HD U& operator=(T x) { v = x; return *this; }
    template <class X> RTK_HD U& operator+=(X x) { v = static_cast<T>(rtk_u(v) + x); return *this; }
    template <class X> RTK_HD U& operator-=(X x) { v = static_cast<T>(rtk_u(v) - x); return *this; }
    template <class X> RTK_HD U& operator*=(X x) { v = static_cast<T>(rtk_u(v) * x); return *this; }
    template <class X> RTK_HD U& operator|=(X x) { v = static_cast<T>(rtk_u(v) | x); return *this; }
    RTK_HD U& operator++() { v = rtk_u(v) + 1; return *this; }
    RTK_HD U& operator--() { v = rtk_u(v) - 1; return *this; }
    RTK_HD T operator++(int) { const T o = rtk_u(v); v = o + 1; return o; }
    RTK_HD T operator--(int) { const T o = rtk_u(v); v = o - 1; return o; }
    RTK_HD T operator->() const { return rtk_gp(rtk_u(v)); }
    RTK_HD decltype(auto) operator*() const { return *rtk_gp(rtk_u(v)); }
    template <class I> RTK_HD decltype(auto) operator[](I i) const { return rtk_gp(rtk_u(v))[i]; }
};
template <class T> struct UL {
    T v;
    RTK_HD operator T() const { return rtk_u(v); }
    RTK_HD T get() const { return rtk_u(v); }
    RTK_HD UL& operator=(T x) { v = x; return *this; }
    RTK_HD T operator->() const { return rtk_u(v); }
    RTK_HD decltype(auto) operator*() const { return *rtk_u(v); }
};

#define RTK_NONE32 0xFFFFFFFFu
#define RTK_EMPTY_KEY 0xFFFFFFFFFFFFFFFFull

#define RTK_F_EDGE_MASK 0xFFu
#define RTK_F_SHORT_CYCLE (1u << 8)
#define RTK_F_BRANCHING (1u << 9)
#define RTK_F_AMBIGUITY (1u << 10)

struct GraphView {
    U<int32_t> k;
    U<uint32_t> n_unitigs;
    U<uint64_t> n_kmers;
    U<uint64_t> ht_slots;
    U<const uint64_t*> useq;
    U<const uint64_t*> uoff;
    U<const uint32_t*> adj;
    U<const uint32_t*> flags;
    U<const uint32_t*> kcov;
    U<const uint32_t*> card;
    U<const uint64_t*> loff;
    U<const int32_t*> gid;
    U<const uint64_t*> goff;
    U<const uint32_t*> col;
    U<const uint64_t*> ht;
    U<const uint64_t*> bf;
    U<uint64_t> bf_mask;
    U<const uint64_t*> bf1;
    U<uint64_t> bf1_mask;
    U<const uint64_t*> cycoff;
    U<const char*> cyc;
    U<const uint64_t*> amb;
    U<const uint64_t*> hap;
    U<uint64_t> n_amb;
    U<const uint64_t*> hx;
    U<uint64_t> hx_mask;
    U<const uint64_t*> hxl;
};

RTK_HD uint32_t rtk_ulen(const GraphView& g, uint32_t u) { return static_cast<uint32_t>(g.uoff[u + 1] - g.uoff[u]); }
RTK_HD uint32_t rtk_nkm(const GraphView& g, uint32_t u) { return rtk_ulen(g, u) - static_cast<uint32_t>(g.k) + 1u; }
RTK_HD uint32_t rtk_base(const GraphView& g, uint64_t pos) { return static_cast<uint32_t>((g.useq[pos >> 5] >> (2 * (pos & 31))) & 3ull); }

RTK_HD uint64_t rtk_hash64(uint64_t x) {
    x ^= x >> 33; x *= 0xff51afd7ed558ccdull;
    x ^= x >> 33; x *= 0xc4ceb9fe1a85ec53ull;
    x ^= x >> 33;
    return x;
}

RTK_HD uint64_t rtk_revcomp(uint64_t x, int k) {
    x = ~x;
    x = ((x >> 2) & 0x3333333333333333ull) | ((x & 0x3333333333333333ull) << 2);
    x = ((x >> 4) & 0x0F0F0F0F0F0F0F0Full) | ((x & 0x0F0F0F0F0F0F0F0Full) << 4);
    x = ((x >> 8) & 0x00FF00FF00FF00FFull) | ((x & 0x00FF00FF00FF00FFull) << 8);
    x = ((x >> 16) & 0x0000FFFF0000FFFFull) | ((x & 0x0000FFFF0000FFFFull) << 16);
    x = (x >> 32) | (x << 32);
    return x >> (64 - 2 * k);
}

enum RtkCounterSlot {
    RTK_CNT_WINDOWS = 0, RTK_CNT_PROBES_EXACT = 1, RTK_CNT_PROBES_INEXACT = 2, RTK_CNT_HITS_INEXACT = 3, RTK_CNT_REGIONS = 4, RTK_CNT_ITEMS = 5,
    RTK_CNT_OVERFLOW = 6,
    RTK_CNT_EXPAND = 7, RTK_CNT_COLOUR = 8, RTK_CNT_PATHBASE = 9, RTK_CNT_ALIGN = 10, RTK_CNT_CELLS = 11,
    RTK_CNT_SLOTS_EXACT = 12, RTK_CNT_SLOTS_INEXACT = 13,
    RTK_CNT_EVENTS_END = 14,
    RTK_CNT_SEED_READBACK = 16,
    RTK_CNT_CYC = 16,
    RTK_CNT_CYC_COLOUR = 16, RTK_CNT_CYC_PATHS = 17, RTK_CNT_CYC_CONSENSUS = 18, RTK_CNT_CYC_TOTAL = 19, RTK_CNT_CYC_MYERS = 20, RTK_CNT_CYC_SETS = 21, RTK_CNT_CYC_TOSTRING = 22, RTK_CNT_CYC_PATHQUAL = 23,
    RTK_CNT_CYC_END = 24,
    RTK_CNT_FINALIZE = 24,
    RTK_CNT_FINALIZE_SLOWEST = 31,
    RTK_CNT_FINALIZE_END = 32,
    RTK_CNT_WALK = 32,
    RTK_CNT_WALK_CYCLES = 32, RTK_CNT_WALK_MOVES = 33, RTK_CNT_WALK_RELOADS = 34, RTK_CNT_WALK_SCALAR = 35, RTK_CNT_WALK_CALLS = 36, RTK_CNT_WALK_TAIL = 37,
    RTK_CNT_CYC_DFS = 38, RTK_CNT_CYC_COLOUR_OK = 39,
    RTK_CNT_WALK_END = 40,
    RTK_CNT_FINE = 40,
    RTK_CNT_FINE_END = 56,
    RTK_CNT_HIST = 56,
    RTK_CNT_HIST_END = 88,
    RTK_CNT_PHASE_TRACE = 59,
    RTK_CNT_PHASE_TRACE_END = 64,
    RTK_CNT_FINALIZE_SLOWEST_PHASES = 72,
    RTK_CNT_FINALIZE_SLOWEST_PHASES_END = 79,
    RTK_CNT_PROF = 96,
    RTK_CNT_PROF_END = 144,
    RTK_CNT_WAVE_TRACE = 144,
    RTK_CNT_WAVE_TRACE_END = 152,
    RTK_CNT_LANE_HANDED = 152, RTK_CNT_LANE_DONE = 153,
    RTK_CNT_LANE_END = 154,
    RTK_CNT_ROUTES = 154,
    RTK_CNT_ROUTES_END = 159,
    RTK_CNT_LANE_PROF = 160,
    RTK_CNT_LANE_PROF2 = 184,
    RTK_CNT_LANE_PROF_END = 208,
    RTK_CNT_PHASE_SKIPPED = 210,
    RTK_CNT_FA_LINKED = 211,
    RTK_CNT_FA_LINKED_END = 214,
    RTK_CNT_STRAND2 = 214,
    RTK_CNT_STRAND2_END = 217,
    RTK_CNT_PARK = 217,
    RTK_CNT_PARK_END = 219,
    RTK_CNT_COLOURS = 219,
    RTK_CNT_COLOURS_END = 224,
    RTK_CNT_USED_END = RTK_CNT_COLOURS_END,
    RTK_CNT_TOTAL = (RTK_CNT_USED_END + 31) / 32 * 32
};
static_assert(RTK_CNT_TOTAL == 224, "counter map: the size of the block changed (it is part of what the kernels and the host agree on)");
constexpr bool rtk_cnt_apart(int a, int a_end, int b, int b_end) { return a_end <= b || b_end <= a; }
static_assert(RTK_CNT_EVENTS_END <= RTK_CNT_CYC && RTK_CNT_CYC_END <= RTK_CNT_FINALIZE && RTK_CNT_FINALIZE_END <= RTK_CNT_WALK && RTK_CNT_WALK_END <= RTK_CNT_FINE, "counter map: the event, cycle, finalize and walk ranges overlap");
static_assert(RTK_CNT_FINE_END <= RTK_CNT_HIST && RTK_CNT_HIST_END <= RTK_CNT_PROF && RTK_CNT_PROF_END <= RTK_CNT_WAVE_TRACE && RTK_CNT_WAVE_TRACE_END <= RTK_CNT_LANE_HANDED, "counter map: the trace ranges overlap");
static_assert(RTK_CNT_LANE_END <= RTK_CNT_ROUTES && RTK_CNT_ROUTES_END <= RTK_CNT_LANE_PROF, "counter map: the route counters overlap the lane ranges");
static_assert(RTK_CNT_LANE_END <= RTK_CNT_LANE_PROF && RTK_CNT_LANE_PROF2 - RTK_CNT_LANE_PROF == 24 && RTK_CNT_LANE_PROF_END <= RTK_CNT_PHASE_SKIPPED && RTK_CNT_PHASE_SKIPPED < RTK_CNT_TOTAL, "counter map: the lane ranges overlap");
static_assert(RTK_CNT_PHASE_SKIPPED < RTK_CNT_FA_LINKED && RTK_CNT_FA_LINKED_END <= RTK_CNT_TOTAL, "counter map: the fixAmbiguity counters overlap the phasing slot or leave the block");
static_assert(RTK_CNT_FA_LINKED_END <= RTK_CNT_STRAND2 && RTK_CNT_STRAND2_END <= RTK_CNT_TOTAL, "counter map: the second-strand counters overlap the fixAmbiguity counters or leave the block");
static_assert(RTK_CNT_STRAND2_END <= RTK_CNT_PARK && RTK_CNT_PARK_END <= RTK_CNT_TOTAL, "counter map: the park counters overlap the second-strand counters or leave the block");
static_assert(RTK_CNT_PARK_END <= RTK_CNT_COLOURS && RTK_CNT_COLOURS_END <= RTK_CNT_TOTAL, "counter map: the colour-route counters overlap the park counters or leave the block");
static_assert(rtk_cnt_apart(RTK_CNT_PHASE_TRACE, RTK_CNT_PHASE_TRACE_END, RTK_CNT_FINALIZE_SLOWEST_PHASES, RTK_CNT_FINALIZE_SLOWEST_PHASES_END), "counter map: the two guests of the size-class table overlap");
static_assert(RTK_CNT_HIST <= RTK_CNT_PHASE_TRACE && RTK_CNT_FINALIZE_SLOWEST_PHASES_END <= RTK_CNT_HIST_END, "counter map: the guests of the size-class table left it (update the comment above)");

enum RtkRegionCnt { RTK_RC_EXPAND = 0, RTK_RC_COLOUR = 1, RTK_RC_PATHBASE = 2, RTK_RC_ALIGN = 3, RTK_RC_CELLS = 4,
    RTK_RC_CYC_COLOUR = 5, RTK_RC_CYC_PATHS = 6, RTK_RC_CYC_CONSENSUS = 7, RTK_RC_CYC_TOTAL = 8, RTK_RC_CYC_MYERS = 9, RTK_RC_CYC_SETS = 10,
    RTK_RC_CYC_PATHREC = 11 , RTK_RC_CYC_TOSTRING = 12, RTK_RC_CYC_PATHQUAL = 13, RTK_RC_CYC_DFS = 14, RTK_RC_CYC_COLOUR_OK = 15,
    RTK_RC_TRIM_STORED = 16, RTK_RC_TRIM_COLUMN = 17, RTK_RC_TRIM_FALLBACK = 18, RTK_RC_CONS_RESUMED = 19, RTK_RC_CONS_SWEPT = 20,
    RTK_RC_FA_LINKED_RUN = 21, RTK_RC_FA_LINKED_SKIPPED = 22, RTK_RC_FA_LINKED_ENTRIES = 23,
    RTK_RC_STRAND2_RUN = 24, RTK_RC_STRAND2_SKIPPED = 25, RTK_RC_STRAND2_AUDIT_MISMATCH = 26,
    RTK_RC_PARK_WALKED = 27, RTK_RC_PARK_DEFERRED = 28,
    RTK_RC_COLOURS_SMALL = 29, RTK_RC_COLOURS_WIDE = 30, RTK_RC_COLOURS_BITS = 31, RTK_RC_COLOURS_GENERAL = 32, RTK_RC_COLOURS_AUDIT_MISMATCH = 33, RTK_RC_N = 34 };
static_assert(RTK_CNT_ROUTES_END - RTK_CNT_ROUTES == static_cast<int>(RTK_RC_FA_LINKED_RUN) - static_cast<int>(RTK_RC_TRIM_STORED), "counter map: one slot per route counter");
static_assert(RTK_CNT_FA_LINKED_END - RTK_CNT_FA_LINKED == static_cast<int>(RTK_RC_STRAND2_RUN) - static_cast<int>(RTK_RC_FA_LINKED_RUN), "counter map: one slot per fixAmbiguity counter");
static_assert(RTK_CNT_STRAND2_END - RTK_CNT_STRAND2 == static_cast<int>(RTK_RC_PARK_WALKED) - static_cast<int>(RTK_RC_STRAND2_RUN), "counter map: one slot per second-strand counter");
static_assert(RTK_CNT_PARK_END - RTK_CNT_PARK == static_cast<int>(RTK_RC_COLOURS_SMALL) - static_cast<int>(RTK_RC_PARK_WALKED), "counter map: one slot per park counter");
static_assert(RTK_CNT_COLOURS_END - RTK_CNT_COLOURS == static_cast<int>(RTK_RC_N) - static_cast<int>(RTK_RC_COLOURS_SMALL), "counter map: one slot per colour-route counter");
#define RTK_CM_ROUTE 3u
#define RTK_CM_ROUTE_BITS 1u
#define RTK_CM_ROUTE_GENERAL 2u
#define RTK_CM_AUDIT 4u
#define RTK_CM_FAULT 8u
enum RtkRegionFine { RTK_FINE_COL_GENERAL = 0 , RTK_FINE_COL_UNIONS = 0, RTK_FINE_FA_ALIGN = 1, RTK_FINE_FA_WALK = 2, RTK_FINE_FA_LINKED = 3, RTK_FINE_FA_APPLY = 4, RTK_FINE_COL_S_VECTORS = 5, RTK_FINE_COL_S_SELECT = 6,
    RTK_FINE_SIDE_LISTS = 7, RTK_FINE_TRIM = 8, RTK_FINE_FIX_AMBIGUITY = 9, RTK_FINE_FA_CALLS = 10, RTK_FINE_FA_ALL_CONFIDENT = 11, RTK_FINE_COL_S_CYCLES = 12, RTK_FINE_COL_B_CYCLES = 13,
    RTK_FINE_COL_S_CALLS = 14, RTK_FINE_COL_B_CALLS = 15, RTK_FINE_N = 16 };

struct UMap {
    uint32_t unitig;
    uint32_t dist;
    uint32_t len;
    uint32_t strand;
};

RTK_HD UMap rtk_um_empty() { UMap u; u.unitig = RTK_NONE32; u.dist = 0; u.len = 0; u.strand = 1; return u; }
RTK_HD bool rtk_um_is_empty(const UMap& u) { return u.unitig == RTK_NONE32; }
RTK_HD bool rtk_um_eq(const UMap& a, const UMap& b) { return a.unitig == b.unitig && a.dist == b.dist && a.len == b.len && a.strand == b.strand; }

#define RTK_NO_HIT 0xFFFFFFFFFFFFFFFFull
RTK_HD uint64_t rtk_pack_hit(uint32_t unitig, uint32_t dist, uint32_t strand) { return (static_cast<uint64_t>(unitig) << 33) | (static_cast<uint64_t>(dist) << 1) | (strand & 1u); }
RTK_HD UMap rtk_unpack_hit(uint64_t h) { UMap u; u.unitig = static_cast<uint32_t>(h >> 33); u.dist = static_cast<uint32_t>((h >> 1) & 0xFFFFFFFFull); u.len = 1; u.strand = static_cast<uint32_t>(h & 1ull); return u; }

RTK_HD uint64_t rtk_ht_slot(uint64_t hh, uint64_t slots) {
#if defined(__HIP_DEVICE_COMPILE__) && !defined(RTK_SIM)
    return __umul64hi(hh, slots);
#else
    return static_cast<uint64_t>((static_cast<unsigned __int128>(hh) * static_cast<unsigned __int128>(slots)) >> 64);
#endif
}
RTK_HD uint64_t rtk_ht_next(uint64_t i, uint64_t slots) { return i + 1 == slots ? 0 : i + 1; }

RTK_HD uint64_t rtk_find_kmer(const GraphView& g, uint64_t fw, uint32_t* n_probes) {
    const uint64_t rc = rtk_revcomp(fw, g.k);
    const uint64_t can = fw < rc ? fw : rc;
    const uint64_t hh = rtk_hash64(can);
    {
        const uint64_t b1 = (hh >> 12) & g.bf1_mask;
        if (!((g.bf1[b1 >> 6] >> (b1 & 63ull)) & 1ull)) { if (n_probes) *n_probes = 0; return RTK_NO_HIT; }
    }
    {
        const uint64_t bits = (1ull << (hh & 63)) | (1ull << ((hh >> 6) & 63));
        if ((g.bf[(hh >> 32) & g.bf_mask] & bits) != bits) { if (n_probes) *n_probes = 0; return RTK_NO_HIT; }
    }
    uint64_t i = rtk_ht_slot(hh, g.ht_slots);
    uint32_t np = 0;
    while (true) {
        const uint64_t key = g.ht[2 * i];
        ++np;
        if (key == can) {
            const uint64_t v = g.ht[2 * i + 1];
            const uint32_t stored_is_can = static_cast<uint32_t>(v & 1ull), query_is_can = (fw <= rc) ? 1u : 0u;
            if (n_probes) *n_probes = np;
            return rtk_pack_hit(static_cast<uint32_t>(v >> 32), static_cast<uint32_t>((v & 0xFFFFFFFFull) >> 1), stored_is_can == query_is_can ? 1u : 0u);
        }
        if (key == RTK_EMPTY_KEY) { if (n_probes) *n_probes = np; return RTK_NO_HIT; }
        i = rtk_ht_next(i, g.ht_slots);
    }
}


struct RtkKm { uint64_t hi, lo; };
RTK_HD RtkKm rtk_km_zero() { RtkKm x; x.hi = 0; x.lo = 0; return x; }
RTK_HD bool rtk_km_eq(const RtkKm& a, const RtkKm& b) { return a.hi == b.hi && a.lo == b.lo; }
RTK_HD bool rtk_km_less(const RtkKm& a, const RtkKm& b) { return a.hi != b.hi ? a.hi < b.hi : a.lo < b.lo; }
RTK_HD RtkKm rtk_km_mask(int k) { RtkKm m; m.lo = (k >= 32) ? ~0ull : ((1ull << (2 * k)) - 1ull); m.hi = (k <= 32) ? 0ull : ((1ull << (2 * k - 64)) - 1ull); return m; }
RTK_HD RtkKm rtk_km_push(const RtkKm& x, uint64_t b, int k) {
    const RtkKm m = rtk_km_mask(k); RtkKm r; r.hi = ((x.hi << 2) | (x.lo >> 62)) & m.hi; r.lo = ((x.lo << 2) | b) & m.lo; return r;
}
RTK_HD RtkKm rtk_km_revcomp(const RtkKm& x, int k) {
    if (k <= 32) { RtkKm r; r.hi = 0; r.lo = rtk_revcomp(x.lo, k); return r; }
    const uint64_t a = rtk_revcomp(x.lo, 32), b = rtk_revcomp(x.hi, 32);
    const int s = 128 - 2 * k;
    RtkKm r; r.lo = (b >> s) | (a << (64 - s)); r.hi = a >> s; return r;
}
RTK_HD uint64_t rtk_km_hash(const RtkKm& can) { return rtk_hash64(can.lo ^ rtk_hash64(can.hi ^ 0x9e3779b97f4a7c15ull)); }
RTK_HD uint64_t rtk_km_fingerprint(const RtkKm& can) { const uint64_t f = rtk_hash64(can.lo + 0x9e3779b97f4a7c15ull) ^ rtk_hash64(can.hi ^ 0xd6e8feb86659fd93ull); return f == RTK_EMPTY_KEY ? 0ull : f; }
RTK_HD RtkKm rtk_km_rc_of_unitig(const GraphView& g, uint64_t pos, int k) {
    const uint64_t w = pos >> 5; const int sh = static_cast<int>(2 * (pos & 31));
    const uint64_t x0 = g.useq[w], x1 = g.useq[w + 1];
    RtkKm l;
    if (sh == 0) { l.lo = x0; l.hi = x1; }
    else { l.lo = (x0 >> sh) | (x1 << (64 - sh)); l.hi = x1 >> sh; if (sh + 2 * k > 128) l.hi |= g.useq[w + 2] << (64 - sh); }
    const RtkKm m = rtk_km_mask(k);
    l.lo = ~l.lo & m.lo; l.hi = ~l.hi & m.hi;
    return l;
}
RTK_HD uint64_t rtk_find_kmer_wide(const GraphView& g, const RtkKm& fw, uint32_t* n_probes) {
    const RtkKm rc = rtk_km_revcomp(fw, g.k);
    const RtkKm can = rtk_km_less(fw, rc) ? fw : rc;
    const uint64_t hh = rtk_km_hash(can);
    { const uint64_t b1 = (hh >> 12) & g.bf1_mask; if (!((g.bf1[b1 >> 6] >> (b1 & 63ull)) & 1ull)) { if (n_probes) *n_probes = 0; return RTK_NO_HIT; } }
    { const uint64_t bits = (1ull << (hh & 63)) | (1ull << ((hh >> 6) & 63)); if ((g.bf[(hh >> 32) & g.bf_mask] & bits) != bits) { if (n_probes) *n_probes = 0; return RTK_NO_HIT; } }
    const uint64_t fp = rtk_km_fingerprint(can);
    uint64_t i = rtk_ht_slot(hh, g.ht_slots);
    uint32_t np = 0;
    while (true) {
        const uint64_t key = g.ht[2 * i];
        ++np;
        if (key == fp) {
            const uint64_t v = g.ht[2 * i + 1];
            const uint32_t u = static_cast<uint32_t>(v >> 32), off = static_cast<uint32_t>((v & 0xFFFFFFFFull) >> 1);
            const RtkKm urc = rtk_km_rc_of_unitig(g, g.uoff[u] + off, g.k);
            if (rtk_km_eq(urc, rc)) { if (n_probes) *n_probes = np; return rtk_pack_hit(u, off, 1u); }
            if (rtk_km_eq(urc, fw)) { if (n_probes) *n_probes = np; return rtk_pack_hit(u, off, 0u); }
        }
        if (key == RTK_EMPTY_KEY) { if (n_probes) *n_probes = np; return RTK_NO_HIT; }
        i = rtk_ht_next(i, g.ht_slots);
    }
}
RTK_HD uint64_t rtk_find_km(const GraphView& g, const RtkKm& fw, uint32_t* n_probes) { return g.k <= 31 ? rtk_find_kmer(g, fw.lo, n_probes) : rtk_find_kmer_wide(g, fw, n_probes); }

RTK_HD void rtk_kmer_prepare(uint64_t fw, int k, uint64_t* can, uint64_t* hh, uint32_t* query_is_can) {
    const uint64_t rc = rtk_revcomp(fw, k);
    *can = fw < rc ? fw : rc; *query_is_can = (fw <= rc) ? 1u : 0u; *hh = rtk_hash64(*can);
}
RTK_HD bool rtk_filter1_pass(uint64_t word1, uint64_t hh, uint64_t bf1_mask) { const uint64_t b1 = (hh >> 12) & bf1_mask; return (word1 >> (b1 & 63ull)) & 1ull; }
RTK_HD bool rtk_filter_pass(uint64_t word, uint64_t hh) { const uint64_t bits = (1ull << (hh & 63)) | (1ull << ((hh >> 6) & 63)); return (word & bits) == bits; }
RTK_HD uint64_t rtk_table_probe_from(const GraphView& g, uint64_t can, uint64_t i, uint32_t query_is_can, uint32_t* n_slots);
RTK_HD uint64_t rtk_table_lookup(const GraphView& g, uint64_t can, uint64_t hh, uint32_t query_is_can, uint32_t* n_slots) { return rtk_table_probe_from(g, can, rtk_ht_slot(hh, g.ht_slots), query_is_can, n_slots); }
RTK_HD uint64_t rtk_table_probe_from(const GraphView& g, uint64_t can, uint64_t i, uint32_t query_is_can, uint32_t* n_slots) {
    uint32_t np = 0;
    while (true) {
        const uint64_t key = g.ht[2 * i]; ++np;
        if (key == can) { const uint64_t v = g.ht[2 * i + 1]; *n_slots = np; return rtk_pack_hit(static_cast<uint32_t>(v >> 32), static_cast<uint32_t>((v & 0xFFFFFFFFull) >> 1), (static_cast<uint32_t>(v & 1ull) == query_is_can) ? 1u : 0u); }
        if (key == RTK_EMPTY_KEY) { *n_slots = np; return RTK_NO_HIT; }
        i = rtk_ht_next(i, g.ht_slots);
    }
}

#endif
```

Baseline: 2.145 billion.

## Build colour universe with tagged radix sort, dropping binary search pass

The colour selection now packs each id with its slot/side tag (or carries tags in a side array) and radix-sorts once with fused digit histograms. The sorted run then yields both the deduplicated universe and the per-slot bit vectors, replacing the second gather and per-element binary search. Vectors are sized to the actual universe (VW from U) and placed in LDS when they fit, so the 8-word and 64-word bitmap routines are chosen by size. A new decline path hands oversized cases to the general route, and a counter records it; the counter block grows from 224 to 256 slots.

```diff
diff --git a/include/ratatosk_hip.h b/include/ratatosk_hip.h
--- a/include/ratatosk_hip.h
+++ b/include/ratatosk_hip.h
@@ -62,6 +62,7 @@
     uint64_t n_strand2_run, n_strand2_skipped, n_strand2_audit_mismatch;
     uint64_t n_park_walked, n_park_deferred;
     uint64_t n_colours_small, n_colours_wide, n_colours_bits, n_colours_general, n_colours_audit_mismatch;
+    uint64_t n_colours_declined_fit;
 } rtk_stats;
 
 int rtk_graph_load(const char* unitig_fasta_gz, const char* rtsk, int k, int n_threads, rtk_graph** out);
@@ -157,8 +158,11 @@
 #define RTK_SETS_RADIX_PAIRS_U32 6
 #define RTK_SETS_BM_LOWEST 7
 #define RTK_SETS_BM8_LOWEST 8
+#define RTK_SETS_RADIX_TAGGED 9
+#define RTK_SETS_COLOUR_UNIVERSE 10
 #define RTK_SETS_OK 0
 #define RTK_SETS_NOT_IN_BUILD 1
+#define RTK_SETS_DECLINED 2
 int rtk_sets_batch(uint32_t n, const uint32_t* op, const uint32_t* const* a, const uint32_t* na, const uint32_t* const* b, const uint32_t* nb, const uint32_t* scalar,
                    uint32_t* out_pool, const uint64_t* out_off, uint32_t* out_n, uint32_t* result, uint32_t* status);
 
diff --git a/ratatosk_amd/api.py b/ratatosk_amd/api.py
--- a/ratatosk_amd/api.py
+++ b/ratatosk_amd/api.py
@@ -33,7 +33,7 @@
                                          "n_fa_linked_run", "n_fa_linked_skipped", "n_fa_linked_entries",
                                          "n_strand2_run", "n_strand2_skipped", "n_strand2_audit_mismatch",
                                          "n_park_walked", "n_park_deferred",
-                                         "n_colours_small", "n_colours_wide", "n_colours_bits", "n_colours_general", "n_colours_audit_mismatch")]
+                                         "n_colours_small", "n_colours_wide", "n_colours_bits", "n_colours_general", "n_colours_audit_mismatch", "n_colours_declined_fit")]
 
     def as_dict(self):
         return {n: getattr(self, n) for n, _ in self._fields_}
@@ -353,8 +353,8 @@
     return a.value, b.value
 
 
-SETS_UNION, SETS_INTER, SETS_DIFF, SETS_INTER_COUNT, SETS_SORT_PAIRS, SETS_RADIX_U32, SETS_RADIX_PAIRS_U32, SETS_BM_LOWEST, SETS_BM8_LOWEST = range(9)
-SETS_OK, SETS_NOT_IN_BUILD = 0, 1
+SETS_UNION, SETS_INTER, SETS_DIFF, SETS_INTER_COUNT, SETS_SORT_PAIRS, SETS_RADIX_U32, SETS_RADIX_PAIRS_U32, SETS_BM_LOWEST, SETS_BM8_LOWEST, SETS_RADIX_TAGGED, SETS_COLOUR_UNIVERSE = range(11)
+SETS_OK, SETS_NOT_IN_BUILD, SETS_DECLINED = 0, 1, 2
 
 
 def sets_batch(problems, lib_path=None):
@@ -377,7 +377,8 @@
         ops[i], na[i], nb[i], sc[i] = op, count_a, count_b, scalar
         pa[i] = a.ctypes.data_as(C.POINTER(C.c_uint32)); pb[i] = b.ctypes.data_as(C.POINTER(C.c_uint32))
         need = {SETS_UNION: count_a + count_b, SETS_INTER: count_a, SETS_DIFF: count_a, SETS_INTER_COUNT: 0, SETS_SORT_PAIRS: 4 * count_a, SETS_RADIX_U32: count_a,
-                SETS_RADIX_PAIRS_U32: 2 * count_a, SETS_BM_LOWEST: min(scalar, count_b), SETS_BM8_LOWEST: min(scalar, count_b)}.get(op, 0)
+                SETS_RADIX_PAIRS_U32: 2 * count_a, SETS_BM_LOWEST: min(scalar, count_b), SETS_BM8_LOWEST: min(scalar, count_b),
+                SETS_RADIX_TAGGED: 2 * count_a, SETS_COLOUR_UNIVERSE: 2 + count_a + 2 * count_b * max(1, (count_a + 63) // 64)}.get(op, 0)
         off.append(off[-1] + need)
     out = np.zeros(max(1, off[-1]), dtype=np.uint32)
     offs = (C.c_uint64 * (n + 1))(*off)
diff --git a/ratatosk_amd/csrc/hip/rtk_colours.h b/ratatosk_amd/csrc/hip/rtk_colours.h
--- a/ratatosk_amd/csrc/hip/rtk_colours.h
+++ b/ratatosk_amd/csrc/hip/rtk_colours.h
@@ -47,6 +47,55 @@
         }
         uint32_t* t_ = src; src = dst; dst = t_;
     }
+}
+
+RTK_DEV uint32_t* rtk_radix_sort_tagged(uint32_t* a, uint32_t* b, uint8_t* ta, uint8_t* tb, uint32_t n, uint32_t* bins, uint32_t bins_words, uint32_t lo, uint32_t max_key) {
+    const uint32_t lane = static_cast<uint32_t>(rtk_lane());
+    const uint64_t lt = (1ull << lane) - 1ull;
+    uint32_t passes = 0; { uint32_t m = max_key; while (m) { ++passes; m >>= 8; } if (passes == 0) passes = 1; }
+    const bool fused = passes * 256u <= bins_words;
+    if (fused) {
+        for (uint32_t i = lane; i < passes * 256u; i += RTK_WAVE) bins[i] = 0u;
+        RTK_WG_SYNC();
+        for (uint32_t i = lane; i < n; i += RTK_WAVE) { const uint32_t key = a[i] >> lo; for (uint32_t ps = 0; ps < passes; ++ps) atomicAdd(&bins[256u * ps + ((key >> (8u * ps)) & 0xFFu)], 1u); }
+        RTK_WG_SYNC();
+    }
+    uint32_t* src = a; uint32_t* dst = b; uint8_t* ts = ta; uint8_t* td = tb;
+    for (uint32_t ps = 0; ps < passes; ++ps) {
+        const uint32_t sh = lo + 8u * ps;
+        uint32_t* const pb = fused ? bins + 256u * ps : bins;
+        if (!fused) {
+            for (uint32_t i = lane; i < 256u; i += RTK_WAVE) pb[i] = 0u;
+            RTK_WG_SYNC();
+            for (uint32_t i = lane; i < n; i += RTK_WAVE) atomicAdd(&pb[(src[i] >> sh) & 0xFFu], 1u);
+            RTK_WG_SYNC();
+        }
+        {
+            uint32_t v[4]; uint32_t sum = 0;
+            for (int x = 0; x < 4; ++x) { v[x] = pb[4u * lane + static_cast<uint32_t>(x)]; sum += v[x]; }
+            int tot; uint32_t base = static_cast<uint32_t>(rtk_wave_excl_scan(static_cast<int>(sum), &tot));
+            RTK_WG_SYNC();
+            for (int x = 0; x < 4; ++x) { pb[4u * lane + static_cast<uint32_t>(x)] = base; base += v[x]; }
+        }
+        RTK_WG_SYNC();
+        for (uint32_t c0 = 0; c0 < n; c0 += RTK_WAVE) {
+            const uint32_t i = c0 + lane; const bool ok = i < n;
+            const uint32_t key = ok ? src[i] : 0u;
+            const uint32_t tag = (ok && ts) ? ts[i] : 0u;
+            const uint32_t d = ok ? ((key >> sh) & 0xFFu) : 0x100u;
+            uint64_t eq = rtk_ballot(ok);
+            for (int bt = 0; bt < 8; ++bt) { const uint64_t bb = rtk_ballot((d >> bt) & 1u); eq &= ((d >> bt) & 1u) ? bb : ~bb; }
+            const uint32_t before = static_cast<uint32_t>(rtk_popc(eq & lt));
+            uint32_t base = 0;
+            if (ok) base = pb[d];
+            RTK_WG_SYNC();
+            if (ok && before == 0u) pb[d] = base + static_cast<uint32_t>(rtk_popc(eq));
+            if (ok) { dst[base + before] = key; if (ts) td[base + before] = static_cast<uint8_t>(tag); }
+            RTK_WG_SYNC();
+        }
+        { uint32_t* t_ = src; src = dst; dst = t_; uint8_t* u_ = ts; ts = td; td = u_; }
+    }
+    return src;
 }
 #endif
 
@@ -100,7 +149,66 @@
 #ifndef RTK_CS_MAX_IDS
 #define RTK_CS_MAX_IDS 512u
 #endif
-static_assert(2u * RTK_CS_MAX_IDS + 768u <= RTK_LDS_SET_CAP && RTK_CS_MAX_IDS <= 512u, "small path of the colour selection: universe + unsorted ids + 24 x 2 x 8 vector words in the LDS buffer");
+#define RTK_CS_TAG_BITS 6u
+#define RTK_CS_PACKED_LIMIT (1u << (32u - RTK_CS_TAG_BITS))
+static_assert(2u * RTK_CB_MAX_SLOTS <= (1u << RTK_CS_TAG_BITS), "colour selection: a tag fits its bits");
+static_assert(2u * RTK_CS_MAX_IDS + 768u + RTK_CS_MAX_IDS / 2u <= RTK_LDS_SET_CAP && RTK_CS_MAX_IDS <= 512u && RTK_CS_MAX_IDS % 4u == 0u, "colour selection, at most RTK_CS_MAX_IDS ids: two key buffers, 24 x 2 x 8 vector words (before them: three sets of sort counters) and two tag arrays in the LDS buffer");
+
+RTK_DEV uint8_t* rtk_cu_tags(uint32_t* L, uint32_t T, uint8_t* gtags) { return T > RTK_CS_MAX_IDS ? gtags : reinterpret_cast<uint8_t*>(L + 2u * RTK_CS_MAX_IDS + 768u); }
+RTK_DEV uint32_t* rtk_cu_sort(uint32_t* L, uint32_t T, uint32_t mx, uint32_t* gbuf, uint8_t* gtags, const uint8_t** tsrt) {
+    const bool big = T > RTK_CS_MAX_IDS, packed = mx < RTK_CS_PACKED_LIMIT;
+    uint8_t* const ta = packed ? nullptr : rtk_cu_tags(L, T, gtags); uint8_t* const tb = packed ? nullptr : ta + (big ? RTK_CB_MAX_IDS : RTK_CS_MAX_IDS);
+    uint32_t* const srt = rtk_radix_sort_tagged(L, big ? gbuf : L + RTK_CS_MAX_IDS, ta, tb, T, big ? L + RTK_CB_MAX_IDS : L + 2u * RTK_CS_MAX_IDS, big ? 256u : 768u, packed ? RTK_CS_TAG_BITS : 0u, mx);
+    *tsrt = srt == L ? ta : tb;
+    return srt;
+}
+RTK_DEV bool rtk_colour_universe(uint32_t* L, uint32_t T, uint32_t n_vec, uint32_t mx, uint32_t* gbuf, uint8_t* gtags, uint32_t* U_out, uint32_t* VW_out, uint64_t** vec_out) {
+    const uint32_t lane = static_cast<uint32_t>(rtk_lane());
+    const uint64_t le = (2ull << lane) - 1ull;
+    const bool big = T > RTK_CS_MAX_IDS, packed = mx < RTK_CS_PACKED_LIMIT;
+    const uint8_t* tsrt;
+    const uint32_t* srt = rtk_cu_sort(L, T, mx, gbuf, gtags, &tsrt);
+    if (big && srt == L) { for (uint32_t i = lane; i < T; i += RTK_WAVE) gbuf[i] = L[i]; RTK_WG_SYNC(); srt = gbuf; }
+    uint32_t carry = 0;
+    auto heads = [&](uint32_t idx, uint32_t w, uint32_t* id) -> uint64_t {
+        *id = packed ? (w >> RTK_CS_TAG_BITS) : w;
+        const uint32_t prev = rtk_shfl_up1(*id, carry);
+        carry = rtk_shfl(*id, 63);
+        return rtk_ballot(idx < T && (idx == 0u || *id != prev));
+    };
+    uint32_t U = 0;
+    for (uint32_t i0 = 0; i0 < T; i0 += 4u * RTK_WAVE) {
+        uint32_t w[4];
+        for (uint32_t k = 0; k < 4u; ++k) { const uint32_t idx = i0 + k * RTK_WAVE + lane; w[k] = idx < T ? srt[idx] : 0u; }
+        for (uint32_t k = 0; k < 4u; ++k) { uint32_t id; U += static_cast<uint32_t>(rtk_popc(heads(i0 + k * RTK_WAVE + lane, w[k], &id))); }
+    }
+    const uint32_t VW = U ? (U + 63u) / 64u : 1u;
+    *U_out = U; *VW_out = VW;
+    const uint32_t at = big ? ((U + 1u) & ~1u) : 2u * RTK_CS_MAX_IDS;
+    if (at + 2u * n_vec * VW > (big ? RTK_LDS_SET_CAP : 2u * RTK_CS_MAX_IDS + 768u)) return false;
+    uint64_t* const vec = reinterpret_cast<uint64_t*>(L + at);
+    for (uint32_t i = lane; i < n_vec * VW; i += RTK_WAVE) vec[i] = 0ull;
+    RTK_WG_SYNC();
+    uint32_t R = 0; carry = 0;
+    for (uint32_t i0 = 0; i0 < T; i0 += 4u * RTK_WAVE) {
+        uint32_t w[4], tg[4];
+        for (uint32_t k = 0; k < 4u; ++k) { const uint32_t idx = i0 + k * RTK_WAVE + lane; w[k] = idx < T ? srt[idx] : 0u; tg[k] = packed ? (w[k] & ((1u << RTK_CS_TAG_BITS) - 1u)) : (idx < T ? tsrt[idx] : 0u); }
+        RTK_WG_SYNC();
+        for (uint32_t k = 0; k < 4u; ++k) {
+            const uint32_t idx = i0 + k * RTK_WAVE + lane; uint32_t id;
+            const uint64_t bal = heads(idx, w[k], &id);
+            if (idx < T) {
+                const uint32_t rank = R + static_cast<uint32_t>(rtk_popc(bal & le)) - 1u;
+                if ((bal >> lane) & 1ull) L[rank] = id;
+                atomicOr(reinterpret_cast<unsigned long long*>(vec) + tg[k] * VW + (rank >> 6), 1ull << (rank & 63u));
+            }
+            R += static_cast<uint32_t>(rtk_popc(bal));
+        }
+    }
+    RTK_WG_SYNC();
+    *vec_out = vec;
+    return true;
+}
 RTK_DEV int rtk_sum8(int v) {
     v += __builtin_amdgcn_update_dpp(0, v, 0xB1, 0xF, 0xF, false);
     v += __builtin_amdgcn_update_dpp(0, v, 0x4E, 0xF, 0xF, false);
@@ -142,7 +250,7 @@
     int total = 0; const uint32_t st = static_cast<uint32_t>(rtk_wave_excl_scan(static_cast<int>(m_nl + m_ng), &total));
     const uint32_t T = static_cast<uint32_t>(rtk_u(total));
     const bool big = T > RTK_CS_MAX_IDS;
-    if (T > RTK_CB_MAX_IDS || (big && (s.set_cap < RTK_CB_MAX_IDS || s.set_cap < 2u * 2u * 64u * RTK_CB_MAX_SLOTS))) return RTK_NONE32;
+    if (T > RTK_CB_MAX_IDS || (big && s.set_cap < RTK_CB_MAX_IDS)) return RTK_NONE32;
     RTK_CS_LAP(1)
     const uint32_t min_cov_v = c.o.min_cov_vertices;
     bool dup = false;
@@ -159,62 +267,38 @@
     uint32_t k_quota = k_card < cov ? k_card : cov;
     RTK_CS_LAP(2)
     uint32_t* const L = rtk_lds_set_buf();
-    uint32_t* const uni = L; uint32_t* const raw = L + RTK_CS_MAX_IDS;
-    uint64_t* const cbm = big ? reinterpret_cast<uint64_t*>(s.set[2].get()) : reinterpret_cast<uint64_t*>(L + 2u * RTK_CS_MAX_IDS);
-    const uint32_t VW = big ? 64u : 8u;
-    uint32_t P = 64; while (P < T) P <<= 1;
-    for (uint32_t t0 = 0; t0 < P; t0 += RTK_WAVE) {
-        const uint32_t t = t0 + lane;
-        uint32_t i = 0;
-        for (uint32_t j = 1; j < n_slots; ++j) { const uint32_t sj = rtk_shfl(st, static_cast<int>(j)); if (sj <= t) i = j; }
-        const uint32_t s_i = rtk_shfl(st, static_cast<int>(i)), nl_i = rtk_shfl(m_nl, static_cast<int>(i));
-        const uint64_t lo_i = rtk_shfl(m_lo, static_cast<int>(i)), go_i = rtk_shfl(m_go, static_cast<int>(i));
-        uint32_t x = 0xFFFFFFFFu;
-        if (t < T) { const uint32_t off = t - s_i; x = col[off < nl_i ? lo_i + off : go_i + (off - nl_i)]; if (!big) raw[t] = x; }
-        if (t < T || !big) uni[t] = x;
+    uint32_t* const uni = L;
+    uint8_t* const gtags = reinterpret_cast<uint8_t*>(s.set[2].get());
+    uint32_t mx = 0;
+    for (bool packed = true;; packed = false) {
+        uint8_t* const tags = rtk_cu_tags(L, T, gtags);
+        for (uint32_t t0 = 0; t0 < T; t0 += RTK_WAVE) {
+            const uint32_t t = t0 + lane;
+            uint32_t i = 0;
+            for (uint32_t j = 1; j < n_slots; ++j) { const uint32_t sj = rtk_shfl(st, static_cast<int>(j)); if (sj <= t) i = j; }
+            const uint32_t s_i = rtk_shfl(st, static_cast<int>(i)), nl_i = rtk_shfl(m_nl, static_cast<int>(i));
+            const uint64_t lo_i = rtk_shfl(m_lo, static_cast<int>(i)), go_i = rtk_shfl(m_go, static_cast<int>(i));
+            if (t < T) {
+                const uint32_t off = t - s_i; const uint32_t tag = 2u * i + (off >= nl_i ? 1u : 0u);
+                const uint32_t x = col[off < nl_i ? lo_i + off : go_i + (off - nl_i)];
+                mx = x > mx ? x : mx;
+                if (packed) L[t] = (x << RTK_CS_TAG_BITS) | tag; else { L[t] = x; tags[t] = static_cast<uint8_t>(tag); }
+            }
+        }
+        for (int o = 32; o > 0; o >>= 1) { const uint32_t v2 = static_cast<uint32_t>(__shfl_xor(static_cast<int>(mx), o, 64)); mx = v2 > mx ? v2 : mx; }
+        mx = rtk_u(mx);
+        if (!packed || mx < RTK_CS_PACKED_LIMIT) break;
     }
     RTK_WG_SYNC();
+    RTK_CS_LAP(3)
+    uint32_t U = 0, VW = 1; uint64_t* cbm = nullptr;
+    if (!rtk_colour_universe(L, T, 2u * n_slots, mx, s.set[1], gtags, &U, &VW, &cbm)) { s.cnt[RTK_RC_COLOURS_DECLINED_FIT] += 1; return RTK_NONE32; }
     s.cnt[RTK_RC_COLOUR] += T;
-    RTK_CS_LAP(3)
-    {
-        uint32_t mx = 0; for (uint32_t i2 = lane; i2 < T; i2 += RTK_WAVE) mx = uni[i2] > mx ? uni[i2] : mx;
-        for (int o = 32; o > 0; o >>= 1) { const uint32_t v2 = static_cast<uint32_t>(__shfl_xor(static_cast<int>(mx), o, 64)); mx = v2 > mx ? v2 : mx; }
-        if (big) rtk_radix_sort_u32(uni, s.set[1], T, L + RTK_CB_MAX_IDS, rtk_u(mx));
-        else rtk_radix_sort_u32(uni, L + 2u * RTK_CS_MAX_IDS, T, L + 2u * RTK_CS_MAX_IDS + RTK_CS_MAX_IDS, rtk_u(mx));
-    }
-    uint32_t U = 0;
-    for (uint32_t i0 = 0; i0 < T; i0 += RTK_WAVE) {
-        const uint32_t i = i0 + lane;
-        uint32_t x = 0; bool keep = false;
-        if (i < T) { x = uni[i]; keep = (i == 0) || (uni[i - 1] != x); }
-        RTK_WG_SYNC();
-        const uint64_t bal = rtk_ballot(keep);
-        if (keep) uni[U + static_cast<uint32_t>(rtk_popc(bal & ((1ull << lane) - 1ull)))] = x;
-        U += static_cast<uint32_t>(rtk_popc(bal));
-        RTK_WG_SYNC();
-    }
     RTK_CS_LAP(4)
-    for (uint32_t i = lane; i < n_slots * 2u * VW; i += RTK_WAVE) cbm[i] = 0ull;
-    RTK_WG_SYNC();
-    for (uint32_t t0 = 0; t0 < T; t0 += RTK_WAVE) {
-        const uint32_t t = t0 + lane;
-        uint32_t i = 0;
-        for (uint32_t j = 1; j < n_slots; ++j) { const uint32_t sj = rtk_shfl(st, static_cast<int>(j)); if (sj <= t) i = j; }
-        const uint32_t s_i = rtk_shfl(st, static_cast<int>(i)), nl_i = rtk_shfl(m_nl, static_cast<int>(i));
-        const uint64_t lo_i2 = rtk_shfl(m_lo, static_cast<int>(i)), go_i2 = rtk_shfl(m_go, static_cast<int>(i));
-        if (t < T) {
-            const uint32_t off2 = t - s_i;
-            const uint32_t id = big ? col[off2 < nl_i ? lo_i2 + off2 : go_i2 + (off2 - nl_i)] : raw[t];
-            uint32_t lo = 0, hi = U; while (lo < hi) { const uint32_t mid = (lo + hi) >> 1; if (uni[mid] < id) lo = mid + 1; else hi = mid; }
-            const uint32_t seg = 2u * i + ((t - s_i) >= nl_i ? 1u : 0u);
-            atomicOr(reinterpret_cast<unsigned long long*>(cbm) + seg * VW + (lo >> 6), 1ull << (lo & 63u));
-        }
-    }
-    RTK_WG_SYNC();
-    RTK_CS_LAP(5)
-    auto ld = [&](uint32_t idx) -> RtkBM { if (lane >= VW) return 0ull; return big ? static_cast<RtkBM>(__hip_atomic_load(reinterpret_cast<const unsigned long long*>(cbm) + idx * VW + lane, __ATOMIC_RELAXED, __HIP_MEMORY_SCOPE_AGENT)) : cbm[idx * VW + lane]; };
-    auto cnt_ = [&](RtkBM a) -> uint32_t { return big ? rtk_bm_count(a) : rtk_bm8_count(a); };
-    auto low_ = [&](RtkBM a, uint32_t q) -> RtkBM { return big ? rtk_bm_lowest(a, q) : rtk_bm8_lowest(a, q); };
+    const bool w8 = VW <= 8u;
+    auto ld = [&](uint32_t idx) -> RtkBM { return lane < VW ? cbm[idx * VW + lane] : 0ull; };
+    auto cnt_ = [&](RtkBM a) -> uint32_t { return w8 ? rtk_bm8_count(a) : rtk_bm_count(a); };
+    auto low_ = [&](RtkBM a, uint32_t q) -> RtkBM { return w8 ? rtk_bm8_lowest(a, q) : rtk_bm_lowest(a, q); };
     RtkBM a[6];
     for (int sh = 0; sh < 6; ++sh) {
         RtkBM acc = 0ull;
@@ -268,7 +352,7 @@
             nb_unselected += quota > 0 ? 1u : 0u;
         }
     }
-    RTK_CS_LAP(6)
+    RTK_CS_LAP(5)
     const uint32_t n_all = rtk_bm_count(all);
     if (n_all > s.set_cap) { rtk_fail_ovf(s, 9); return 0; }
     uint32_t* out = s.set[0];
diff --git a/ratatosk_amd/csrc/hip/rtk_device.hip b/ratatosk_amd/csrc/hip/rtk_device.hip
--- a/ratatosk_amd/csrc/hip/rtk_device.hip
+++ b/ratatosk_amd/csrc/hip/rtk_device.hip
@@ -758,6 +758,34 @@
             for (uint32_t i = lane; i < na; i += RTK_WAVE) { out[i] = ka[i]; out[na + i] = pa[i]; }
             nout = 2u * na;
         }
+        else if (op == RTK_SETS_RADIX_TAGGED || op == RTK_SETS_COLOUR_UNIVERSE) {
+            uint32_t* const L = rtk_lds_set_buf(); uint8_t* const gtags = reinterpret_cast<uint8_t*>(work32 + RTK_CB_MAX_IDS);
+            const bool packed = sc < RTK_CS_PACKED_LIMIT; uint8_t* const tags = rtk_cu_tags(L, na, gtags);
+            for (uint32_t i = lane; i < na; i += RTK_WAVE) {
+                uint32_t tag = 0;
+                if (op == RTK_SETS_RADIX_TAGGED) tag = b[i];
+                else { uint32_t end = 0; for (uint32_t j = 0; j < nb; ++j) { end += b[j]; if (i >= end) tag = j + 1u; } }
+                if (packed) L[i] = (a[i] << RTK_CS_TAG_BITS) | tag; else { L[i] = a[i]; tags[i] = static_cast<uint8_t>(tag); }
+            }
+            rtk_sync();
+            if (op == RTK_SETS_RADIX_TAGGED) {
+                const uint8_t* tsrt; const uint32_t* const srt = rtk_cu_sort(L, na, sc, work32, gtags, &tsrt);
+                rtk_sync();
+                for (uint32_t i = lane; i < na; i += RTK_WAVE) { out[i] = packed ? (srt[i] >> RTK_CS_TAG_BITS) : srt[i]; out[na + i] = packed ? (srt[i] & ((1u << RTK_CS_TAG_BITS) - 1u)) : tsrt[i]; }
+                nout = 2u * na;
+            } else {
+                uint32_t U = 0, VW = 1; uint64_t* vec = nullptr;
+                const bool fits = rtk_colour_universe(L, na, nb, sc, work32, gtags, &U, &VW, &vec);
+                res = U;
+                if (!fits) st = RTK_SETS_DECLINED;
+                else {
+                    if (lane == 0u) { out[0] = U; out[1] = VW; }
+                    for (uint32_t i = lane; i < U; i += RTK_WAVE) out[2u + i] = L[i];
+                    for (uint32_t i = lane; i < nb * VW; i += RTK_WAVE) { out[2u + U + 2u * i] = static_cast<uint32_t>(vec[i]); out[2u + U + 2u * i + 1u] = static_cast<uint32_t>(vec[i] >> 32); }
+                    nout = 2u + U + 2u * nb * VW;
+                }
+            }
+        }
 #endif
         else if (op == RTK_SETS_BM_LOWEST
 #ifndef RTK_SIM
@@ -810,6 +838,19 @@
                 case RTK_SETS_SORT_PAIRS: { if (B != A || A > (1u << 24)) return rtk_fail(RTK_ERR_ARG, "rtk_sets_batch: SORT_PAIRS wants nb == na <= 2^24"); uint64_t pw = 1; while (pw < A) pw <<= 1; need = 4 * A; work = 2 * pw; wa = 2 * A; wb = 2 * B; break; }
                 case RTK_SETS_RADIX_U32: if (A > RTK_CB_MAX_IDS) return rtk_fail(RTK_ERR_ARG, "rtk_sets_batch: RADIX_U32 sorts at most 1664 keys"); need = A; work = (A + 1) / 2; wb = 0; break;
                 case RTK_SETS_RADIX_PAIRS_U32: if (B != A) return rtk_fail(RTK_ERR_ARG, "rtk_sets_batch: RADIX_PAIRS_U32 wants nb == na"); need = 2 * A; work = 2 * A; break;
+                case RTK_SETS_RADIX_TAGGED: case RTK_SETS_COLOUR_UNIVERSE: {
+                    if (A > RTK_CB_MAX_IDS || scalar[i] == 0xFFFFFFFFu) return rtk_fail(RTK_ERR_ARG, "rtk_sets_batch: at most 1664 ids, none above the scalar <= 0xFFFFFFFE");
+                    for (uint64_t x = 0; x < A; ++x) if (a[i][x] > scalar[i]) return rtk_fail(RTK_ERR_ARG, "rtk_sets_batch: an id above the scalar");
+                    if (op[i] == RTK_SETS_RADIX_TAGGED) {
+                        if (B != A) return rtk_fail(RTK_ERR_ARG, "rtk_sets_batch: RADIX_TAGGED wants nb == na");
+                        for (uint64_t x = 0; x < B; ++x) if (b[i][x] >= 2u * RTK_CB_MAX_SLOTS) return rtk_fail(RTK_ERR_ARG, "rtk_sets_batch: a tag above 47");
+                        need = 2 * A;
+                    } else {
+                        uint64_t sum = 0; for (uint64_t x = 0; x < B; ++x) sum += b[i][x];
+                        if (B == 0 || B > 2u * RTK_CB_MAX_SLOTS || sum != A) return rtk_fail(RTK_ERR_ARG, "rtk_sets_batch: COLOUR_UNIVERSE wants 1 .. 48 list lengths that add up to na");
+                        need = 2 + A + 2 * B * std::max<uint64_t>(1, (A + 63) / 64);
+                    }
+                    work = (RTK_CB_MAX_IDS + RTK_CB_MAX_IDS / 2u) / 2u; break; }
                 case RTK_SETS_BM_LOWEST: case RTK_SETS_BM8_LOWEST: {
                     if (A > (op[i] == RTK_SETS_BM8_LOWEST ? 512u : 4096u)) return rtk_fail(RTK_ERR_ARG, "rtk_sets_batch: universe too large for the bit vector");
                     for (uint64_t x = 1; x < A; ++x) if (a[i][x - 1] >= a[i][x]) return rtk_fail(RTK_ERR_ARG, "rtk_sets_batch: the universe is not sorted and free of repeats");
diff --git a/ratatosk_amd/csrc/hip/rtk_pipeline_run.inc b/ratatosk_amd/csrc/hip/rtk_pipeline_run.inc
--- a/ratatosk_amd/csrc/hip/rtk_pipeline_run.inc
+++ b/ratatosk_amd/csrc/hip/rtk_pipeline_run.inc
@@ -724,8 +724,8 @@
             cnt[RTK_CNT_FA_LINKED + 2], double(cnt[RTK_CNT_FINE + RTK_FINE_FA_LINKED]));
     fprintf(stderr, "[rtk trace] second strand of gap regions: run %llu, skipped %llu (the forward result decides), audit mismatches %llu\n", cnt[RTK_CNT_STRAND2 + 0], cnt[RTK_CNT_STRAND2 + 1], cnt[RTK_CNT_STRAND2 + 2]);
     fprintf(stderr, "[rtk trace] stored sweeps of the forward trims: walked for a consensus %llu, never walked %llu\n", cnt[RTK_CNT_PARK + 0], cnt[RTK_CNT_PARK + 1]);
-    fprintf(stderr, "[rtk trace] colour selections answered by: small %llu, wide %llu, bits %llu, general %llu; audit mismatches %llu\n", cnt[RTK_CNT_COLOURS + 0], cnt[RTK_CNT_COLOURS + 1], cnt[RTK_CNT_COLOURS + 2],
-            cnt[RTK_CNT_COLOURS + 3], cnt[RTK_CNT_COLOURS + 4]);
+    fprintf(stderr, "[rtk trace] colour selections answered by: small %llu, wide %llu, bits %llu, general %llu; audit mismatches %llu; handed on by the register program for room %llu\n", cnt[RTK_CNT_COLOURS + 0], cnt[RTK_CNT_COLOURS + 1], cnt[RTK_CNT_COLOURS + 2],
+            cnt[RTK_CNT_COLOURS + 3], cnt[RTK_CNT_COLOURS + 4], cnt[RTK_CNT_COLOURS + 5]);
     fprintf(stderr, "[rtk trace] walks %llu moves %llu reloads %llu scalar steps %llu cycles %.3g tail cycles %.3g\n", cnt[RTK_CNT_WALK_CALLS], cnt[RTK_CNT_WALK_MOVES],
             cnt[RTK_CNT_WALK_RELOADS], cnt[RTK_CNT_WALK_SCALAR], double(cnt[RTK_CNT_WALK_CYCLES]), double(cnt[RTK_CNT_WALK_TAIL]));
 }
@@ -746,7 +746,7 @@
     st.n_strand2_run = cnt[RTK_CNT_STRAND2 + 0]; st.n_strand2_skipped = cnt[RTK_CNT_STRAND2 + 1]; st.n_strand2_audit_mismatch = cnt[RTK_CNT_STRAND2 + 2];
     st.n_park_walked = cnt[RTK_CNT_PARK + 0]; st.n_park_deferred = cnt[RTK_CNT_PARK + 1];
     st.n_colours_small = cnt[RTK_CNT_COLOURS + 0]; st.n_colours_wide = cnt[RTK_CNT_COLOURS + 1]; st.n_colours_bits = cnt[RTK_CNT_COLOURS + 2]; st.n_colours_general = cnt[RTK_CNT_COLOURS + 3];
-    st.n_colours_audit_mismatch = cnt[RTK_CNT_COLOURS + 4];
+    st.n_colours_audit_mismatch = cnt[RTK_CNT_COLOURS + 4]; st.n_colours_declined_fit = cnt[RTK_CNT_COLOURS + 5];
     st.ms_stitch = R.t_st.elapsed(); st.ms_total = b->t_all.elapsed();
     st.n_windows = b->n_bases;
     st.n_probes_exact = cnt[RTK_CNT_PROBES_EXACT]; st.n_probes_inexact = cnt[RTK_CNT_PROBES_INEXACT]; st.n_hits_inexact = cnt[RTK_CNT_HITS_INEXACT];
diff --git a/ratatosk_amd/csrc/hip/rtk_types.h b/ratatosk_amd/csrc/hip/rtk_types.h
--- a/ratatosk_amd/csrc/hip/rtk_types.h
+++ b/ratatosk_amd/csrc/hip/rtk_types.h
@@ -168,11 +168,11 @@
     RTK_CNT_PARK = 217,
     RTK_CNT_PARK_END = 219,
     RTK_CNT_COLOURS = 219,
-    RTK_CNT_COLOURS_END = 224,
+    RTK_CNT_COLOURS_END = 225,
     RTK_CNT_USED_END = RTK_CNT_COLOURS_END,
     RTK_CNT_TOTAL = (RTK_CNT_USED_END + 31) / 32 * 32
 };
-static_assert(RTK_CNT_TOTAL == 224, "counter map: the size of the block changed (it is part of what the kernels and the host agree on)");
+static_assert(RTK_CNT_TOTAL == 256, "counter map: the size of the block changed (it is part of what the kernels and the host agree on)");
 constexpr bool rtk_cnt_apart(int a, int a_end, int b, int b_end) { return a_end <= b || b_end <= a; }
 static_assert(RTK_CNT_EVENTS_END <= RTK_CNT_CYC && RTK_CNT_CYC_END <= RTK_CNT_FINALIZE && RTK_CNT_FINALIZE_END <= RTK_CNT_WALK && RTK_CNT_WALK_END <= RTK_CNT_FINE, "counter map: the event, cycle, finalize and walk ranges overlap");
 static_assert(RTK_CNT_FINE_END <= RTK_CNT_HIST && RTK_CNT_HIST_END <= RTK_CNT_PROF && RTK_CNT_PROF_END <= RTK_CNT_WAVE_TRACE && RTK_CNT_WAVE_TRACE_END <= RTK_CNT_LANE_HANDED, "counter map: the trace ranges overlap");
@@ -192,7 +192,7 @@
     RTK_RC_FA_LINKED_RUN = 21, RTK_RC_FA_LINKED_SKIPPED = 22, RTK_RC_FA_LINKED_ENTRIES = 23,
     RTK_RC_STRAND2_RUN = 24, RTK_RC_STRAND2_SKIPPED = 25, RTK_RC_STRAND2_AUDIT_MISMATCH = 26,
     RTK_RC_PARK_WALKED = 27, RTK_RC_PARK_DEFERRED = 28,
-    RTK_RC_COLOURS_SMALL = 29, RTK_RC_COLOURS_WIDE = 30, RTK_RC_COLOURS_BITS = 31, RTK_RC_COLOURS_GENERAL = 32, RTK_RC_COLOURS_AUDIT_MISMATCH = 33, RTK_RC_N = 34 };
+    RTK_RC_COLOURS_SMALL = 29, RTK_RC_COLOURS_WIDE = 30, RTK_RC_COLOURS_BITS = 31, RTK_RC_COLOURS_GENERAL = 32, RTK_RC_COLOURS_AUDIT_MISMATCH = 33, RTK_RC_COLOURS_DECLINED_FIT = 34, RTK_RC_N = 35 };
 static_assert(RTK_CNT_ROUTES_END - RTK_CNT_ROUTES == static_cast<int>(RTK_RC_FA_LINKED_RUN) - static_cast<int>(RTK_RC_TRIM_STORED), "counter map: one slot per route counter");
 static_assert(RTK_CNT_FA_LINKED_END - RTK_CNT_FA_LINKED == static_cast<int>(RTK_RC_STRAND2_RUN) - static_cast<int>(RTK_RC_FA_LINKED_RUN), "counter map: one slot per fixAmbiguity counter");
 static_assert(RTK_CNT_STRAND2_END - RTK_CNT_STRAND2 == static_cast<int>(RTK_RC_PARK_WALKED) - static_cast<int>(RTK_RC_STRAND2_RUN), "counter map: one slot per second-strand counter");
```

New measurement: 2.234 billion (median of 6 runs). 4.2% higher.
